# iammcy/BFLC-demo

Hardware: NVIDIA H100
Metric: federated_rounds_per_sec (higher is better)
Workload: dtype mxfp8

## Files before the change

### bflc_demo_b200/csrc/bindings/bindings_extra.cpp

```cpp
#include <ATen/cuda/CUDAContext.h>
#include <c10/cuda/CUDAGuard.h>
#include <torch/extension.h>

#include <cmath>
#include <cstring>
#include <memory>
#include <cuda.h>

#include <optional>

#include "bflc_kernels.h"
#include "consensus_math.hpp"
#include "symm_heap.hpp"

namespace py = pybind11;
using OptT = std::optional<at::Tensor>;

namespace {

void check(cudaError_t e, const char* what) {
  TORCH_CHECK(e == cudaSuccess, "bflc::", what, " failed: ", cudaGetErrorString(e));
}
cudaStream_t cur_stream() { return at::cuda::getCurrentCUDAStream().stream(); }

template <typename T>
T* P(int64_t addr) { return reinterpret_cast<T*>(static_cast<uintptr_t>(addr)); }

void check_flat(const at::Tensor& t, const char* what, at::ScalarType dtype, int64_t n, int align) {
  TORCH_CHECK(t.is_cuda() && t.is_contiguous() && t.scalar_type() == dtype, what, " must be a contiguous CUDA ",
              c10::toString(dtype), " tensor");
  TORCH_CHECK(t.numel() == n, what, " has ", t.numel(), " elements, expected ", n);
  TORCH_CHECK(reinterpret_cast<uintptr_t>(t.data_ptr()) % align == 0, what, " must be ", align, "-byte aligned");
}

const float* prox_anchor(const OptT& anchor, double mu, const at::Tensor& master, const char* what) {
  const float m32 = static_cast<float>(mu);
  TORCH_CHECK(std::isfinite(m32) && m32 >= 0.f, what, ": prox_mu must be finite and >= 0, got ", mu);
  if (m32 == 0.f) return nullptr;
  TORCH_CHECK(anchor.has_value(), what, ": prox_mu > 0 needs the anchor (the round's global model)");
  check_flat(*anchor, "anchor", at::kFloat, master.numel(), 16);
  TORCH_CHECK(anchor->device() == master.device(), what, ": anchor must be on master's device");
  return anchor->data_ptr<float>();
}

bflc::FedArgs make_fed(const py::dict& d) {
  bflc::FedArgs f;
  std::memset(&f, 0, sizeof(f));
  f.rank = d["rank"].cast<int>();
  f.n_ranks = d["n_ranks"].cast<int>();
  auto bases = d["peer_bases"].cast<std::vector<int64_t>>();
  TORCH_CHECK((int)bases.size() == f.n_ranks && f.n_ranks <= bflc::kMaxRanks, "bad peer table");
  for (int r = 0; r < f.n_ranks; ++r) f.peers.base[r] = P<char>(bases[r]);
  f.peers.mc_base = P<char>(d["mc_base"].cast<int64_t>());
  auto& l = f.lay;
  l.flags_off = d["flags_off"].cast<int64_t>();
  l.state_off = d["state_off"].cast<int64_t>();
  l.plan_off = d["plan_off"].cast<int64_t>();
  l.scores_off = d["scores_off"].cast<int64_t>();
  l.meta_off = d["meta_off"].cast<int64_t>();
  l.work_master_off = d["work_master_off"].cast<int64_t>();
  l.work_shadow_off = d["work_shadow_off"].cast<int64_t>();
  auto um = d["upload_master_off"].cast<std::vector<int64_t>>();
  auto us = d["upload_shadow_off"].cast<std::vector<int64_t>>();
  l.upload_master_off[0] = um.at(0); l.upload_master_off[1] = um.at(1);
  l.upload_shadow_off[0] = us.at(0); l.upload_shadow_off[1] = us.at(1);
  l.global_off = d["global_off"].cast<int64_t>();
  l.global_shadow_off = d["global_shadow_off"].cast<int64_t>();
  l.ring_off = d["ring_off"].cast<int64_t>();
  l.n_params = d["n_params"].cast<int64_t>();
  l.admit_off = d["admit_off"].cast<int64_t>();
  l.ring_slots = d["ring_slots"].cast<int>();
  return f;
}

struct PyHeap {
  std::unique_ptr<bflc::SymmHeap> h;
};

}

void bind_extra(py::module_& m) {
  py::class_<PyHeap>(m, "SymmHeap")
      .def(py::init([](int64_t bytes, int rank, int world, int device, const std::string& mode) {
        bflc::SymmHeap::Mode md = mode == "vmm"   ? bflc::SymmHeap::Mode::VMM
                                  : mode == "ipc" ? bflc::SymmHeap::Mode::IPC
                                                  : bflc::SymmHeap::Mode::LOCAL;
        auto p = std::make_unique<PyHeap>();
        p->h = std::make_unique<bflc::SymmHeap>((size_t)bytes, rank, world, device, md);
        return p;
      }))
      .def("export_handle", [](PyHeap& s) { return py::bytes(s.h->export_handle()); })
      .def("import_handles",
           [](PyHeap& s, const std::vector<py::bytes>& blobs) {
             std::vector<std::string> v;
             for (auto& b : blobs) v.emplace_back(static_cast<std::string>(b));
             s.h->import_handles(v);
           })
      .def("fd_listen", [](PyHeap& s, const std::string& tag) { return s.h->fd_listen(tag); })
      .def("import_via_sockets",
           [](PyHeap& s, const std::vector<std::string>& names) { s.h->import_via_sockets(names); })
      .def("mc_import_via_sockets",
           [](PyHeap& s, const std::vector<std::string>& names) { return s.h->mc_import_via_sockets(names); })
      .def("mc_create_and_export", [](PyHeap& s) { return py::bytes(s.h->mc_create_and_export()); })
      .def("mc_import_and_add",
           [](PyHeap& s, const py::bytes& b) { return s.h->mc_import_and_add(std::string(b)); })
      .def("mc_bind_and_map", [](PyHeap& s) { return s.h->mc_bind_and_map(); })
      .def("local_ptr", [](PyHeap& s) { return reinterpret_cast<int64_t>(s.h->local_ptr()); })
      .def("peer_ptr", [](PyHeap& s, int r) { return reinterpret_cast<int64_t>(s.h->peer_ptr(r)); })
      .def("mc_ptr", [](PyHeap& s) { return reinterpret_cast<int64_t>(s.h->mc_ptr()); })
      .def("bytes", [](PyHeap& s) { return (int64_t)s.h->bytes(); })
      .def("last_error", [](PyHeap& s) { return s.h->last_error(); })
      .def_static("multicast_supported", [](int dev) { return bflc::SymmHeap::multicast_supported(dev); });

  m.def("tensor_from_ptr", [](int64_t ptr, std::vector<int64_t> shape, py::object dtype, int device) {
    auto st = torch::python::detail::py_object_to_dtype(dtype);
    auto opts = at::TensorOptions().dtype(st).device(at::kCUDA, device);
    return at::for_blob(P<void>(ptr), shape)
        .deleter([](void*) {})
        .options(opts)
        .target_device(at::Device(at::kCUDA, static_cast<c10::DeviceIndex>(device)))
        .make_tensor();
  });

  m.def("struct_sizes", [] {
    py::dict d;
    d["RoundState"] = sizeof(bflc::RoundState);
    d["RoundPlan"] = sizeof(bflc::RoundPlan);
    d["BlockRecord"] = sizeof(bflc::BlockRecord);
    d["UploadMeta"] = sizeof(bflc::UploadMeta);
    d["AdmitPage"] = sizeof(bflc::AdmitPage);
    d["DpPage"] = sizeof(bflc::DpPage);
    d["dp_norm_off"] = offsetof(bflc::DpPage, norm);
    d["dp_scale_off"] = offsetof(bflc::DpPage, scale);
    d["dp_sigma_off"] = offsetof(bflc::DpPage, sigma);
    d["dp_epoch_off"] = offsetof(bflc::DpPage, epoch);
    d["FLAG_NORM"] = (int)bflc::FLAG_NORM;
    d["GemmDynamic"] = sizeof(bflc::GemmDynamic);
    d["FLAG_COUNT"] = (int)bflc::FLAG_COUNT;
    d["kMaxRanks"] = bflc::kMaxRanks;
    d["kMirrorSeqWord"] = bflc::kMirrorSeqWord;
    d["plan_dyn_off"] = offsetof(bflc::RoundPlan, dyn);
    d["plan_correct_off"] = offsetof(bflc::RoundPlan, correct);
    d["plan_loss_sum_off"] = offsetof(bflc::RoundPlan, loss_sum);
    d["plan_train_correct_off"] = offsetof(bflc::RoundPlan, train_correct);
    d["plan_opt_step_off"] = offsetof(bflc::RoundPlan, opt_step);
    d["plan_is_trainer_off"] = offsetof(bflc::RoundPlan, is_trainer);
    d["plan_is_comm_off"] = offsetof(bflc::RoundPlan, is_comm);
    d["plan_step_barrier_off"] = offsetof(bflc::RoundPlan, step_barrier);
    d["plan_stamps_off"] = offsetof(bflc::RoundPlan, t_stamp);
    d["plan_round_seq_off"] = offsetof(bflc::RoundPlan, round_seq);
    d["plan_opt_total_off"] = offsetof(bflc::RoundPlan, opt_total);
    d["plan_cand_blob_off"] = offsetof(bflc::RoundPlan, cand_blob);
    d["plan_n_cand_off"] = offsetof(bflc::RoundPlan, n_cand);
    d["plan_cand_rank_off"] = offsetof(bflc::RoundPlan, cand_rank);
    d["plan_parity_off"] = offsetof(bflc::RoundPlan, parity);
    d["plan_digest_acc_off"] = offsetof(bflc::RoundPlan, digest_acc);
    d["plan_upload_blocks_off"] = offsetof(bflc::RoundPlan, upload_blocks_done);
    d["plan_consensus_blocks_off"] = offsetof(bflc::RoundPlan, consensus_blocks_done);
    d["dyn_map_index_off"] = offsetof(bflc::GemmDynamic, map_index);
    d["dyn_bias_off"] = offsetof(bflc::GemmDynamic, bias);
    d["dyn_wait_flag_off"] = offsetof(bflc::GemmDynamic, wait_flag);
    d["dyn_wait_value_off"] = offsetof(bflc::GemmDynamic, wait_value);
    d["admit_slot_off"] = offsetof(bflc::AdmitPage, slot);
    d["rec_role_before_off"] = offsetof(bflc::BlockRecord, role_before);
    d["rec_score_rows_off"] = offsetof(bflc::BlockRecord, score_rows);
    d["rec_scored_mask_off"] = offsetof(bflc::BlockRecord, scored_mask);
    d["rec_median_off"] = offsetof(bflc::BlockRecord, median);
    d["rec_n_samples_off"] = offsetof(bflc::BlockRecord, n_samples);
    d["rec_avg_cost_off"] = offsetof(bflc::BlockRecord, avg_cost);
    d["rec_weight_off"] = offsetof(bflc::BlockRecord, weight);
    d["rec_admitted_mask_off"] = offsetof(bflc::BlockRecord, admitted_mask);
    d["rec_weight_by_score_off"] = offsetof(bflc::BlockRecord, weight_by_score);
    d["rec_model_digest_off"] = offsetof(bflc::BlockRecord, model_digest);
    d["rec_seq_off"] = offsetof(bflc::BlockRecord, seq);
    d["rec_agg_off"] = offsetof(bflc::BlockRecord, agg);
    d["state_epoch_off"] = offsetof(bflc::RoundState, epoch);
    d["state_role_off"] = offsetof(bflc::RoundState, role);
    d["state_global_loss_off"] = offsetof(bflc::RoundState, global_loss);
    d["state_digest_off"] = offsetof(bflc::RoundState, model_digest);
    d["CUtensorMap"] = sizeof(CUtensorMap);
    return d;
  });

  m.def("state_init_bytes", [](int n_ranks, int n_comm, int n_aggregate, std::vector<int> roles, int n_needed) {
    bflc::RoundState st;
    std::memset(&st, 0, sizeof(st));
    st.epoch = 0; st.n_ranks = n_ranks; st.n_comm = n_comm; st.n_aggregate = n_aggregate;
    st.n_needed = (uint32_t)n_needed;
    for (int r = 0; r < n_ranks && r < bflc::kMaxRanks; ++r) st.role[r] = (uint32_t)roles.at(r);
    return py::bytes(reinterpret_cast<const char*>(&st), sizeof(st));
  }, py::arg("n_ranks"), py::arg("n_comm"), py::arg("n_aggregate"), py::arg("roles"), py::arg("n_needed") = 0);

  m.def("fed_plan_round", [](const py::dict& fd, std::vector<std::pair<int64_t, bool>> layers,
                             int steps_per_round, bool staged, int64_t blob_stage_ptr, int64_t blob_bytes,
                             std::vector<int64_t> upq_off, int64_t stage_master_ptr) {
    bflc::FedArgs f = make_fed(fd);
    TORCH_CHECK(stage_master_ptr == 0 || staged, "stage_master_ptr: the fp32 staging slots of staged validation");
    bflc::PlanLayer pl[bflc::kMaxPlanLayers];
    TORCH_CHECK((int)layers.size() <= bflc::kMaxPlanLayers, "too many plan layers");
    for (size_t i = 0; i < layers.size(); ++i) {
      pl[i].bias_off = layers[i].first;
      pl[i].use_bias = layers[i].second ? 1 : 0;
    }
    bflc::PlanBlobs pb;
    const bool blobs = blob_bytes > 0;
    if (blobs) {
      TORCH_CHECK(upq_off.size() == 2, "upq_off: heap offsets of the two parity upload blobs");
      pb.stage = P<uint8_t>(blob_stage_ptr); pb.bytes = blob_bytes;
      pb.upq_off[0] = upq_off[0]; pb.upq_off[1] = upq_off[1];
    }
    check(bflc::fed_plan_round(f, pl, (int)layers.size(), steps_per_round, staged ? 1 : 0, cur_stream(),
                               blobs ? &pb : nullptr, P<const float>(stage_master_ptr)),
          "fed_plan_round");
  }, py::arg("fed"), py::arg("layers"), py::arg("steps_per_round"), py::arg("staged"),
     py::arg("blob_stage_ptr") = 0, py::arg("blob_bytes") = 0, py::arg("upq_off") = std::vector<int64_t>{},
     py::arg("stage_master_ptr") = 0);
  m.def("fed_pull_blobs", [](const py::dict& fd, int64_t off0, int64_t off1, at::Tensor stage, at::Tensor stage_dq,
                             int in_dim, int hidden, int n_classes, std::vector<int64_t> w_offs) {
    TORCH_CHECK(stage.dim() == 2 && stage_dq.dim() == 2 && stage.size(0) == stage_dq.size(0) &&
                    stage_dq.scalar_type() == at::kBFloat16 && stage.is_contiguous() && stage_dq.is_contiguous(),
                "stage: u8 [slots, blob_bytes]; stage_dq: bf16 [slots, n_params]");
    TORCH_CHECK(w_offs.size() == 2 && w_offs[0] + (int64_t)hidden * in_dim <= stage_dq.size(1) &&
                    w_offs[1] + (int64_t)n_classes * hidden <= stage_dq.size(1) && w_offs[0] % 8 == 0 &&
                    w_offs[1] % 8 == 0,
                "w_offs: 8-aligned element offsets of W1 and W2 inside a stage_dq row");
    const bflc::Mx8Unpack un = bflc::mx8_unpack_args(in_dim, hidden, n_classes, w_offs[0], w_offs[1]);
    check(bflc::fed_pull_blobs(make_fed(fd), off0, off1, un, stage.data_ptr(), stage.size(1), stage_dq.data_ptr(),
                               stage_dq.size(1), cur_stream()),
          "fed_pull_blobs");
  });
  m.def("fed_upload", [](const py::dict& fd, int n_samples, int n_loss_terms, int byz_mode,
                         double byz_scale, int straggle_us) {
    check(bflc::fed_upload(make_fed(fd), n_samples, n_loss_terms, byz_mode, (float)byz_scale, cur_stream(),
                           straggle_us),
          "fed_upload");
  }, py::arg("fed"), py::arg("n_samples"), py::arg("n_loss_terms"), py::arg("byz_mode"), py::arg("byz_scale"),
     py::arg("straggle_us") = 0);
  m.def("fed_consensus_aggregate", [](const py::dict& fd, int n_val, bool weight_by_score,
                                      bool two_shot, bool use_mc, int64_t host_mirror,
                                      int64_t bump_seq, int rule, int trim, int server_opt,
                                      const std::vector<float>& server_hp, int64_t server_m_off,
                                      int64_t server_v_off, int dp_mode, double dp_clip, double dp_noise,
                                      uint64_t dp_seed, int64_t dp_off) {
    TORCH_CHECK(bflc::agg_rule_valid(rule, trim), "fed_consensus_aggregate: rule must be 0 (FedAvg), 1 (median) "
                "or 2 (trimmed mean, 1 <= trim <= ", bflc::kMaxTrim, "), got rule ", rule, " trim ", trim);
    TORCH_CHECK(rule == bflc::AGG_FEDAVG || !weight_by_score,
                "fed_consensus_aggregate: weight_by_score needs the FedAvg rule");
    bflc::ServerOptArgs so{};
    so.opt = server_opt;
    if (server_opt != bflc::SOPT_NONE) {
      TORCH_CHECK(server_hp.size() == 6, "fed_consensus_aggregate: server_hp = (lr, b1, b2, c1, c2, tau)");
      so.lr = server_hp[0]; so.b1 = server_hp[1]; so.b2 = server_hp[2];
      so.c1 = server_hp[3]; so.c2 = server_hp[4]; so.tau = server_hp[5];
      so.m_off = server_m_off; so.v_off = server_v_off;
    }
    const char* err = bflc::server_opt_check(so.opt, so.lr, so.b1, so.b2, so.tau);
    TORCH_CHECK(*err == '\0', "fed_consensus_aggregate: ", err);
    TORCH_CHECK(server_opt == bflc::SOPT_NONE ||
                    (server_m_off > 0 && server_m_off % 16 == 0 &&
                     (bflc::server_state_vectors(server_opt) < 2 || (server_v_off > 0 && server_v_off % 16 == 0))),
                "fed_consensus_aggregate: server optimizer state offsets must be positive multiples of 16 "
                "(server_v_off for adam / yogi)");
    bflc::DpArgs dp{};
    dp.mode = dp_mode; dp.clip = (float)dp_clip; dp.noise = (float)dp_noise; dp.seed = dp_seed; dp.off = dp_off;
    const char* dperr = bflc::dp_check(dp.mode, dp.clip, dp.noise, rule);
    TORCH_CHECK(*dperr == '\0', "fed_consensus_aggregate: ", dperr);
    TORCH_CHECK(dp_mode == bflc::DP_OFF || (dp_off > 0 && dp_off % 16 == 0),
                "fed_consensus_aggregate: dp_off must be a positive multiple of 16 (the HeapLayout dp region)");
    check(bflc::fed_consensus_aggregate(make_fed(fd), n_val, weight_by_score ? 1 : 0,
                                        two_shot ? 1 : 0, use_mc ? 1 : 0, cur_stream(),
                                        P<uint32_t>(host_mirror), P<uint32_t>(bump_seq), rule, trim, &so, &dp),
          "fed_consensus_aggregate");
  }, py::arg("fed"), py::arg("n_val"), py::arg("weight_by_score"), py::arg("two_shot"),
     py::arg("use_mc"), py::arg("host_mirror") = 0, py::arg("bump_seq") = 0, py::arg("rule") = 0,
     py::arg("trim") = 0, py::arg("server_opt") = 0, py::arg("server_hp") = std::vector<float>{},
     py::arg("server_m_off") = 0, py::arg("server_v_off") = 0, py::arg("dp_mode") = 0, py::arg("dp_clip") = 0.0,
     py::arg("dp_noise") = 0.0, py::arg("dp_seed") = 0, py::arg("dp_off") = 0);
  m.def("fed_update_norms", [](const py::dict& fd, int64_t dp_off) {
    TORCH_CHECK(dp_off > 0 && dp_off % 16 == 0, "fed_update_norms: dp_off must be a positive multiple of 16");
    check(bflc::fed_update_norms(make_fed(fd), dp_off, cur_stream()), "fed_update_norms");
  }, py::arg("fed"), py::arg("dp_off"));
  m.def("fed_pull_candidates", [](const py::dict& fd, at::Tensor stage_shadow, const OptT& stage_master,
                                  const OptT& ranges) {
    const long long* rp = ranges.has_value() ? reinterpret_cast<const long long*>(ranges->data_ptr<int64_t>())
                                             : nullptr;
    check(bflc::fed_pull_candidates(make_fed(fd), stage_shadow.data_ptr(),
                                    stage_master.has_value() ? stage_master->data_ptr<float>() : nullptr,
                                    cur_stream(), rp, ranges.has_value() ? (int)ranges->size(0) : 0),
          "fed_pull_candidates");
  }, py::arg("fed"), py::arg("stage_shadow"), py::arg("stage_master"), py::arg("ranges") = py::none());
  m.def("fed_wait_trained", [](const py::dict& fd) {
    check(bflc::fed_wait_trained(make_fed(fd), cur_stream()), "fed_wait_trained");
  });
  m.def("set_predicate", [](int64_t ptr) { bflc::set_predicate(P<const int>(ptr)); });
  m.def("current_predicate_is_null", [] { return bflc::current_predicate() == nullptr; });
  m.def("set_pdl", [](bool on) { bflc::set_pdl(on); });
  m.def("pdl_fallbacks", [] { return bflc::pdl_fallbacks(); });
  m.def("set_debug_times", [](int64_t ptr) { bflc::set_debug_times(P<long long>(ptr)); });
  m.def("p2p_read_probe", [](int64_t src, int64_t dst, int64_t n_vec) {
    check(bflc::p2p_read_probe(P<const float4>(src), P<float4>(dst), n_vec, cur_stream()),
          "p2p_read_probe");
  });
  m.def("mc_store_probe", [](int64_t mc_dst, int64_t src, int64_t n_vec) {
    check(bflc::mc_store_probe(P<float4>(mc_dst), P<const float4>(src), n_vec, cur_stream()),
          "mc_store_probe");
  });

  m.def("mx8_mlp_layout", [](int in_dim, int hidden) {
    const bflc::Mx8MlpLayout l = bflc::mx8_mlp_layout(in_dim, hidden);
    py::dict d;
    d["w1q"] = l.w1q; d["w1sf"] = l.w1sf; d["w2q"] = l.w2q; d["w2sf"] = l.w2sf;
    d["b1"] = l.b1; d["b2"] = l.b2; d["total"] = l.total; d["kb1"] = l.kb1; d["kb2"] = l.kb2;
    return d;
  });
  m.def("mlp_round", [](at::Tensor x, at::Tensor labels, at::Tensor master, at::Tensor shadow,
                        at::Tensor grad, std::vector<int64_t> offs, at::Tensor h, at::Tensor dlogits,
                        at::Tensor dh, at::Tensor loss_sum, at::Tensor correct, int64_t barrier_ptr,
                        int batch, int steps, int in_dim, int hidden, int n_classes, double lr,
                        bool adam, const OptT& mm, const OptT& vv, int64_t step_base_ptr,
                        const OptT& dbg, int plan, int epiopt, int64_t x_ready_ptr,
                        int64_t round_seq_ptr, const OptT& x_dq, const OptT& work_q, const OptT& work_dq,
                        const OptT& h_dq, const std::optional<py::dict>& fed,
                        std::vector<int64_t> upq_off, int n_samples, int n_loss_terms, int byz_mode,
                        double byz_scale, int straggle_us, const OptT& anchor, double prox_mu,
                        int64_t epoch_rows) {
    TORCH_CHECK(offs.size() == 4, "offs = element offsets of w1, b1, w2, b2 in the flat buffer");
    if (epoch_rows == 0) epoch_rows = (int64_t)steps * batch;
    TORCH_CHECK(batch > 0 && steps > 0 && epoch_rows >= batch && epoch_rows % batch == 0 &&
                    epoch_rows / batch <= steps && epoch_rows <= INT32_MAX,
                "mlp_round: epoch_rows must be a multiple of batch, between batch and steps * batch (got ",
                epoch_rows, " rows, batch ", batch, ", steps ", steps, ")");
    auto rows_of = [&](const at::Tensor& t, const char* name, int64_t width, at::ScalarType dt) {
      TORCH_CHECK(t.is_cuda() && t.scalar_type() == dt && t.is_contiguous(), "mlp_round: ", name,
                  " must be a contiguous CUDA tensor of ", c10::toString(dt));
      TORCH_CHECK(t.numel() >= epoch_rows * width, "mlp_round: ", name, " holds ", t.numel() / width,
                  " rows, one local epoch reads ", epoch_rows);
    };
    rows_of(x, "x", in_dim, at::kBFloat16);
    rows_of(labels, "labels", 1, at::kInt);
    if (x_dq.has_value()) rows_of(*x_dq, "x_dq", in_dim, at::kBFloat16);
    bflc::MlpRoundArgs r;
    r.epoch_rows = (int)epoch_rows;
    r.prox_anchor = prox_anchor(anchor, prox_mu, master, "mlp_round");
    r.prox_mu = static_cast<float>(prox_mu);
    r.batch = batch; r.steps = steps; r.in_dim = in_dim; r.hidden = hidden; r.n_classes = n_classes;
    r.ncp = (int)dlogits.stride(0);
    r.n_params = master.numel();
    r.x = x.data_ptr(); r.labels = labels.data_ptr<int32_t>();
    float* mp = master.data_ptr<float>(); float* gp = grad.data_ptr<float>();
    auto* sp = reinterpret_cast<uint16_t*>(shadow.data_ptr());
    r.master = mp; r.shadow = sp; r.grad = gp;
    r.w1_shadow = sp + offs[0]; r.w2_shadow = sp + offs[2];
    r.b1 = mp + offs[1]; r.b2 = mp + offs[3];
    r.gw1 = gp + offs[0]; r.gb1 = gp + offs[1]; r.gw2 = gp + offs[2]; r.gb2 = gp + offs[3];
    r.h = h.data_ptr(); r.dlogits = dlogits.data_ptr(); r.dh = dh.data_ptr();
    r.loss_sum = loss_sum.data_ptr<float>();
    r.correct = reinterpret_cast<unsigned int*>(correct.data_ptr());
    r.barrier = P<unsigned int>(barrier_ptr);
    r.adam = adam;
    r.adam_m = mm.has_value() ? mm->data_ptr<float>() : nullptr;
    r.adam_v = vv.has_value() ? vv->data_ptr<float>() : nullptr;
    r.lr = (float)lr;
    r.step_base = P<const int>(step_base_ptr);
    r.plan = plan; r.epiopt = epiopt;
    r.x_ready = P<const unsigned int>(x_ready_ptr); r.round_seq = P<const unsigned int>(round_seq_ptr);
    if (dbg.has_value()) {
      TORCH_CHECK(dbg->numel() >= (int64_t)steps * 32 && dbg->element_size() == 8, "dbg: int64 [steps, 32]");
      r.dbg = reinterpret_cast<unsigned long long*>(dbg->data_ptr());
    }
    if (x_dq.has_value()) {
      TORCH_CHECK(work_q.has_value() && work_dq.has_value() && h_dq.has_value(),
                  "fp8 mode needs x_dq, work_q, work_dq, h_dq");
      TORCH_CHECK(x_dq->scalar_type() == at::kBFloat16 && work_dq->scalar_type() == at::kBFloat16 &&
                      h_dq->scalar_type() == at::kBFloat16 &&
                      work_dq->numel() >= (int64_t)hidden * in_dim + 64LL * hidden,
                  "x_dq / h_dq: bf16; work_dq: bf16 [hidden * in_dim + 64 * hidden]");
      r.fp8 = true;
      r.x_dq = x_dq->data_ptr();
      r.work_q = work_q->data_ptr<uint8_t>();
      r.work_dq = reinterpret_cast<uint16_t*>(work_dq->data_ptr());
      r.h_dq = h_dq->data_ptr();
    }
    bflc::FedArgs f;
    if (fed.has_value()) {
      f = make_fed(*fed);
      r.fed = &f;
      if (upq_off.size() == 2) { r.upq_off[0] = upq_off[0]; r.upq_off[1] = upq_off[1]; }
      r.n_samples = n_samples; r.n_loss_terms = n_loss_terms; r.byz_mode = byz_mode; r.byz_scale = (float)byz_scale;
      r.straggle_us = straggle_us;
    }
    check(bflc::mlp_round_sm100(r, cur_stream()), "mlp_round_sm100");
  }, py::arg("x"), py::arg("labels"), py::arg("master"), py::arg("shadow"), py::arg("grad"), py::arg("offs"),
     py::arg("h"), py::arg("dlogits"), py::arg("dh"), py::arg("loss_sum"), py::arg("correct"),
     py::arg("barrier_ptr"), py::arg("batch"), py::arg("steps"), py::arg("in_dim"), py::arg("hidden"),
     py::arg("n_classes"), py::arg("lr"), py::arg("adam"), py::arg("m"), py::arg("v"),
     py::arg("step_base_ptr"), py::arg("dbg"), py::arg("plan"), py::arg("epiopt"), py::arg("x_ready_ptr") = 0,
     py::arg("round_seq_ptr") = 0, py::arg("x_dq") = py::none(), py::arg("work_q") = py::none(),
     py::arg("work_dq") = py::none(), py::arg("h_dq") = py::none(),
     py::arg("fed") = py::none(), py::arg("upq_off") = std::vector<int64_t>{}, py::arg("n_samples") = 0,
     py::arg("n_loss_terms") = 0, py::arg("byz_mode") = 0, py::arg("byz_scale") = 0.0,
     py::arg("straggle_us") = 0, py::arg("anchor") = py::none(), py::arg("prox_mu") = 0.0,
     py::arg("epoch_rows") = 0);
  m.def("mlp_val", [](at::Tensor x, at::Tensor labels, at::Tensor correct, at::Tensor maps,
                      int64_t dyn1_ptr, int64_t dyn2_ptr, int n_val, int in_dim, int hidden,
                      int n_classes, int max_cand, int64_t cand_blob_ptr) {
    TORCH_CHECK(x.scalar_type() == at::kBFloat16, "x: bf16 (fp8 mode: the dequantised MXFP8 x)");
    bflc::MlpValArgs r;
    r.n_val = n_val; r.in_dim = in_dim; r.hidden = hidden; r.n_classes = n_classes;
    r.max_cand = max_cand;
    r.x = x.data_ptr(); r.ldx = x.stride(0);
    r.maps = reinterpret_cast<const CUtensorMap*>(maps.data_ptr());
    r.dyn1 = P<const bflc::GemmDynamic>(dyn1_ptr);
    r.dyn2 = P<const bflc::GemmDynamic>(dyn2_ptr);
    r.labels = labels.data_ptr<int32_t>();
    r.correct = reinterpret_cast<unsigned int*>(correct.data_ptr());
    if (cand_blob_ptr != 0) {
      r.fp8 = true;
      r.cand_blob = P<const uint8_t* const>(cand_blob_ptr);
    }
    check(bflc::mlp_val_sm100(r, cur_stream()), "mlp_val_sm100");
  }, py::arg("x"), py::arg("labels"), py::arg("correct"), py::arg("maps"), py::arg("dyn1_ptr"),
     py::arg("dyn2_ptr"), py::arg("n_val"), py::arg("in_dim"), py::arg("hidden"), py::arg("n_classes"),
     py::arg("max_cand"), py::arg("cand_blob_ptr") = 0);
  m.def("quantize_mlp_blob", [](at::Tensor master, std::vector<int64_t> offs, int in_dim, int hidden,
                                int n_classes, at::Tensor blob, const OptT& dq) {
    TORCH_CHECK(offs.size() == 4, "offs = element offsets of w1, b1, w2, b2");
    TORCH_CHECK(!dq.has_value() || (dq->scalar_type() == at::kBFloat16 &&
                                    dq->numel() >= (int64_t)hidden * in_dim + 64LL * hidden),
                "dq: bf16 [hidden * in_dim + 64 * hidden]");
    check(bflc::quantize_mlp_blob(master.data_ptr<float>(), offs[0], offs[1], offs[2], offs[3], in_dim, hidden,
                                  n_classes, blob.data_ptr<uint8_t>(), cur_stream(),
                                  dq.has_value() ? dq->data_ptr() : nullptr),
          "quantize_mlp_blob");
  }, py::arg("master"), py::arg("offs"), py::arg("in_dim"), py::arg("hidden"), py::arg("n_classes"),
     py::arg("blob"), py::arg("dq") = py::none());
  m.def("mx8_dequant", [](at::Tensor q, at::Tensor sf, at::Tensor dst) {
    TORCH_CHECK(q.dim() == 2 && q.is_contiguous() && q.element_size() == 1, "q: contiguous e4m3 / u8 [R, K]");
    TORCH_CHECK(dst.sizes() == q.sizes() && dst.is_contiguous() && dst.scalar_type() == at::kBFloat16,
                "dst: contiguous bf16 [R, K]");
    check(bflc::mx8_dequant_bf16(q.data_ptr(), sf.data_ptr<uint8_t>(), (int)q.size(0), (int)q.size(1),
                                 dst.data_ptr(), cur_stream()),
          "mx8_dequant_bf16");
  });
  m.def("optim_step",
        [](bool adam, at::Tensor master, at::Tensor grad, const OptT& shadow, const OptT& mm,
           const OptT& vv, double lr, double wd, double b1, double b2, double eps, int step,
           int64_t step_dev_ptr, int64_t active_ptr, bool zero_grad) {
          const int64_t n = master.numel();
          check_flat(master, "master", at::kFloat, n, 16);
          check_flat(grad, "grad", at::kFloat, n, 16);
          if (shadow.has_value()) check_flat(*shadow, "shadow", at::kBFloat16, n, 8);
          if (adam) {
            TORCH_CHECK(mm.has_value() && vv.has_value(), "adam needs m and v");
            check_flat(*mm, "m", at::kFloat, n, 16);
            check_flat(*vv, "v", at::kFloat, n, 16);
            TORCH_CHECK(step >= 1, "adam step must be >= 1 (bias correction 1 - beta^t), got ", step);
          }
          bflc::OptimArgs a;
          a.master = master.data_ptr<float>();
          a.grad = grad.data_ptr<float>();
          a.shadow_bf16 = shadow.has_value() ? shadow->data_ptr() : nullptr;
          a.n = master.numel();
          a.lr = (float)lr; a.weight_decay = (float)wd;
          a.m = mm.has_value() ? mm->data_ptr<float>() : nullptr;
          a.v = vv.has_value() ? vv->data_ptr<float>() : nullptr;
          a.beta1 = (float)b1; a.beta2 = (float)b2; a.eps = (float)eps;
          a.step = step;
          a.step_dev = P<const int>(step_dev_ptr);
          a.active = active_ptr ? P<const int>(active_ptr) : bflc::current_predicate();
          a.zero_grad = zero_grad ? 1 : 0;
          check(adam ? bflc::adam_step(a, cur_stream()) : bflc::sgd_step(a, cur_stream()),
                "optim_step");
        });
  m.def("grad_norm_workspace_bytes", [] { return bflc::kGradNormWorkspaceBytes; });
  m.def("grad_norm",
        [](at::Tensor grad, at::Tensor workspace, at::Tensor norms, int64_t index, double max_norm,
           const OptT& skipped, int64_t active_ptr) {
          auto f32 = [](const at::Tensor& t, const char* what) {
            TORCH_CHECK(t.is_cuda() && t.is_contiguous() && t.scalar_type() == at::kFloat, what,
                        " must be a contiguous CUDA float32 tensor");
          };
          check_flat(grad, "grad", at::kFloat, grad.numel(), 16);
          f32(norms, "norms");
          TORCH_CHECK(grad.numel() > 0, "grad is empty");
          TORCH_CHECK(workspace.is_cuda() && workspace.is_contiguous() && workspace.scalar_type() == at::kByte &&
                          workspace.numel() >= bflc::kGradNormWorkspaceBytes &&
                          reinterpret_cast<uintptr_t>(workspace.data_ptr()) % 8 == 0,
                      "workspace must be an 8-byte aligned contiguous CUDA uint8 tensor of grad_norm_workspace_bytes()");
          TORCH_CHECK(0 <= index && index < norms.numel(), "norm index ", index, " outside norms[", norms.numel(), "]");
          TORCH_CHECK(max_norm > 0, "max_norm must be > 0");
          if (skipped.has_value())
            TORCH_CHECK(skipped->is_cuda() && skipped->scalar_type() == at::kInt && skipped->numel() >= 1,
                        "skipped must be a CUDA int32 tensor");
          check(bflc::grad_norm_f32(grad.data_ptr<float>(), grad.numel(), workspace.data_ptr(),
                                    norms.data_ptr<float>() + index, (float)max_norm,
                                    skipped.has_value() ? skipped->data_ptr<int>() : nullptr,
                                    active_ptr ? P<const int>(active_ptr) : bflc::current_predicate(), cur_stream()),
                "grad_norm");
        },
        py::arg("grad"), py::arg("workspace"), py::arg("norms"), py::arg("index"), py::arg("max_norm"),
        py::arg("skipped") = py::none(), py::arg("active_ptr") = 0);
  m.def("optim_recipe_step",
        [](bool adam, at::Tensor master, at::Tensor grad, const OptT& shadow, const OptT& mm, const OptT& vv,
           double lr, double b1, double b2, double eps, int step, int64_t step_dev_ptr, double decay,
           const OptT& no_decay, int schedule, int warmup, int total, const OptT& clip_workspace,
           int64_t active_ptr, bool zero_grad, const OptT& anchor, double prox_mu) {
          const int64_t n = master.numel();
          check_flat(master, "master", at::kFloat, n, 16);
          check_flat(grad, "grad", at::kFloat, n, 16);
          if (shadow.has_value()) check_flat(*shadow, "shadow", at::kBFloat16, n, 8);
          if (adam) {
            TORCH_CHECK(mm.has_value() && vv.has_value(), "adam needs m and v");
            check_flat(*mm, "m", at::kFloat, n, 16);
            check_flat(*vv, "v", at::kFloat, n, 16);
          }
          const float* anc = prox_anchor(anchor, prox_mu, master, "optim_recipe_step");
          TORCH_CHECK(step >= 1, "step must be >= 1, got ", step);
          TORCH_CHECK(schedule >= bflc::kLrConstant && schedule <= bflc::kLrCosine, "schedule id ", schedule,
                      " outside [0, 2] (constant, linear, cosine)");
          TORCH_CHECK(warmup >= 0 && total >= 0, "warmup and total steps must be >= 0");
          TORCH_CHECK(schedule == bflc::kLrConstant || total > warmup,
                      "a decaying schedule needs total steps > warmup steps");
          TORCH_CHECK(decay >= 0, "weight decay must be >= 0");
          if (no_decay.has_value()) {
            TORCH_CHECK(no_decay->is_cuda() && no_decay->is_contiguous() && no_decay->scalar_type() == at::kInt,
                        "no_decay must be a contiguous CUDA int32 tensor");
            TORCH_CHECK(no_decay->numel() == (n + 255) / 256, "no_decay has ", no_decay->numel(),
                        " words, n = ", n, " needs ", (n + 255) / 256, " (one bit per 8 floats)");
          }
          TORCH_CHECK(decay == 0 || no_decay.has_value(), "weight decay needs the no_decay mask");
          if (clip_workspace.has_value())
            TORCH_CHECK(clip_workspace->is_cuda() && clip_workspace->scalar_type() == at::kByte &&
                            clip_workspace->numel() >= bflc::kGradNormWorkspaceBytes &&
                            reinterpret_cast<uintptr_t>(clip_workspace->data_ptr()) % 8 == 0,
                        "clip_workspace must be grad_norm's CUDA uint8 workspace");
          bflc::RecipeArgs a;
          a.master = master.data_ptr<float>();
          a.grad = grad.data_ptr<float>();
          a.shadow_bf16 = shadow.has_value() ? shadow->data_ptr() : nullptr;
          a.n = n;
          a.lr = (float)lr;
          a.m = adam ? mm->data_ptr<float>() : nullptr;
          a.v = adam ? vv->data_ptr<float>() : nullptr;
          a.beta1 = (float)b1; a.beta2 = (float)b2; a.eps = (float)eps;
          a.step = step;
          a.step_dev = P<const int>(step_dev_ptr);
          a.active = active_ptr ? P<const int>(active_ptr) : bflc::current_predicate();
          a.zero_grad = zero_grad ? 1 : 0;
          a.decay = (float)decay;
          a.no_decay = no_decay.has_value() ? reinterpret_cast<const uint32_t*>(no_decay->data_ptr<int>()) : nullptr;
          a.schedule = schedule; a.warmup = warmup; a.total = total;
          a.clip = clip_workspace.has_value() ? static_cast<const bflc::GradNormState*>(clip_workspace->data_ptr())
                                              : nullptr;
          a.anchor = anc;
          a.mu = static_cast<float>(prox_mu);
          check(adam ? bflc::adam_recipe_step(a, cur_stream()) : bflc::sgd_recipe_step(a, cur_stream()),
                "optim_recipe_step");
        },
        py::arg("adam"), py::arg("master"), py::arg("grad"), py::arg("shadow"), py::arg("m"), py::arg("v"),
        py::arg("lr"), py::arg("beta1"), py::arg("beta2"), py::arg("eps"), py::arg("step"), py::arg("step_dev_ptr"),
        py::arg("decay"), py::arg("no_decay"), py::arg("schedule"), py::arg("warmup"), py::arg("total"),
        py::arg("clip_workspace"), py::arg("active_ptr") = 0, py::arg("zero_grad") = true,
        py::arg("anchor") = py::none(), py::arg("prox_mu") = 0.0);

  m.def("cast_f32_to_bf16", [](at::Tensor src, at::Tensor dst) {
    check_flat(src, "src", at::kFloat, src.numel(), 16);
    check_flat(dst, "dst", at::kBFloat16, src.numel(), 16);
    check(bflc::cast_f32_to_bf16(src.data_ptr<float>(), dst.data_ptr(), src.numel(), cur_stream()),
          "cast_f32_to_bf16");
  });
  m.def("cast_bf16_to_f32", [](at::Tensor src, at::Tensor dst) {
    check(bflc::cast_bf16_to_f32(src.data_ptr(), dst.data_ptr<float>(), src.numel(), cur_stream()),
          "cast_bf16_to_f32");
  });
  m.def("prep_inputs", [](at::Tensor src, const OptT& dst_bf16, const OptT& dst_q, const OptT& dst_sf,
                          double scale, const OptT& dst_dq) {
    TORCH_CHECK(src.dim() == 2 && src.is_contiguous(), "src: contiguous u8 [R, K]");
    TORCH_CHECK(!dst_dq.has_value() || (dst_dq->scalar_type() == at::kBFloat16 && dst_dq->numel() >= src.numel()),
                "dst_dq: bf16 [R, K]");
    check(bflc::prep_inputs_u8(src.data_ptr<uint8_t>(), dst_bf16.has_value() ? dst_bf16->data_ptr() : nullptr,
// ... 105 lines not shown
```

### bflc_demo_b200/csrc/include/bflc_kernels.h

```cpp
#pragma once
#include <cstdint>
#include <cuda.h>
#include <cuda_runtime.h>

namespace bflc {

enum class DType : int { F32 = 0, BF16 = 1, FP8_E4M3 = 2, U8 = 3 };
enum class Act : int { NONE = 0, RELU = 1, GELU = 2 };
enum class EpiKind : int { GENERIC = 0, XENT = 1, ARGMAX_ACC = 2 };

struct GemmOperand {
  const void* ptr = nullptr;
  int64_t ld = 0;
  int64_t batch_stride = 0;
  bool mn_major = false;
};

struct GemmEpilogue {
  EpiKind kind = EpiKind::GENERIC;
  void* d = nullptr;
  DType d_dtype = DType::BF16;
  int64_t ldd = 0;
  int64_t d_batch_stride = 0;
  float alpha = 1.f;
// ... 130 lines not shown
cudaError_t mlp_val_sm100(const MlpValArgs& r, cudaStream_t stream);

cudaError_t prep_inputs_u8(const uint8_t* src, void* dst_bf16, void* dst_q, uint8_t* dst_sf, int R,
                           int K, float scale, cudaStream_t s, void* dst_dq = nullptr);
cudaError_t prep_inputs_u8_chunks(const uint8_t* src, void* dst_bf16, void* dst_q, uint8_t* dst_sf,
                                  int rows_per_chunk, int K, int n_chunks, float scale,
                                  const int* in_flags, const int* in_seq, unsigned int* cnt,
                                  unsigned int* ready, unsigned int* err, cudaStream_t s,
                                  void* dst_dq = nullptr);
cudaError_t mx8_dequant_bf16(const void* q, const uint8_t* sf, int R, int K, void* dst, cudaStream_t s);
cudaError_t quantize_mlp_blob(const float* master, long long off_w1, long long off_b1,
                              long long off_w2, long long off_b2, int in_dim, int hidden,
                              int n_classes, uint8_t* blob, cudaStream_t s, void* dq = nullptr);

int gemm_pick_bn(int N, EpiKind kind, int M, int z);
unsigned long long launch_count();
void note_launch();

cudaError_t cast_f32_to_bf16(const float* src, void* dst, int64_t n, cudaStream_t s);
cudaError_t cast_bf16_to_f32(const void* src, float* dst, int64_t n, cudaStream_t s);
cudaError_t cast_u8_to_bf16(const uint8_t* src, void* dst, int64_t n, float scale, cudaStream_t s);
cudaError_t quantize_fp8(const void* src_bf16, uint8_t* dst, int64_t n, float inv_scale,
                         cudaStream_t s);
cudaError_t amax_bf16(const void* src, int64_t n, float* amax_out, cudaStream_t s);
cudaError_t fill_f32(float* dst, int64_t n, float v, cudaStream_t s);

struct OptimArgs {
  float* master = nullptr;
  const float* grad = nullptr;
  void* shadow_bf16 = nullptr;
  int64_t n = 0;
  float lr = 1e-3f, weight_decay = 0.f;
  float* m = nullptr;
  float* v = nullptr;
  float beta1 = 0.9f, beta2 = 0.999f, eps = 1e-8f;
  const int* step_dev = nullptr;
  int step = 1;
  const int* active = nullptr;
  int zero_grad = 1;
};
cudaError_t sgd_step(const OptimArgs& a, cudaStream_t s);
cudaError_t adam_step(const OptimArgs& a, cudaStream_t s);

enum LrSchedule : int { kLrConstant = 0, kLrLinear = 1, kLrCosine = 2 };
struct GradNormState {
  float coef;
  int nonfinite;
  unsigned int ticket;
  int pad;
};
constexpr int kGradNormMaxCtas = 132 * 8;
constexpr int64_t kGradNormWorkspaceBytes = sizeof(GradNormState) + 8 * kGradNormMaxCtas;
struct RecipeArgs : OptimArgs {
  float decay = 0.f;
  const uint32_t* no_decay = nullptr;
  int schedule = kLrConstant, warmup = 0, total = 0;
  const GradNormState* clip = nullptr;
  const float* anchor = nullptr;
  float mu = 0.f;
};
cudaError_t sgd_recipe_step(const RecipeArgs& a, cudaStream_t s);
cudaError_t adam_recipe_step(const RecipeArgs& a, cudaStream_t s);
cudaError_t grad_norm_f32(const float* grad, int64_t n, void* workspace, float* norm_out, float max_norm,
                          int* skipped, const int* active, cudaStream_t s);

cudaError_t im2col_bf16(const void* x, void* col, int N, int C, int H, int W, int KH, int KW,
                        int stride, int pad, int OH, int OW, int64_t ld_col, cudaStream_t s);
cudaError_t upsample_zero_bf16(const void* dy, void* up, int N, int H, int W, int OH, int OW, int C,
                               int stride, cudaStream_t s);
cudaError_t col2im_bf16(const void* col, void* dx, int N, int C, int H, int W, int KH, int KW,
                        int stride, int pad, int OH, int OW, int64_t ld_col, cudaStream_t s);
cudaError_t maxpool2d_fwd(const void* x, void* y, int32_t* idx, int N, int C, int H, int W, int k,
                          int stride, int pad, int OH, int OW, cudaStream_t s);
cudaError_t maxpool2d_bwd(const void* dy, const int32_t* idx, float* dx_f32, int64_t n_out,
                          int64_t per_out, int64_t per_in, cudaStream_t s);
cudaError_t avgpool_global_fwd(const void* x, void* y, int N, int HW, int C, cudaStream_t s);
cudaError_t avgpool_global_bwd(const void* dy, void* dx, int N, int HW, int C, cudaStream_t s);
cudaError_t batchnorm_fwd(const void* x, void* y, const float* gamma, const float* beta,
                          float* mean, float* rstd, float* run_mean, float* run_var,
                          int64_t rows, int C, float eps, float momentum, int training, int relu,
                          const void* residual, cudaStream_t s);
cudaError_t batchnorm_bwd(const void* dy, const void* x, const void* y, const float* gamma,
                          const float* mean, const float* rstd, void* dx, float* dgamma,
                          float* dbeta, void* dresidual, int64_t rows, int C, int relu,
                          cudaStream_t s);
cudaError_t layernorm_fwd(const void* x, const void* residual, void* y, const float* gamma,
                          const float* beta, float* mean, float* rstd, int64_t rows, int C,
                          float eps, cudaStream_t s);
cudaError_t layernorm_bwd(const void* dy, const void* xin, const float* gamma, const float* mean,
                          const float* rstd, void* dx, float* dgamma, float* dbeta, int64_t rows,
                          int C, cudaStream_t s);
cudaError_t softmax_rows_fwd(const void* x, void* y, int64_t rows, int cols, float scale,
                             cudaStream_t s);
cudaError_t softmax_rows_bwd(const void* dy, const void* y, void* dx, int64_t rows, int cols,
                             float scale, cudaStream_t s);
cudaError_t embedding_fwd(const int32_t* ids, const void* table_bf16, const void* pos_bf16,
                          void* out, int64_t rows, int seq, int C, cudaStream_t s,
                          const int32_t* pos_ids = nullptr);
cudaError_t embedding_bwd(const int32_t* ids, const void* dy, float* dtable, float* dpos,
                          int64_t rows, int seq, int C, cudaStream_t s, const int32_t* pos_ids = nullptr);
cudaError_t add_bf16(const void* a, const void* b, void* out, int64_t n, cudaStream_t s);
cudaError_t act_bwd_colsum(const void* dy, const void* aux, void* dz, float* colsum, int64_t rows,
                           int C, int mode, cudaStream_t s);
struct DropoutArgs {
  float p = 0.f;
  uint64_t seed = 0;
  const int32_t* step = nullptr;
  int step_add = 0;
  uint32_t site = 0;
};
cudaError_t attention_fwd_sm100(const void* q, const void* k, const void* v, void* o, float* lse, int B,
                                int S, int H, int D, long long ld, float scale, cudaStream_t stream,
                                const int32_t* lengths, const DropoutArgs* drop = nullptr, bool causal = false);
cudaError_t attention_bwd_sm100(const void* q, const void* k, const void* v, const void* o,
                                const void* dout, const float* lse, void* dq, void* dk, void* dv, int B,
                                int S, int H, int D, long long ld, float scale, cudaStream_t stream,
                                float* delta, const int32_t* lengths, const DropoutArgs* drop = nullptr,
                                bool causal = false);
cudaError_t attention_packed_fwd_sm100(const void* q, const void* k, const void* v, void* o, float* lse,
                                       const int32_t* cu_seqlens, int B, int T, int max_seqlen, int H, int D,
                                       long long ld, float scale, cudaStream_t stream,
                                       const DropoutArgs* drop = nullptr);
cudaError_t attention_packed_bwd_sm100(const void* q, const void* k, const void* v, const void* o,
                                       const void* dout, const float* lse, void* dq, void* dk, void* dv,
                                       const int32_t* cu_seqlens, int B, int T, int max_seqlen, int H, int D,
                                       long long ld, float scale, cudaStream_t stream, float* delta,
                                       const DropoutArgs* drop = nullptr);
cudaError_t dropout_keep_mask(uint8_t* mask, int B, int H, int S, const DropoutArgs& drop, cudaStream_t s);
cudaError_t dropout_add_bf16(const void* x, const void* z, void* y, int64_t rows, int C, int S,
                             const int32_t* seq_ids, const int32_t* pos_ids, const DropoutArgs& drop,
                             cudaStream_t s);
cudaError_t transpose_0213_bf16(const void* x, void* y, int d0, int d1, int d2, int d3,
                                cudaStream_t s);
cudaError_t xent_rows(const float* logits, int64_t M, int V, int64_t ld, const int32_t* targets, float* loss,
                      int32_t* hits, void* dlogits, int64_t ldd, float grad_scale, cudaStream_t s);

constexpr int kMaxRanks = 8;
constexpr int kMaxPlanLayers = 4;

struct GemmDynamic {
  int active_batches;
  int map_index[kMaxRanks];
  const float* bias[kMaxRanks];
  const uint32_t* wait_flag[kMaxRanks];
  uint32_t wait_value;
};

struct RoundState {
  uint32_t epoch;
  uint32_t n_ranks, n_comm, n_aggregate;
  uint32_t role[kMaxRanks];
  float last_median[kMaxRanks];
  uint32_t selected_mask;
  float global_loss;
  unsigned long long model_digest;
  uint32_t blocks_appended;
  uint32_t n_needed;
};

struct UploadMeta {
  uint32_t n_samples;
  float avg_cost;
};

struct RoundPlan {
  int is_trainer;
  int is_comm;
  int n_cand;
  int cand_rank[kMaxRanks];
  uint32_t parity;
  GemmDynamic dyn[kMaxPlanLayers];
  const uint8_t* cand_blob[kMaxRanks];
  unsigned int correct[kMaxRanks];
  float loss_sum;
  unsigned int train_correct;
  int opt_step;
  int opt_total;
  unsigned int upload_blocks_done;
  unsigned int consensus_blocks_done;
  unsigned long long digest_acc;
  unsigned int step_barrier;
  unsigned int round_seq;
  unsigned long long t_stamp[8];
};

enum StampSlot : int {
  STAMP_PLAN = 0,
  STAMP_UPLOAD_BEGIN = 1,
  STAMP_UPLOAD_END = 2,
  STAMP_PULL_BEGIN = 3,
  STAMP_PULL_END = 4,
  STAMP_CONS_BEGIN = 5,
  STAMP_CONS_SCORED = 6,
  STAMP_CONS_END = 7,
};

struct PeerTable {
  char* base[kMaxRanks];
  char* mc_base;
};

struct HeapLayout {
  long long flags_off;
  long long state_off;
  long long plan_off;
  long long scores_off;
  long long meta_off;
  long long work_master_off;
  long long work_shadow_off;
  long long upload_master_off[2];
  long long upload_shadow_off[2];
  long long global_off;
  long long global_shadow_off;
  long long ring_off;
  long long n_params;
  long long admit_off;
  int ring_slots;
  int pad;
};

struct AdmitPage {
  uint32_t ticket;
  uint32_t slot[kMaxRanks];
  uint32_t pad[7];
};

struct BlockRecord {
  uint32_t epoch;
  uint32_t n_ranks, n_comm, n_aggregate;
  uint32_t role_before[kMaxRanks];
  uint32_t role_after[kMaxRanks];
  float score_rows[kMaxRanks][kMaxRanks];
  uint32_t scored_mask[kMaxRanks];
  float median[kMaxRanks];
  uint32_t n_samples[kMaxRanks];
  float avg_cost[kMaxRanks];
  float weight[kMaxRanks];
  uint32_t admitted_mask;
  uint32_t selected_mask;
  float global_loss;
  uint32_t weight_by_score;
  unsigned long long model_digest;
  uint32_t seq;
  uint32_t agg;
};

enum FlagSlot : int {
  FLAG_TRAINED = 0,
  FLAG_SCORED = 8,
  FLAG_DONE = 16,
  FLAG_SLICE = 24,
  FLAG_NORM = 32,
  FLAG_COUNT = 64
};

constexpr int kDpMaxBlocks = 132 * 4;
struct DpPage {
  double partial[2][kMaxRanks][kMaxRanks];
  float norm[kMaxRanks];
  float scale[kMaxRanks];
  float sigma;
  uint32_t epoch;
  unsigned int ticket;
  uint32_t pad;
  double block[kDpMaxBlocks][kMaxRanks];
};

struct FedArgs {
  PeerTable peers;
  HeapLayout lay;
  int rank;
  int n_ranks;
};

struct PlanLayer {
  long long bias_off;
  int use_bias;
};

struct PlanBlobs {
  uint8_t* stage = nullptr; long long bytes = 0; long long upq_off[2] = {0, 0};
};
cudaError_t fed_plan_round(const FedArgs& f, const PlanLayer* layers, int n_layers,
                           int steps_per_round, int staged, cudaStream_t s,
                           const PlanBlobs* blobs = nullptr, const float* stage_master = nullptr);
cudaError_t fed_upload(const FedArgs& f, int n_samples, int n_loss_terms, int byz_mode,
                       float byz_scale, cudaStream_t s, int straggle_us = 0);
constexpr int kMirrorSeqWord = 64;
struct ServerOptArgs {
  int opt;
  float lr, b1, b2, c1, c2, tau;
  long long m_off, v_off;
};
struct DpArgs {
  int mode;
  float clip, noise;
  unsigned long long seed;
  long long off;
};
cudaError_t fed_consensus_aggregate(const FedArgs& f, int n_val, int weight_by_score,
                                    int two_shot, int use_multicast, cudaStream_t s,
                                    uint32_t* host_mirror = nullptr, uint32_t* bump_seq = nullptr,
                                    int rule = 0, int trim = 0, const ServerOptArgs* so = nullptr,
                                    const DpArgs* dp = nullptr);
cudaError_t fed_update_norms(const FedArgs& f, long long dp_off, cudaStream_t s);

cudaError_t fed_pull_candidates(const FedArgs& f, void* stage_shadow, float* stage_master,
                                cudaStream_t s, const long long* ranges = nullptr, int n_ranges = 0);
cudaError_t fed_pull_blobs(const FedArgs& f, long long off0, long long off1, const Mx8Unpack& un,
                           void* stage_blob, long long blob_bytes, void* stage_dq, long long stage_stride,
                           cudaStream_t s);
cudaError_t fed_wait_trained(const FedArgs& f, cudaStream_t s);

void set_predicate(const int* pred);
void set_pdl(bool on);
bool pdl_enabled();
unsigned long long pdl_fallbacks();
void set_debug_times(long long* dev_buf8);
const int* current_predicate();

cudaError_t p2p_read_probe(const float4* peer_src, float4* local_dst, int64_t n_vec,
                           cudaStream_t s);
cudaError_t mc_store_probe(float4* mc_dst, const float4* local_src, int64_t n_vec,
                           cudaStream_t s);

}
```

### bflc_demo_b200/csrc/kernels/elementwise_optim.cu

```cuda
#include <cuda_bf16.h>
#include <cuda_fp8.h>

#include "bflc_kernels.h"
#include "epi_common.cuh"
#include "launch.cuh"
#include "sm100_ptx.cuh"

namespace bflc {

namespace {

constexpr int kBlock = 256;
inline int grid_for(int64_t n_vec) {
  int64_t g = (n_vec + kBlock - 1) / kBlock;
  const int64_t cap = 132 * 8;
  if (g > cap) g = cap;
  if (g < 1) g = 1;
  return static_cast<int>(g);
}

using epi::pack_bf16x2;

__global__ void k_cast_f32_bf16(const float* __restrict__ src, __nv_bfloat16* __restrict__ dst,
                                int64_t n) {
// ... 132 lines not shown
}

__device__ __forceinline__ float prox_grad(float g, float w, float w0, float mu) {
  return __fmaf_rn(mu, __fsub_rn(w, w0), g);
}

template <bool kAdam, bool kRecipe = false>
__global__ void k_optim(OptimParams<kRecipe> a) {
  ptx::pdl_launch_dependents();
  ptx::pdl_wait();
  if (a.active != nullptr && *a.active == 0) return;
  const int64_t tid = blockIdx.x * static_cast<int64_t>(blockDim.x) + threadIdx.x;
  const int64_t stride = static_cast<int64_t>(gridDim.x) * blockDim.x;
  float bc1 = 1.f, bc2 = 1.f;
  if (kAdam) {
    const int t = (a.step_dev ? *a.step_dev : 0) + a.step;
    bc1 = 1.f - powf(a.beta1, static_cast<float>(t));
    bc2 = 1.f - powf(a.beta2, static_cast<float>(t));
  }
  float lr = a.lr, coef = 1.f, dec = 0.f;
  if constexpr (kRecipe) {
    if (a.clip != nullptr) {
      coef = a.clip->coef;
      if (a.clip->nonfinite) {
        if (a.zero_grad) {
          float* g = const_cast<float*>(a.grad);
          for (int64_t i = tid; i < a.n / 4; i += stride)
            reinterpret_cast<float4*>(g)[i] = make_float4(0.f, 0.f, 0.f, 0.f);
          for (int64_t i = a.n / 4 * 4 + tid; i < a.n; i += stride) g[i] = 0.f;
        }
        return;
      }
    }
    const int t = (a.step_dev ? *a.step_dev : 0) + a.step;
    lr = a.lr * lr_factor(a.schedule, a.warmup, a.total, t - 1);
    dec = lr * a.decay;
  }
  const int64_t nv = a.n / 4;
  __nv_bfloat16* sh = reinterpret_cast<__nv_bfloat16*>(a.shadow_bf16);
  for (int64_t i = tid; i < nv; i += stride) {
    float4 w = reinterpret_cast<float4*>(a.master)[i];
    const float4 g4 = reinterpret_cast<const float4*>(a.grad)[i];
    float wv[4] = {w.x, w.y, w.z, w.w};
    const float gv[4] = {g4.x, g4.y, g4.z, g4.w};
    float keep = 1.f;
    float gq[4] = {gv[0], gv[1], gv[2], gv[3]};
    if constexpr (kRecipe) {
      keep = 1.f - block_decay(a.no_decay, i >> 1, dec);
#pragma unroll
      for (int k = 0; k < 4; ++k) gq[k] = __fmul_rn(coef, gv[k]);
      if (a.anchor != nullptr) {
        const float4 w0 = __ldg(reinterpret_cast<const float4*>(a.anchor) + i);
        gq[0] = prox_grad(gq[0], wv[0], w0.x, a.mu); gq[1] = prox_grad(gq[1], wv[1], w0.y, a.mu);
        gq[2] = prox_grad(gq[2], wv[2], w0.z, a.mu); gq[3] = prox_grad(gq[3], wv[3], w0.w, a.mu);
      }
    }
    if (kAdam) {
      float4 m4 = reinterpret_cast<float4*>(a.m)[i];
      float4 v4 = reinterpret_cast<float4*>(a.v)[i];
      float mv[4] = {m4.x, m4.y, m4.z, m4.w};
      float vv[4] = {v4.x, v4.y, v4.z, v4.w};
#pragma unroll
      for (int k = 0; k < 4; ++k) {
        if constexpr (kRecipe) {
          recipe_update<true>(wv[k], mv[k], vv[k], gq[k], keep, a, lr, bc1, bc2);
        } else {
          const float g = gv[k] + a.weight_decay * wv[k];
          mv[k] = a.beta1 * mv[k] + (1.f - a.beta1) * g;
          vv[k] = a.beta2 * vv[k] + (1.f - a.beta2) * g * g;
          wv[k] -= a.lr * (mv[k] / bc1) / (sqrtf(vv[k] / bc2) + a.eps);
        }
      }
      reinterpret_cast<float4*>(a.m)[i] = make_float4(mv[0], mv[1], mv[2], mv[3]);
      reinterpret_cast<float4*>(a.v)[i] = make_float4(vv[0], vv[1], vv[2], vv[3]);
    } else {
#pragma unroll
      for (int k = 0; k < 4; ++k) {
        if constexpr (kRecipe) {
          float m_unused = 0.f, v_unused = 0.f;
          recipe_update<false>(wv[k], m_unused, v_unused, gq[k], keep, a, lr, bc1, bc2);
        } else {
          wv[k] -= a.lr * (gv[k] + a.weight_decay * wv[k]);
        }
      }
    }
    reinterpret_cast<float4*>(a.master)[i] = make_float4(wv[0], wv[1], wv[2], wv[3]);
    if (sh) {
      uint2 o;
      o.x = pack_bf16x2(wv[0], wv[1]);
      o.y = pack_bf16x2(wv[2], wv[3]);
      reinterpret_cast<uint2*>(sh)[i] = o;
    }
    if (a.zero_grad)
      reinterpret_cast<float4*>(const_cast<float*>(a.grad))[i] = make_float4(0.f, 0.f, 0.f, 0.f);
  }
  for (int64_t i = nv * 4 + tid; i < a.n; i += stride) {
    float w = a.master[i];
    if constexpr (kRecipe) {
      float m = kAdam ? a.m[i] : 0.f, v = kAdam ? a.v[i] : 0.f;
      float g = __fmul_rn(coef, a.grad[i]);
      if (a.anchor != nullptr) g = prox_grad(g, w, __ldg(a.anchor + i), a.mu);
      recipe_update<kAdam>(w, m, v, g, 1.f - block_decay(a.no_decay, i >> 3, dec), a, lr, bc1, bc2);
      if (kAdam) { a.m[i] = m; a.v[i] = v; }
    } else {
      float g = a.grad[i] + a.weight_decay * w;
      if (kAdam) {
        const float m = a.beta1 * a.m[i] + (1.f - a.beta1) * g;
        const float v = a.beta2 * a.v[i] + (1.f - a.beta2) * g * g;
        a.m[i] = m; a.v[i] = v;
        w -= a.lr * (m / bc1) / (sqrtf(v / bc2) + a.eps);
      } else {
        w -= a.lr * g;
      }
    }
    a.master[i] = w;
    if (sh) sh[i] = __float2bfloat16(w);
    if (a.zero_grad) const_cast<float*>(a.grad)[i] = 0.f;
  }
}

struct NormArgs {
  const float* grad; int64_t n; GradNormState* st; double* partials; float* norm_out; float max_norm;
  int* skipped; const int* active;
};

__device__ __forceinline__ double block_sum(double x, double* red) {
#pragma unroll
  for (int off = 16; off >= 1; off >>= 1) x += __shfl_xor_sync(0xffffffffu, x, off);
  if ((threadIdx.x & 31) == 0) red[threadIdx.x >> 5] = x;
  __syncthreads();
  double s = 0.0;
#pragma unroll
  for (int w = 0; w < kBlock / 32; ++w) s += red[w];
  return s;
}

__global__ void __launch_bounds__(kBlock) k_grad_norm(NormArgs a) {
  ptx::pdl_launch_dependents();
  ptx::pdl_wait();
  if (a.active != nullptr && *a.active == 0) return;
  __shared__ double red[kBlock / 32];
  __shared__ bool last;
  const int64_t tid = blockIdx.x * static_cast<int64_t>(blockDim.x) + threadIdx.x;
  const int64_t stride = static_cast<int64_t>(gridDim.x) * blockDim.x;
  const int64_t nv = a.n / 4;
  double acc = 0.0;
  for (int64_t i = tid; i < nv; i += stride) {
    const float4 g = reinterpret_cast<const float4*>(a.grad)[i];
    acc = fma(static_cast<double>(g.x), static_cast<double>(g.x), acc);
    acc = fma(static_cast<double>(g.y), static_cast<double>(g.y), acc);
    acc = fma(static_cast<double>(g.z), static_cast<double>(g.z), acc);
    acc = fma(static_cast<double>(g.w), static_cast<double>(g.w), acc);
  }
  for (int64_t i = nv * 4 + tid; i < a.n; i += stride) acc = fma(static_cast<double>(a.grad[i]), static_cast<double>(a.grad[i]), acc);
  const double cta = block_sum(acc, red);
  if (threadIdx.x == 0) {
    a.partials[blockIdx.x] = cta;
    __threadfence();
    last = atomicAdd(&a.st->ticket, 1u) == gridDim.x - 1;
  }
  __syncthreads();
  if (!last) return;
  __threadfence();
  double p = 0.0;
  for (int j = threadIdx.x; j < static_cast<int>(gridDim.x); j += kBlock) p += __ldcg(a.partials + j);
  __syncthreads();
  const double total = block_sum(p, red);
  if (threadIdx.x == 0) {
    const float norm = static_cast<float>(sqrt(total));
    const bool bad = !isfinite(norm);
    *a.norm_out = norm;
    a.st->coef = bad ? 1.f : fminf(1.f, __fdiv_rn(a.max_norm, norm + 1e-6f));
    a.st->nonfinite = bad ? 1 : 0;
    if (bad && a.skipped != nullptr) *a.skipped += 1;
    a.st->ticket = 0u;
  }
}

__device__ __forceinline__ void prep_group(const uint8_t* __restrict__ src, __nv_bfloat16* dbf, uint8_t* dq,
                                           uint8_t* dsf, __nv_bfloat16* ddq, int row, int g, int K, int n_kb,
                                           float scale) {
  const int k0 = g * 32;
  const int n = K - k0 < 32 ? K - k0 : 32;
  const long long off = static_cast<long long>(row) * K + k0;
  uint32_t wd[8] = {0, 0, 0, 0, 0, 0, 0, 0};
  {
    const uint4 a = __ldcg(reinterpret_cast<const uint4*>(src + off));
    wd[0] = a.x; wd[1] = a.y; wd[2] = a.z; wd[3] = a.w;
    if (n > 16) {
      const uint4 b = __ldcg(reinterpret_cast<const uint4*>(src + off + 16));
      wd[4] = b.x; wd[5] = b.y; wd[6] = b.z; wd[7] = b.w;
    }
  }
  float v[32];
#pragma unroll
  for (int i = 0; i < 32; ++i) v[i] = static_cast<float>((wd[i >> 2] >> (8 * (i & 3))) & 0xffu) * scale;
  if (dbf != nullptr) {
    uint4* o = reinterpret_cast<uint4*>(dbf + off);
#pragma unroll
    for (int i = 0; i < 4; ++i) {
      if (i * 8 >= n) break;
      o[i] = make_uint4(pack_bf16x2(v[8 * i], v[8 * i + 1]), pack_bf16x2(v[8 * i + 2], v[8 * i + 3]),
                        pack_bf16x2(v[8 * i + 4], v[8 * i + 5]), pack_bf16x2(v[8 * i + 6], v[8 * i + 7]));
    }
  }
  if (dq != nullptr || ddq != nullptr) {
    uint32_t w[8];
    const int e = epi::mx8_quant32(v, w);
    if (dq != nullptr) {
      uint4* o = reinterpret_cast<uint4*>(dq + off);
      o[0] = make_uint4(w[0], w[1], w[2], w[3]);
      if (n > 16) o[1] = make_uint4(w[4], w[5], w[6], w[7]);
      dsf[epi::mx8_sf_index(row, g, n_kb)] = static_cast<uint8_t>(e);
    }
    if (ddq != nullptr) epi::mx8_dq32_store(w, e, ddq + off, n);
  }
}

struct PrepArgs {
  const uint8_t* src; __nv_bfloat16* dbf; uint8_t* dq; uint8_t* dsf; __nv_bfloat16* ddq;
  int R, K; float scale;
  int rows_per_chunk, n_chunks;
  const int* in_flags;
  const int* in_seq;
  unsigned int* cnt;
  unsigned int* ready;
  unsigned int* err;
};

__global__ void __launch_bounds__(256) k_prep_inputs(PrepArgs a, const int* pred) {
  ptx::pdl_launch_dependents();
  ptx::pdl_wait();
  if (pred != nullptr && *pred == 0) return;
  const int G = (a.K + 31) / 32, n_kb = (a.K + 127) / 128;
  const long long total = static_cast<long long>(a.R) * G;
  const long long stride = static_cast<long long>(gridDim.x) * blockDim.x;
  for (long long i = blockIdx.x * static_cast<long long>(blockDim.x) + threadIdx.x; i < total; i += stride)
    prep_group(a.src, a.dbf, a.dq, a.dsf, a.ddq, static_cast<int>(i / G), static_cast<int>(i % G), a.K, n_kb,
               a.scale);
}

__global__ void __launch_bounds__(256) k_mx8_dequant(const uint8_t* __restrict__ q, const uint8_t* __restrict__ sf,
                                                     int R, int K, __nv_bfloat16* __restrict__ dst) {
  ptx::pdl_launch_dependents();
  ptx::pdl_wait();
  const int G = (K + 31) / 32, n_kb = (K + 127) / 128;
  const long long total = static_cast<long long>(R) * G;
  const long long stride = static_cast<long long>(gridDim.x) * blockDim.x;
  for (long long i = blockIdx.x * static_cast<long long>(blockDim.x) + threadIdx.x; i < total; i += stride) {
    const int row = static_cast<int>(i / G), g = static_cast<int>(i % G);
    const int n = K - g * 32 < 32 ? K - g * 32 : 32;
    const long long off = static_cast<long long>(row) * K + g * 32;
    uint32_t w[8] = {0, 0, 0, 0, 0, 0, 0, 0};
    const uint4 a = *reinterpret_cast<const uint4*>(q + off);
    w[0] = a.x; w[1] = a.y; w[2] = a.z; w[3] = a.w;
    if (n > 16) {
      const uint4 b = *reinterpret_cast<const uint4*>(q + off + 16);
      w[4] = b.x; w[5] = b.y; w[6] = b.z; w[7] = b.w;
    }
    epi::mx8_dq32_store(w, sf[epi::mx8_sf_index(row, g, n_kb)], dst + off, n);
  }
}

__global__ void __launch_bounds__(256) k_prep_chunks(PrepArgs a) {
  ptx::pdl_launch_dependents();
  ptx::pdl_wait();
  const int want = *reinterpret_cast<const volatile int*>(a.in_seq) + 1;
  const int G = (a.K + 31) / 32, n_kb = (a.K + 127) / 128;
  const long long per = static_cast<long long>(a.rows_per_chunk) * G;
  const long long tid = blockIdx.x * static_cast<long long>(blockDim.x) + threadIdx.x;
  const long long stride = static_cast<long long>(gridDim.x) * blockDim.x;
  for (int s = 0; s < a.n_chunks; ++s) {
    if (threadIdx.x == 0) {
      unsigned long long spins = 0;
      unsigned int ns = 20;
      while (static_cast<int>(ptx::ld_acquire_sys(reinterpret_cast<const uint32_t*>(a.in_flags + s))) - want < 0) {
        if (++spins > (1ull << 14)) { __nanosleep(ns); if (ns < 2000) ns *= 2; }
        if (spins > (1ull << 14) + 5000000ull) {
          if (a.err != nullptr) atomicExch(a.err, 1u);
          break;
        }
      }
    }
    __syncthreads();
    const int row0 = s * a.rows_per_chunk;
    for (long long i = tid; i < per; i += stride)
      prep_group(a.src, a.dbf, a.dq, a.dsf, a.ddq, row0 + static_cast<int>(i / G), static_cast<int>(i % G), a.K,
                 n_kb, a.scale);
    __syncthreads();
    if (threadIdx.x == 0) {
      __threadfence();
      const unsigned int old = atomicAdd(a.cnt + s, 1u);
      if ((old + 1u) % gridDim.x == 0u)
        asm volatile("st.release.gpu.global.u32 [%0], %1;" ::"l"(a.ready + s), "r"(static_cast<unsigned int>(want))
                     : "memory");
    }
  }
}

struct BlobArgs {
  const float* master; long long off_w1, off_b1, off_w2, off_b2;
  int in_dim, hidden, n_classes; uint8_t* blob; Mx8MlpLayout l; __nv_bfloat16* dq;
};
__device__ __forceinline__ void blob_group(const float* w, int ld, int rows, int K, int row, int g, int n_kb,
                                           uint8_t* q, uint8_t* sf, int q_rows, __nv_bfloat16* dq) {
  uint8_t* sfp = sf + epi::mx8_sf_index(row, g, n_kb);
  const int k0 = g * 32;
  if (k0 >= K || row >= q_rows) { *sfp = 127; return; }
  const int n = K - k0 < 32 ? K - k0 : 32;
  float v[32];
#pragma unroll
  for (int i = 0; i < 32; ++i) v[i] = (row < rows && i < n) ? w[static_cast<long long>(row) * ld + k0 + i] : 0.f;
  uint32_t o[8];
  const int e = epi::mx8_quant32(v, o);
  *sfp = static_cast<uint8_t>(e);
  uint8_t* qp = q + static_cast<long long>(row) * ld + k0;
  for (int i = 0; i < n / 4; ++i) reinterpret_cast<uint32_t*>(qp)[i] = o[i];
  if (dq != nullptr) {
    __nv_bfloat16* d = dq + static_cast<long long>(row) * ld + k0;
    for (int i = 0; i < n / 4; ++i) *reinterpret_cast<uint2*>(d + 4 * i) = epi::mx8_dq4(o[i], e);
  }
}
__global__ void __launch_bounds__(256) k_quantize_mlp_blob(BlobArgs a) {
  ptx::pdl_launch_dependents();
  ptx::pdl_wait();
  const int g1 = a.l.kb1 * 4, g2 = a.l.kb2 * 4;
  const int r1 = (a.hidden + 127) / 128 * 128;
  const long long n1 = static_cast<long long>(r1) * g1, n2 = 128LL * g2, n3 = a.hidden + 64;
  const long long stride = static_cast<long long>(gridDim.x) * blockDim.x;
  for (long long i = blockIdx.x * static_cast<long long>(blockDim.x) + threadIdx.x; i < n1 + n2 + n3; i += stride) {
    if (i < n1) {
      blob_group(a.master + a.off_w1, a.in_dim, a.hidden, a.in_dim, static_cast<int>(i / g1), static_cast<int>(i % g1),
                 a.l.kb1, a.blob + a.l.w1q, a.blob + a.l.w1sf, a.hidden, a.dq);
    } else if (i < n1 + n2) {
      const long long u = i - n1;
      blob_group(a.master + a.off_w2, a.hidden, a.n_classes, a.hidden, static_cast<int>(u / g2), static_cast<int>(u % g2),
                 a.l.kb2, a.blob + a.l.w2q, a.blob + a.l.w2sf, 64,
                 a.dq != nullptr ? a.dq + static_cast<long long>(a.hidden) * a.in_dim : nullptr);
    } else {
      const int u = static_cast<int>(i - n1 - n2);
      float* b = reinterpret_cast<float*>(a.blob + (u < a.hidden ? a.l.b1 + 4 * u : a.l.b2 + 4 * (u - a.hidden)));
      *b = u < a.hidden ? a.master[a.off_b1 + u]
                        : (u - a.hidden < a.n_classes ? a.master[a.off_b2 + u - a.hidden] : 0.f);
    }
  }
}

}

#define BFLC_LAUNCH_1D(kernel, nvec, ...)                       \
  do {                                                          \
    (void)cudaGetLastError();  \
    kernel<<<grid_for(nvec), kBlock, 0, s>>>(__VA_ARGS__);      \
    note_launch();                                              \
    return cudaGetLastError();                                  \
  } while (0)

#define BFLC_LAUNCH_1D_PDL(kernel, nvec, ...)                                          \
  do {                                                                                \
    note_launch();                                                                    \
    return launch_pdl(kernel, dim3(grid_for(nvec)), dim3(kBlock), 0, s, __VA_ARGS__); \
  } while (0)

cudaError_t cast_f32_to_bf16(const float* src, void* dst, int64_t n, cudaStream_t s) {
  BFLC_LAUNCH_1D(k_cast_f32_bf16, n / 8 + 1, src, reinterpret_cast<__nv_bfloat16*>(dst), n);
}
cudaError_t cast_bf16_to_f32(const void* src, float* dst, int64_t n, cudaStream_t s) {
  BFLC_LAUNCH_1D(k_cast_bf16_f32, n, reinterpret_cast<const __nv_bfloat16*>(src), dst, n);
}
cudaError_t prep_inputs_u8(const uint8_t* src, void* dst_bf16, void* dst_q, uint8_t* dst_sf, int R,
                           int K, float scale, cudaStream_t s, void* dst_dq) {
  if (K % 16 != 0 || R <= 0 || (dst_q != nullptr && dst_sf == nullptr)) return cudaErrorInvalidValue;
  PrepArgs a{};
  a.src = src; a.dbf = reinterpret_cast<__nv_bfloat16*>(dst_bf16); a.dq = static_cast<uint8_t*>(dst_q);
  a.dsf = dst_sf; a.ddq = static_cast<__nv_bfloat16*>(dst_dq); a.R = R; a.K = K; a.scale = scale;
  const long long total = static_cast<long long>(R) * ((K + 31) / 32);
  note_launch();
  return launch_pdl(k_prep_inputs, dim3(grid_for(total)), dim3(kBlock), 0, s, a, current_predicate());
}
cudaError_t prep_inputs_u8_chunks(const uint8_t* src, void* dst_bf16, void* dst_q, uint8_t* dst_sf,
                                  int rows_per_chunk, int K, int n_chunks, float scale,
                                  const int* in_flags, const int* in_seq, unsigned int* cnt,
                                  unsigned int* ready, unsigned int* err, cudaStream_t s, void* dst_dq) {
  if (K % 16 != 0 || n_chunks <= 0 || rows_per_chunk <= 0 || (dst_q != nullptr && dst_sf == nullptr))
    return cudaErrorInvalidValue;
  PrepArgs a{};
  a.src = src; a.dbf = reinterpret_cast<__nv_bfloat16*>(dst_bf16); a.dq = static_cast<uint8_t*>(dst_q);
  a.dsf = dst_sf; a.ddq = static_cast<__nv_bfloat16*>(dst_dq); a.R = rows_per_chunk * n_chunks; a.K = K; a.scale = scale;
  a.rows_per_chunk = rows_per_chunk; a.n_chunks = n_chunks;
  a.in_flags = in_flags; a.in_seq = in_seq; a.cnt = cnt; a.ready = ready; a.err = err;
  note_launch();
  return launch_pdl(k_prep_chunks, dim3(16), dim3(256), 0, s, a);
}
cudaError_t quantize_mlp_blob(const float* master, long long off_w1, long long off_b1,
                              long long off_w2, long long off_b2, int in_dim, int hidden,
                              int n_classes, uint8_t* blob, cudaStream_t s, void* dq) {
  if (in_dim % 4 != 0 || hidden % 4 != 0 || n_classes > 64) return cudaErrorInvalidValue;
  BlobArgs a{master, off_w1, off_b1, off_w2, off_b2, in_dim, hidden, n_classes, blob,
             mx8_mlp_layout(in_dim, hidden), static_cast<__nv_bfloat16*>(dq)};
  const long long total = static_cast<long long>((hidden + 127) / 128 * 128) * a.l.kb1 * 4 + 128LL * a.l.kb2 * 4 +
                          hidden + 64;
  note_launch();
  return launch_pdl(k_quantize_mlp_blob, dim3(grid_for(total)), dim3(kBlock), 0, s, a);
}
cudaError_t mx8_dequant_bf16(const void* q, const uint8_t* sf, int R, int K, void* dst, cudaStream_t s) {
  if (K % 16 != 0 || R <= 0) return cudaErrorInvalidValue;
  note_launch();
  return launch_pdl(k_mx8_dequant, dim3(grid_for(static_cast<long long>(R) * ((K + 31) / 32))), dim3(kBlock), 0, s,
                    static_cast<const uint8_t*>(q), sf, R, K, static_cast<__nv_bfloat16*>(dst));
}
cudaError_t cast_u8_to_bf16(const uint8_t* src, void* dst, int64_t n, float scale,
                            cudaStream_t s) {
  BFLC_LAUNCH_1D_PDL(k_cast_u8_bf16, n / 16 + 1, src, reinterpret_cast<__nv_bfloat16*>(dst), n,
                     scale, current_predicate());
}
cudaError_t quantize_fp8(const void* src_bf16, uint8_t* dst, int64_t n, float inv_scale,
                         cudaStream_t s) {
  BFLC_LAUNCH_1D(k_quant_fp8, n / 8 + 1, reinterpret_cast<const __nv_bfloat16*>(src_bf16), dst, n,
                 inv_scale);
}
cudaError_t amax_bf16(const void* src, int64_t n, float* amax_out, cudaStream_t s) {
  BFLC_LAUNCH_1D(k_amax_bf16, n, reinterpret_cast<const __nv_bfloat16*>(src), n, amax_out);
}
cudaError_t fill_f32(float* dst, int64_t n, float v, cudaStream_t s) {
  BFLC_LAUNCH_1D(k_fill, n, dst, n, v);
}
cudaError_t add_bf16(const void* a, const void* b, void* out, int64_t n, cudaStream_t s) {
  BFLC_LAUNCH_1D(k_add_bf16, n / 8 + 1, reinterpret_cast<const __nv_bfloat16*>(a),
                 reinterpret_cast<const __nv_bfloat16*>(b), reinterpret_cast<__nv_bfloat16*>(out),
                 n);
}
cudaError_t sgd_step(const OptimArgs& a, cudaStream_t s) {
  BFLC_LAUNCH_1D_PDL(k_optim<false>, a.n / 4 + 1, a);
}
cudaError_t adam_step(const OptimArgs& a, cudaStream_t s) {
  if (!a.m || !a.v) return cudaErrorInvalidValue;
  BFLC_LAUNCH_1D_PDL(k_optim<true>, a.n / 4 + 1, a);
}

static bool recipe_ok(const RecipeArgs& a) {
  if (a.schedule < kLrConstant || a.schedule > kLrCosine || a.warmup < 0 || a.total < 0 || !(a.decay >= 0.f))
    return false;
  if (a.schedule != kLrConstant && a.total <= a.warmup) return false;
  return a.decay == 0.f || a.no_decay != nullptr;
}
cudaError_t sgd_recipe_step(const RecipeArgs& a, cudaStream_t s) {
  if (!recipe_ok(a)) return cudaErrorInvalidValue;
  BFLC_LAUNCH_1D_PDL((k_optim<false, true>), a.n / 4 + 1, a);
}
cudaError_t adam_recipe_step(const RecipeArgs& a, cudaStream_t s) {
  if (!a.m || !a.v || !recipe_ok(a)) return cudaErrorInvalidValue;
  BFLC_LAUNCH_1D_PDL((k_optim<true, true>), a.n / 4 + 1, a);
}
cudaError_t grad_norm_f32(const float* grad, int64_t n, void* workspace, float* norm_out, float max_norm,
                          int* skipped, const int* active, cudaStream_t s) {
  if (workspace == nullptr || norm_out == nullptr || n <= 0) return cudaErrorInvalidValue;
  NormArgs a{grad, n, static_cast<GradNormState*>(workspace),
             reinterpret_cast<double*>(static_cast<char*>(workspace) + sizeof(GradNormState)), norm_out,
             max_norm, skipped, active};
  static_assert(sizeof(GradNormState) % 8 == 0, "partials must be 8-byte aligned");
  BFLC_LAUNCH_1D_PDL(k_grad_norm, n / 4 + 1, a);
}

}
```

### bflc_demo_b200/csrc/kernels/fed_kernels.cu

```cuda
#include <cuda_bf16.h>

#include "bflc_kernels.h"
#include "consensus_math.hpp"
#include "epi_common.cuh"
#include "fed_admit.cuh"
#include "launch.cuh"
#include "sm100_ptx.cuh"

namespace bflc {

namespace {

constexpr int kFedThreads = 256;

template <typename T>
__device__ __forceinline__ T* at(char* base, long long off) {
  return reinterpret_cast<T*>(base + off);
}

__device__ __forceinline__ uint32_t pack_bf16x2(float a, float b) {
  __nv_bfloat162 t = __floats2bfloat162_rn(a, b);
  return *reinterpret_cast<uint32_t*>(&t);
}

struct PlanLayers {
  PlanLayer l[kMaxPlanLayers];
  int n;
  int steps_per_round;
  int staged;
  int use_blob;
  uint8_t* stage_blob; long long blob_bytes; long long upq_off[2];
  const float* stage_master;
};

__device__ __forceinline__ unsigned long long globaltimer_ns() {
  unsigned long long t;
  asm volatile("mov.u64 %0, %%globaltimer;" : "=l"(t));
  return t;
}
__device__ __forceinline__ void stamp(RoundPlan* plan, int slot) {
  atomicMax(&plan->t_stamp[slot], globaltimer_ns());
}

__global__ void k_plan(FedArgs f, PlanLayers layers) {
  ptx::pdl_launch_dependents();
  ptx::pdl_wait();
  if (threadIdx.x != 0 || blockIdx.x != 0) return;
  char* me = f.peers.base[f.rank];
  const RoundState* st = at<RoundState>(me, f.lay.state_off);
  RoundPlan* plan = at<RoundPlan>(me, f.lay.plan_off);
  for (int i = 0; i < 8; ++i) plan->t_stamp[i] = 0;
  plan->t_stamp[STAMP_PLAN] = globaltimer_ns();
  uint32_t* flags = at<uint32_t>(me, f.lay.flags_off);
  const uint32_t epoch = st->epoch;
  const uint32_t par = epoch & 1u;
  if (epoch >= 2) {
    for (int r = 0; r < f.n_ranks; ++r) ptx::wait_flag_ge(flags + FLAG_DONE + r, epoch - 1);
  }
  plan->is_trainer = (st->role[f.rank] & ROLE_TRAINER) ? 1 : 0;
  plan->is_comm = (st->role[f.rank] & ROLE_COMM) ? 1 : 0;
  plan->parity = par;
  int n_cand = 0;
  for (int r = 0; r < f.n_ranks; ++r)
    if (st->role[r] & ROLE_TRAINER) plan->cand_rank[n_cand++] = r;
  if (admit::first_k(st)) {
    n_cand = static_cast<int>(st->n_needed);
    for (int z = 0; z < kMaxRanks; ++z) plan->cand_rank[z] = -1;
  }
  plan->n_cand = n_cand;
  for (int l = 0; l < layers.n; ++l) {
    GemmDynamic& d = plan->dyn[l];
    d.active_batches = plan->is_comm ? n_cand : 0;
    d.wait_value = epoch + 1;
    for (int z = 0; z < kMaxRanks; ++z) {
      const int t = (z < n_cand && plan->cand_rank[z] >= 0) ? plan->cand_rank[z] : 0;
      d.map_index[z] = layers.staged ? (l * kMaxRanks + z)
                                     : ((l * 2 + static_cast<int>(par)) * kMaxRanks + t);
      const float* params = layers.staged && layers.stage_master != nullptr
                                ? layers.stage_master + static_cast<long long>(z) * f.lay.n_params
                                : at<float>(f.peers.base[t], f.lay.upload_master_off[par]);
      d.bias[z] = layers.l[l].use_bias ? params + layers.l[l].bias_off : nullptr;
      d.wait_flag[z] = layers.staged ? nullptr : flags + FLAG_TRAINED + t;
    }
  }
  for (int z = 0; z < kMaxRanks; ++z) {
    plan->correct[z] = 0;
    const int t = (z < n_cand && plan->cand_rank[z] >= 0) ? plan->cand_rank[z] : f.rank;
    plan->cand_blob[z] = !layers.use_blob ? nullptr
                         : layers.staged  ? layers.stage_blob + z * layers.blob_bytes
                                          : reinterpret_cast<const uint8_t*>(f.peers.base[t]) + layers.upq_off[par];
  }
  plan->loss_sum = 0.f;
  plan->train_correct = 0;
  plan->upload_blocks_done = 0;
  plan->consensus_blocks_done = 0;
  plan->digest_acc = 0ull;
  plan->step_barrier = 0u;
  plan->round_seq = plan->round_seq + 1u;
  plan->opt_step = plan->opt_total;
  if (plan->is_trainer) plan->opt_total += layers.steps_per_round;
}

__global__ void __launch_bounds__(kFedThreads)
k_upload(FedArgs f, int n_samples, int n_loss_terms, int byz_mode, float byz_scale, int straggle_us) {
  ptx::pdl_launch_dependents();
  ptx::pdl_wait();
  char* me = f.peers.base[f.rank];
  const RoundState* st = at<RoundState>(me, f.lay.state_off);
  RoundPlan* plan = at<RoundPlan>(me, f.lay.plan_off);
  if (!(st->role[f.rank] & ROLE_TRAINER)) return;
  if (blockIdx.x == 0 && threadIdx.x == 0) stamp(plan, STAMP_UPLOAD_BEGIN);
  const uint32_t epoch = st->epoch;
  const uint32_t par = epoch & 1u;
  const float4* wm = at<const float4>(me, f.lay.work_master_off);
  const float4* gm = at<const float4>(me, f.lay.global_off);
  float4* um = at<float4>(me, f.lay.upload_master_off[par]);
  uint2* us = at<uint2>(me, f.lay.upload_shadow_off[par]);
  const long long nv = f.lay.n_params / 4;
  const long long tid = blockIdx.x * static_cast<long long>(blockDim.x) + threadIdx.x;
  const long long stride = static_cast<long long>(gridDim.x) * blockDim.x;
  for (long long i = tid; i < nv; i += stride) {
    float4 w = wm[i];
    if (byz_mode == 1) {
      const float4 g = gm[i];
      w.x = g.x - byz_scale * (w.x - g.x);
      w.y = g.y - byz_scale * (w.y - g.y);
      w.z = g.z - byz_scale * (w.z - g.z);
      w.w = g.w - byz_scale * (w.w - g.w);
    }
    um[i] = w;
    us[i] = make_uint2(pack_bf16x2(w.x, w.y), pack_bf16x2(w.z, w.w));
  }
  __syncthreads();
  __shared__ bool last;
  if (threadIdx.x == 0) {
    __threadfence_system();
    const unsigned done = atomicAdd(&plan->upload_blocks_done, 1u);
    last = (done == gridDim.x - 1);
  }
  __syncthreads();
  if (!last) return;
  __threadfence_system();
  __shared__ int ticket;
  if (threadIdx.x == 0) {
    admit::straggle(straggle_us);
    ticket = admit::first_k(st) ? admit::take_ticket(&admit::page(f.peers.base[0], f.lay, par)->ticket, epoch) : 0;
    if (ticket >= static_cast<int>(st->n_needed) && admit::first_k(st)) ticket = -1;
  }
  __syncthreads();
  if (ticket >= 0 && threadIdx.x < f.n_ranks) {
    const int r = threadIdx.x;
    UploadMeta* meta = at<UploadMeta>(f.peers.base[r], f.lay.meta_off) + par * kMaxRanks + f.rank;
    UploadMeta m;
    m.n_samples = static_cast<uint32_t>(n_samples);
    m.avg_cost = plan->loss_sum / static_cast<float>(n_loss_terms > 0 ? n_loss_terms : 1);
    *meta = m;
    __threadfence_system();
    if (admit::first_k(st))
      ptx::st_release_sys(&admit::page(f.peers.base[r], f.lay, par)->slot[ticket],
                          ((epoch + 1u) << 8) | static_cast<uint32_t>(f.rank));
    ptx::st_release_sys(at<uint32_t>(f.peers.base[r], f.lay.flags_off) + FLAG_TRAINED + f.rank,
                        epoch + 1);
  }
  __syncthreads();
  if (threadIdx.x == 0) stamp(plan, STAMP_UPLOAD_END);
}

struct ConsShared {
  ConsensusIn<kMaxRanks> in;
  ConsensusOut<kMaxRanks> out;
  int sel_rank[kMaxRanks];
  float sel_w[kMaxRanks];
  int n_sel;
};

__device__ __forceinline__ unsigned long long digest_term(float v, long long idx) {
  return static_cast<unsigned long long>(__float_as_uint(v)) *
         (static_cast<unsigned long long>(2 * idx + 1) * 0x9E3779B97F4A7C15ull);
}

struct DpShared {
  float s[kMaxRanks];
  float norm[kMaxRanks];
  float scale[kMaxRanks];
  float sigma;
  uint32_t clipped;
};

template <bool kRobust, int kServerOpt, int kDp>
__device__ __forceinline__ void consensus_body(FedArgs f, int n_val, int weight_by_score, int two_shot, int use_mc,
                                               uint32_t* host_mirror, uint32_t* bump_seq, uint32_t agg,
                                               ServerOptArgs so, DpArgs dp, DpShared* dsh) {
  __shared__ ConsShared sh;
  __shared__ bool last;
  ptx::pdl_launch_dependents();
  ptx::pdl_wait();
  char* me = f.peers.base[f.rank];
  RoundState* st = at<RoundState>(me, f.lay.state_off);
  RoundPlan* plan = at<RoundPlan>(me, f.lay.plan_off);
  uint32_t* flags = at<uint32_t>(me, f.lay.flags_off);
  const uint32_t epoch = st->epoch;
  const uint32_t par = epoch & 1u;
  const int n = f.n_ranks;
  const bool i_am_comm = (st->role[f.rank] & ROLE_COMM) != 0;
  if (blockIdx.x == 0 && threadIdx.x == 0) stamp(plan, STAMP_CONS_BEGIN);

  const bool fk = admit::first_k(st);
  __shared__ int cand_of[kMaxRanks];
  __shared__ uint32_t adm_mask;
  if (threadIdx.x == 0) {
    uint32_t m = 0;
    for (int z = 0; z < plan->n_cand; ++z) {
      cand_of[z] = fk ? admit::wait_slot(admit::page(me, f.lay, par), z, epoch) : plan->cand_rank[z];
      m |= 1u << cand_of[z];
    }
    adm_mask = m;
  }
  __syncthreads();

  if (blockIdx.x == 0 && i_am_comm) {
    if (threadIdx.x < n) {
      const int r = threadIdx.x;
      float* row = at<float>(f.peers.base[r], f.lay.scores_off) +
                   (par * kMaxRanks + f.rank) * kMaxRanks;
      for (int z = 0; z < plan->n_cand; ++z)
        row[cand_of[z]] =
            static_cast<float>(plan->correct[z]) / static_cast<float>(n_val > 0 ? n_val : 1);
      ptx::st_release_sys(at<uint32_t>(f.peers.base[r], f.lay.flags_off) + FLAG_SCORED + f.rank,
                          epoch + 1);
    }
  }

  if (threadIdx.x < n) {
    const int r = threadIdx.x;
    if (st->role[r] & ROLE_COMM) ptx::wait_flag_ge(flags + FLAG_SCORED + r, epoch + 1);
    if ((st->role[r] & ROLE_TRAINER) && ((adm_mask >> r) & 1u)) ptx::wait_flag_ge(flags + FLAG_TRAINED + r, epoch + 1);
  }
  __syncthreads();
  if (blockIdx.x == 0 && threadIdx.x == 0) stamp(plan, STAMP_CONS_SCORED);

  {
    ConsensusIn<kMaxRanks>& in = sh.in;
    const float* rows = at<float>(me, f.lay.scores_off) + par * kMaxRanks * kMaxRanks;
    const UploadMeta* meta = at<UploadMeta>(me, f.lay.meta_off) + par * kMaxRanks;
    const int i = threadIdx.x;
    if (i < kMaxRanks * kMaxRanks) {
      const int r = i / kMaxRanks, t = i % kMaxRanks;
      const bool ok = r < n && t < n && (st->role[r] & ROLE_COMM) && (st->role[t] & ROLE_TRAINER) &&
                      ((adm_mask >> t) & 1u);
      in.scored[r][t] = ok ? 1 : 0;
      in.score[r][t] =
          ok ? __uint_as_float(ptx::ld_relaxed_sys(reinterpret_cast<const uint32_t*>(rows + r * kMaxRanks + t))) : 0.f;
    } else if (i < kMaxRanks * kMaxRanks + kMaxRanks) {
      const int r = i - kMaxRanks * kMaxRanks;
      in.role[r] = r < n ? st->role[r] : 0u;
      in.admitted[r] = (r < n && (st->role[r] & ROLE_TRAINER) && ((adm_mask >> r) & 1u)) ? 1 : 0;
      in.n_samples[r] = r < n ? ptx::ld_relaxed_sys(&meta[r].n_samples) : 0u;
      in.avg_cost[r] =
          r < n ? __uint_as_float(ptx::ld_relaxed_sys(reinterpret_cast<const uint32_t*>(&meta[r].avg_cost))) : 0.f;
    }
  }
  __syncthreads();
  if (threadIdx.x == 0) {
    ConsensusIn<kMaxRanks>& in = sh.in;
    in.n_ranks = n;
    in.n_comm = static_cast<int>(st->n_comm);
    in.n_aggregate = static_cast<int>(st->n_aggregate);
    in.weight_by_score = weight_by_score;
    run_consensus<kMaxRanks>(in, sh.out);
    int k = 0;
    for (int r = 0; r < n; ++r)
      if (sh.out.selected[r]) {
        sh.sel_rank[k] = r;
        sh.sel_w[k] = sh.out.weight[r];
        ++k;
      }
    sh.n_sel = k;
  }
  __syncthreads();
  if constexpr (kDp != DP_OFF) {
    if (threadIdx.x < n) ptx::wait_flag_ge(flags + FLAG_NORM + threadIdx.x, epoch + 1);
    __syncthreads();
    if (threadIdx.x == 0) {
      const volatile double* part = at<const double>(me, dp.off + offsetof(DpPage, partial)) + par * kMaxRanks * kMaxRanks;
      for (int t = 0; t < kMaxRanks; ++t) {
        float nrm = __uint_as_float(0x7FC00000u), sc = nrm;
        if (sh.in.admitted[t]) {
          double sum = 0.0;
          for (int q = 0; q < n; ++q) sum += part[q * kMaxRanks + t];
          nrm = dp_norm(sum);
          sc = dp_scale(nrm, dp.clip);
        }
        dsh->norm[t] = nrm;
        dsh->scale[t] = sc;
      }
      uint32_t clipped = 0, wmax = 0;
      for (int k = 0; k < sh.n_sel; ++k) {
        const float sc = dsh->scale[sh.sel_rank[k]];
        dsh->s[k] = sc;
        if (dp_bits(sc) != 0x3F800000u) clipped |= 1u << k;
        const uint32_t wb = dp_bits(sh.sel_w[k]);
        wmax = wb > wmax ? wb : wmax;
      }
      dsh->clipped = clipped;
      dsh->sigma = kDp == DP_NOISE && sh.n_sel > 0 ? so_mul(so_mul(dp.noise, dp.clip), dp_float(wmax)) : 0.f;
    }
    __syncthreads();
  }

  const int n_sel = sh.n_sel;
  const int trim = agg_trim(static_cast<int>(agg & 0xFFu), static_cast<int>((agg >> 8) & 0xFFu), n_sel);
  const float4* src[kMaxRanks];
  float w[kMaxRanks];
#pragma unroll
  for (int k = 0; k < kMaxRanks; ++k) {
    const int r = k < n_sel ? sh.sel_rank[k] : f.rank;
    src[k] = at<const float4>(f.peers.base[r], f.lay.upload_master_off[par]);
    w[k] = k < n_sel ? sh.sel_w[k] : 0.f;
  }
  const long long nv = f.lay.n_params / 4;
  long long lo = 0, hi = nv;
  if (two_shot) {
    long long per = (nv + n - 1) / n;
    per += per & 1;
    lo = per * f.rank;
    hi = lo + per < nv ? lo + per : nv;
    if (lo > nv) lo = nv;
  }
  float4* g_f32 = at<float4>(me, f.lay.global_off);
  uint2* g_b16 = at<uint2>(me, f.lay.global_shadow_off);
  float4* w_f32 = at<float4>(me, f.lay.work_master_off);
  uint2* w_b16 = at<uint2>(me, f.lay.work_shadow_off);
  const bool mc = two_shot && use_mc && f.peers.mc_base != nullptr;
  float4* s_m = at<float4>(me, so.m_off);
  float4* s_v = at<float4>(me, so.v_off);
  unsigned long long dig = 0ull;
  const long long tid = blockIdx.x * static_cast<long long>(blockDim.x) + threadIdx.x;
  const long long stride = static_cast<long long>(gridDim.x) * blockDim.x;
  for (long long i = lo + tid; i < hi; i += stride) {
    float4 acc = make_float4(0.f, 0.f, 0.f, 0.f);
    if (n_sel == 0) {
      acc = g_f32[i];
    } else {
      float4 v[kMaxRanks];
#pragma unroll
      for (int k = 0; k < kMaxRanks; ++k)
        if (k < n_sel) v[k] = ptx::ld_peer_f4(src[k] + i);
      if constexpr (kDp != DP_OFF) {
        const float4 g = g_f32[i];
        const uint32_t clipped = dsh->clipped;
#pragma unroll
        for (int k = 0; k < kMaxRanks; ++k)
          if (k < n_sel && ((clipped >> k) & 1u)) {
            const float s = dsh->s[k];
            v[k].x = dp_clip_value(g.x, v[k].x, s);
            v[k].y = dp_clip_value(g.y, v[k].y, s);
            v[k].z = dp_clip_value(g.z, v[k].z, s);
            v[k].w = dp_clip_value(g.w, v[k].w, s);
          }
      }
      if constexpr (kRobust) {
        float c[kMaxRanks];
#pragma unroll
        for (int k = 0; k < kMaxRanks; ++k) c[k] = v[k].x;
        acc.x = robust_combine<kMaxRanks>(c, n_sel, trim);
#pragma unroll
        for (int k = 0; k < kMaxRanks; ++k) c[k] = v[k].y;
        acc.y = robust_combine<kMaxRanks>(c, n_sel, trim);
#pragma unroll
        for (int k = 0; k < kMaxRanks; ++k) c[k] = v[k].z;
        acc.z = robust_combine<kMaxRanks>(c, n_sel, trim);
#pragma unroll
        for (int k = 0; k < kMaxRanks; ++k) c[k] = v[k].w;
        acc.w = robust_combine<kMaxRanks>(c, n_sel, trim);
      } else {
#pragma unroll
        for (int k = 0; k < kMaxRanks; ++k)
          if (k < n_sel) {
            acc.x = fmaf(w[k], v[k].x, acc.x);
            acc.y = fmaf(w[k], v[k].y, acc.y);
            acc.z = fmaf(w[k], v[k].z, acc.z);
            acc.w = fmaf(w[k], v[k].w, acc.w);
          }
      }
      if constexpr (kDp == DP_NOISE) {
        float z[4];
        dp_gauss4(dp.seed, epoch, static_cast<uint64_t>(i), z);
        const float sigma = dsh->sigma;
        acc.x = so_add(acc.x, so_mul(sigma, z[0]));
        acc.y = so_add(acc.y, so_mul(sigma, z[1]));
        acc.z = so_add(acc.z, so_mul(sigma, z[2]));
        acc.w = so_add(acc.w, so_mul(sigma, z[3]));
      }
      if constexpr (kServerOpt != SOPT_NONE) {
        const ServerOptParams p{so.lr, so.b1, so.b2, so.c1, so.c2, so.tau};
        const float4 g = g_f32[i];
        float4 m = s_m[i];
        float4 v = make_float4(0.f, 0.f, 0.f, 0.f);
        if constexpr (kServerOpt != SOPT_MOMENTUM) v = s_v[i];
        acc.x = server_step(kServerOpt, g.x, acc.x, m.x, v.x, p);
        acc.y = server_step(kServerOpt, g.y, acc.y, m.y, v.y, p);
        acc.z = server_step(kServerOpt, g.z, acc.z, m.z, v.z, p);
        acc.w = server_step(kServerOpt, g.w, acc.w, m.w, v.w, p);
        s_m[i] = m;
        if constexpr (kServerOpt != SOPT_MOMENTUM) s_v[i] = v;
      }
    }
    dig += digest_term(acc.x, 4 * i) + digest_term(acc.y, 4 * i + 1) +
           digest_term(acc.z, 4 * i + 2) + digest_term(acc.w, 4 * i + 3);
    const uint2 b = make_uint2(pack_bf16x2(acc.x, acc.y), pack_bf16x2(acc.z, acc.w));
    if (!two_shot) {
      g_f32[i] = acc; g_b16[i] = b; w_f32[i] = acc; w_b16[i] = b;
    } else if (mc) {
      ptx::multimem_st_f4(at<float4>(f.peers.mc_base, f.lay.global_off) + i, acc);
      ptx::multimem_st_f4(at<float4>(f.peers.mc_base, f.lay.work_master_off) + i, acc);
      const unsigned am = __activemask();
      const uint32_t ox = __shfl_down_sync(am, b.x, 1), oy = __shfl_down_sync(am, b.y, 1);
      if ((i & 1) == 0) {
        const float4 pk = make_float4(__uint_as_float(b.x), __uint_as_float(b.y), __uint_as_float(ox),
                                      __uint_as_float(oy));
        ptx::multimem_st_f4(at<float4>(f.peers.mc_base, f.lay.global_shadow_off) + (i >> 1), pk);
        ptx::multimem_st_f4(at<float4>(f.peers.mc_base, f.lay.work_shadow_off) + (i >> 1), pk);
      }
    } else {
      for (int r = 0; r < n; ++r) {
        char* pb = f.peers.base[r];
        at<float4>(pb, f.lay.global_off)[i] = acc;
        at<uint2>(pb, f.lay.global_shadow_off)[i] = b;
        at<float4>(pb, f.lay.work_master_off)[i] = acc;
        at<uint2>(pb, f.lay.work_shadow_off)[i] = b;
      }
    }
  }
#pragma unroll
  for (int off = 16; off >= 1; off >>= 1) dig += __shfl_xor_sync(0xffffffffu, dig, off);
  if ((threadIdx.x & 31) == 0 && dig) atomicAdd(&plan->digest_acc, dig);

  __syncthreads();
  if (threadIdx.x == 0) {
    __threadfence_system();
    const unsigned done = atomicAdd(&plan->consensus_blocks_done, 1u);
    last = (done == gridDim.x - 1);
  }
  __syncthreads();
  if (!last) return;
  __threadfence_system();

  if (two_shot) {
    if (threadIdx.x < n) {
      const int r = threadIdx.x;
      unsigned long long* slot =
          reinterpret_cast<unsigned long long*>(at<float>(f.peers.base[r], f.lay.scores_off) +
                                                2 * kMaxRanks * kMaxRanks) +
          par * kMaxRanks + f.rank;
      *slot = *reinterpret_cast<volatile unsigned long long*>(&plan->digest_acc);
      __threadfence_system();
      ptx::st_release_sys(at<uint32_t>(f.peers.base[r], f.lay.flags_off) + FLAG_SLICE + f.rank,
                          epoch + 1);
    }
    __syncthreads();
    if (threadIdx.x < n) ptx::wait_flag_ge(flags + FLAG_SLICE + threadIdx.x, epoch + 1);
    __syncthreads();
  }

  if (threadIdx.x == 0) {
    unsigned long long digest = 0ull;
    if (two_shot) {
      const unsigned long long* slots =
          reinterpret_cast<const unsigned long long*>(at<float>(me, f.lay.scores_off) +
                                                      2 * kMaxRanks * kMaxRanks) +
          par * kMaxRanks;
      for (int r = 0; r < n; ++r)
        digest += *reinterpret_cast<const volatile unsigned long long*>(slots + r);
    } else {
      digest = *reinterpret_cast<volatile unsigned long long*>(&plan->digest_acc);
    }
    const ConsensusIn<kMaxRanks>& in = sh.in;
    const ConsensusOut<kMaxRanks>& out = sh.out;
    BlockRecord* rec =
        at<BlockRecord>(me, f.lay.ring_off) + (epoch % static_cast<uint32_t>(f.lay.ring_slots));
    rec->epoch = epoch;
    rec->n_ranks = static_cast<uint32_t>(n);
    rec->n_comm = st->n_comm;
    rec->n_aggregate = st->n_aggregate;
    uint32_t adm = 0, sel = 0;
    for (int r = 0; r < kMaxRanks; ++r) {
      rec->role_before[r] = in.role[r];
      rec->role_after[r] = r < n ? out.role_after[r] : 0u;
      uint32_t m = 0;
      for (int t = 0; t < kMaxRanks; ++t) {
        rec->score_rows[r][t] = in.score[r][t];
        if (in.scored[r][t]) m |= 1u << t;
      }
      rec->scored_mask[r] = m;
      rec->median[r] = r < n ? out.median[r] : 0.f;
      rec->n_samples[r] = in.n_samples[r];
      rec->avg_cost[r] = in.avg_cost[r];
      rec->weight[r] = r < n ? out.weight[r] : 0.f;
      if (in.admitted[r]) adm |= 1u << r;
      if (r < n && out.selected[r]) sel |= 1u << r;
    }
    rec->admitted_mask = adm;
    rec->selected_mask = sel;
    rec->global_loss = out.global_loss;
    rec->weight_by_score = static_cast<uint32_t>(weight_by_score);
    rec->model_digest = digest;
    rec->agg = agg;
    __threadfence();
    rec->seq = epoch + 1;
    for (int r = 0; r < n; ++r) {
      st->role[r] = out.role_after[r];
      st->last_median[r] = out.median[r];
    }
    st->selected_mask = sel;
    st->global_loss = out.global_loss;
    st->model_digest = digest;
    st->blocks_appended = st->blocks_appended + 1;
    st->epoch = epoch + 1;
    if constexpr (kDp != DP_OFF) {
      DpPage* page = at<DpPage>(me, dp.off);
      for (int t = 0; t < kMaxRanks; ++t) {
        page->norm[t] = dsh->norm[t];
        page->scale[t] = dsh->scale[t];
      }
      page->sigma = dsh->sigma;
      page->epoch = epoch + 1;
    }
    __threadfence_system();
  }
  __syncthreads();
  if (bump_seq != nullptr && threadIdx.x == 0) *bump_seq = *bump_seq + 1u;
  if (host_mirror != nullptr) {
    constexpr int kWords = static_cast<int>(sizeof(RoundState) / 4);
    const volatile uint32_t* src = reinterpret_cast<const volatile uint32_t*>(st);
    for (int i = threadIdx.x; i < kWords; i += blockDim.x)
      asm volatile("st.relaxed.sys.global.u32 [%0], %1;" ::"l"(host_mirror + i), "r"(src[i]) : "memory");
    __threadfence_system();
    __syncthreads();
    if (threadIdx.x == 0) ptx::st_release_sys(host_mirror + kMirrorSeqWord, epoch + 1);
  }
  if (threadIdx.x < n)
    ptx::st_release_sys(
        at<uint32_t>(f.peers.base[threadIdx.x], f.lay.flags_off) + FLAG_DONE + f.rank, epoch + 1);
  if (threadIdx.x == 0) stamp(plan, STAMP_CONS_END);
}

template <bool kRobust, int kServerOpt>
__global__ void __launch_bounds__(kFedThreads)
k_consensus(FedArgs f, int n_val, int weight_by_score, int two_shot, int use_mc,
            uint32_t* host_mirror, uint32_t* bump_seq, uint32_t agg, ServerOptArgs so) {
  consensus_body<kRobust, kServerOpt, DP_OFF>(f, n_val, weight_by_score, two_shot, use_mc, host_mirror, bump_seq,
                                               agg, so, DpArgs{}, nullptr);
}

template <bool kRobust, int kServerOpt, int kDp>
__global__ void __launch_bounds__(kFedThreads)
k_consensus_dp(FedArgs f, int n_val, int weight_by_score, int two_shot, int use_mc,
               uint32_t* host_mirror, uint32_t* bump_seq, uint32_t agg, ServerOptArgs so, DpArgs dp) {
  __shared__ DpShared dsh;
  consensus_body<kRobust, kServerOpt, kDp>(f, n_val, weight_by_score, two_shot, use_mc, host_mirror, bump_seq,
                                           agg, so, dp, &dsh);
}

__global__ void __launch_bounds__(kFedThreads) k_update_norms(FedArgs f, long long dp_off) {
  ptx::pdl_launch_dependents();
  ptx::pdl_wait();
  char* me = f.peers.base[f.rank];
  const RoundState* st = at<RoundState>(me, f.lay.state_off);
  const RoundPlan* plan = at<RoundPlan>(me, f.lay.plan_off);
  const uint32_t* flags = at<uint32_t>(me, f.lay.flags_off);
  DpPage* page = at<DpPage>(me, dp_off);
  const uint32_t epoch = st->epoch;
  const uint32_t par = epoch & 1u;
  const int n = f.n_ranks;
  __shared__ int cand_of[kMaxRanks];
  __shared__ int n_cand;
  __shared__ bool last;
  __shared__ double warp_part[kFedThreads / 32][kMaxRanks];
  if (threadIdx.x == 0) {
    const bool fk = admit::first_k(st);
    const int nc = plan->n_cand;
    for (int z = 0; z < nc; ++z) {
      const int t = fk ? admit::wait_slot(admit::page(me, f.lay, par), z, epoch) : plan->cand_rank[z];
      ptx::wait_flag_ge(flags + FLAG_TRAINED + t, epoch + 1);
      cand_of[z] = t;
    }
    n_cand = nc;
  }
  __syncthreads();
  const int nc = n_cand;
  const float4* src[kMaxRanks];
#pragma unroll
  for (int z = 0; z < kMaxRanks; ++z)
    src[z] = at<const float4>(f.peers.base[z < nc ? cand_of[z] : f.rank], f.lay.upload_master_off[par]);
  const float4* g = at<const float4>(me, f.lay.global_off);
  const long long nv = f.lay.n_params / 4;
  const long long per = (nv + n - 1) / n;
  const long long lo = per * f.rank < nv ? per * f.rank : nv;
  const long long hi = lo + per < nv ? lo + per : nv;
  double acc[kMaxRanks];
#pragma unroll
  for (int z = 0; z < kMaxRanks; ++z) acc[z] = 0.0;
  const long long stride = static_cast<long long>(gridDim.x) * blockDim.x;
  for (long long i = lo + blockIdx.x * static_cast<long long>(blockDim.x) + threadIdx.x; i < hi; i += stride) {
    const float4 gv = g[i];
    float4 u[kMaxRanks];
#pragma unroll
    for (int z = 0; z < kMaxRanks; ++z)
      if (z < nc) u[z] = ptx::ld_peer_f4(src[z] + i);
#pragma unroll
    for (int z = 0; z < kMaxRanks; ++z)
      if (z < nc) {
        const double dx = so_sub(u[z].x, gv.x), dy = so_sub(u[z].y, gv.y);
        const double dz = so_sub(u[z].z, gv.z), dw = so_sub(u[z].w, gv.w);
        acc[z] += dx * dx;
        acc[z] += dy * dy;
        acc[z] += dz * dz;
        acc[z] += dw * dw;
      }
  }
  const int lane = threadIdx.x & 31, warp = threadIdx.x >> 5;
#pragma unroll
  for (int z = 0; z < kMaxRanks; ++z) {
#pragma unroll
    for (int o = 16; o >= 1; o >>= 1) acc[z] += __shfl_xor_sync(0xffffffffu, acc[z], o);
    if (lane == 0) warp_part[warp][z] = acc[z];
  }
  __syncthreads();
  if (threadIdx.x < kMaxRanks) {
    double s = 0.0;
    for (int w = 0; w < kFedThreads / 32; ++w) s += warp_part[w][threadIdx.x];
    page->block[blockIdx.x][threadIdx.x] = s;
    __threadfence();
  }
  __syncthreads();
  if (threadIdx.x == 0) {
    const unsigned done = atomicAdd(&page->ticket, 1u);
    last = (done == gridDim.x - 1);
  }
  __syncthreads();
  if (!last) return;
  __threadfence();
  if (threadIdx.x < nc) {
    const int z = threadIdx.x;
    const volatile double* blk = &page->block[0][0];
    double s = 0.0;
    for (unsigned b = 0; b < gridDim.x; ++b) s += blk[b * kMaxRanks + z];
    for (int r = 0; r < n; ++r)
      at<DpPage>(f.peers.base[r], dp_off)->partial[par][f.rank][cand_of[z]] = s;
  }
  __syncthreads();
  if (threadIdx.x == 0) page->ticket = 0u;
  if (threadIdx.x < n) {
    __threadfence_system();
    ptx::st_release_sys(at<uint32_t>(f.peers.base[threadIdx.x], f.lay.flags_off) + FLAG_NORM + f.rank, epoch + 1);
  }
}

__global__ void k_p2p_read(const float4* __restrict__ src, float4* __restrict__ dst, long long n) {
  const long long tid = blockIdx.x * static_cast<long long>(blockDim.x) + threadIdx.x;
  const long long stride = static_cast<long long>(gridDim.x) * blockDim.x;
  for (long long i = tid; i + 3 * stride < n; i += 4 * stride) {
    const float4 a = ptx::ld_peer_f4(src + i);
    const float4 b = ptx::ld_peer_f4(src + i + stride);
    const float4 c = ptx::ld_peer_f4(src + i + 2 * stride);
    const float4 d = ptx::ld_peer_f4(src + i + 3 * stride);
    dst[i] = a; dst[i + stride] = b; dst[i + 2 * stride] = c; dst[i + 3 * stride] = d;
  }
}
__global__ void k_mc_store(float4* mc_dst, const float4* __restrict__ src, long long n) {
  const long long tid = blockIdx.x * static_cast<long long>(blockDim.x) + threadIdx.x;
  const long long stride = static_cast<long long>(gridDim.x) * blockDim.x;
  for (long long i = tid; i < n; i += stride) ptx::multimem_st_f4(mc_dst + i, src[i]);
}

__global__ void k_wait_trained(FedArgs f) {
  char* me = f.peers.base[f.rank];
  const RoundState* st = at<RoundState>(me, f.lay.state_off);
  const uint32_t* flags = at<uint32_t>(me, f.lay.flags_off);
  const int r = threadIdx.x;
  if (r < f.n_ranks && (st->role[r] & ROLE_TRAINER))
    ptx::wait_flag_ge(flags + FLAG_TRAINED + r, st->epoch + 1);
}

__global__ void __launch_bounds__(256)
k_pull(FedArgs f, uint4* stage_shadow, float4* stage_master, const long long* ranges, int n_ranges) {
  ptx::pdl_launch_dependents();
  ptx::pdl_wait();
  char* me = f.peers.base[f.rank];
  const RoundState* st = at<RoundState>(me, f.lay.state_off);
  RoundPlan* plan = at<RoundPlan>(me, f.lay.plan_off);
  if (!(st->role[f.rank] & ROLE_COMM)) return;
  const int z = blockIdx.y;
  if (z >= plan->n_cand) return;
  if (blockIdx.x == 0 && z == 0 && threadIdx.x == 0) stamp(plan, STAMP_PULL_BEGIN);
  const uint32_t epoch = st->epoch;
  const uint32_t par = epoch & 1u;
  __shared__ int t_sh;
  if (threadIdx.x == 0) {
    const int tt = admit::first_k(st) ? admit::wait_slot(admit::page(me, f.lay, par), z, epoch) : plan->cand_rank[z];
    ptx::wait_flag_ge(at<uint32_t>(me, f.lay.flags_off) + FLAG_TRAINED + tt, epoch + 1);
    t_sh = tt;
  }
  __syncthreads();
  const int t = t_sh;
  const long long tid = blockIdx.x * static_cast<long long>(blockDim.x) + threadIdx.x;
  const long long stride = static_cast<long long>(gridDim.x) * blockDim.x;
  {
    const long long nv = f.lay.n_params / 8;
    const uint4* src = at<const uint4>(f.peers.base[t], f.lay.upload_shadow_off[par]);
    uint4* dst = stage_shadow + static_cast<long long>(z) * nv;
    const float4* s4 = reinterpret_cast<const float4*>(src);
    float4* d4 = reinterpret_cast<float4*>(dst);
    long long i = tid;
    for (; i + 3 * stride < nv; i += 4 * stride) {
      const float4 a = ptx::ld_peer_f4(s4 + i), b = ptx::ld_peer_f4(s4 + i + stride);
      const float4 c = ptx::ld_peer_f4(s4 + i + 2 * stride), d = ptx::ld_peer_f4(s4 + i + 3 * stride);
      d4[i] = a; d4[i + stride] = b; d4[i + 2 * stride] = c; d4[i + 3 * stride] = d;
    }
    for (; i < nv; i += stride) d4[i] = ptx::ld_peer_f4(s4 + i);
  }
  if (stage_master != nullptr) {
    const long long nv = f.lay.n_params / 4;
    const float4* src = at<const float4>(f.peers.base[t], f.lay.upload_master_off[par]);
    float4* dst = stage_master + static_cast<long long>(z) * nv;
    if (ranges == nullptr) {
      for (long long i = tid; i < nv; i += stride) dst[i] = ptx::ld_peer_f4(src + i);
    } else {
      for (int r = blockIdx.x; r < n_ranges; r += gridDim.x) {
        const long long o = ranges[2 * r], n4 = ranges[2 * r + 1];
        for (long long i = threadIdx.x; i < n4; i += blockDim.x) dst[o + i] = ptx::ld_peer_f4(src + o + i);
      }
    }
  }
  __syncthreads();
  if (threadIdx.x == 0) stamp(plan, STAMP_PULL_END);
}

__global__ void __launch_bounds__(256)
k_pull_blob(FedArgs f, long long off0, long long off1, Mx8Unpack un, uint8_t* stage_blob, long long blob_bytes,
            __nv_bfloat16* stage_dq, long long stage_stride) {
  ptx::pdl_launch_dependents();
  ptx::pdl_wait();
  char* me = f.peers.base[f.rank];
  const RoundState* st = at<RoundState>(me, f.lay.state_off);
  RoundPlan* plan = at<RoundPlan>(me, f.lay.plan_off);
  if (!(st->role[f.rank] & ROLE_COMM)) return;
  const int z = blockIdx.y;
  if (z >= plan->n_cand) return;
  if (blockIdx.x == 0 && z == 0 && threadIdx.x == 0) stamp(plan, STAMP_PULL_BEGIN);
  const uint32_t epoch = st->epoch;
  __shared__ int t_sh;
  if (threadIdx.x == 0) {
    const int tt = admit::first_k(st) ? admit::wait_slot(admit::page(me, f.lay, epoch & 1u), z, epoch)
                                      : plan->cand_rank[z];
    ptx::wait_flag_ge(at<uint32_t>(me, f.lay.flags_off) + FLAG_TRAINED + tt, epoch + 1);
    t_sh = tt;
  }
  __syncthreads();
  const int t = t_sh;
  const uint8_t* src = at<const uint8_t>(f.peers.base[t], (epoch & 1u) ? off1 : off0);
  uint8_t* dblob = stage_blob + static_cast<long long>(z) * blob_bytes;
  __nv_bfloat16* ddq = stage_dq + static_cast<long long>(z) * stage_stride;
  const long long n = epi::mx8_unpack_units(un);
  const long long stride = static_cast<long long>(gridDim.x) * blockDim.x;
  for (long long i = blockIdx.x * static_cast<long long>(blockDim.x) + threadIdx.x; i < n; i += stride)
    epi::mx8_unpack_unit(un, src, ddq, dblob, i);
  __syncthreads();
  if (threadIdx.x == 0) stamp(plan, STAMP_PULL_END);
}

int fed_grid(long long n_params) {
  long long blocks = (n_params / 4 + kFedThreads * 2 - 1) / (kFedThreads * 2);
  if (blocks > 132 * 4) blocks = 132 * 4;
  if (blocks < 1) blocks = 1;
  return static_cast<int>(blocks);
}

}

cudaError_t fed_plan_round(const FedArgs& f, const PlanLayer* layers, int n_layers,
                           int steps_per_round, int staged, cudaStream_t s, const PlanBlobs* blobs,
                           const float* stage_master) {
  if (n_layers > kMaxPlanLayers) return cudaErrorInvalidValue;
  PlanLayers pl{};
  pl.n = n_layers;
  pl.steps_per_round = steps_per_round;
  pl.staged = staged;
  pl.stage_master = stage_master;
  if (blobs != nullptr) {
    pl.use_blob = 1;
    pl.stage_blob = blobs->stage; pl.blob_bytes = blobs->bytes;
    pl.upq_off[0] = blobs->upq_off[0]; pl.upq_off[1] = blobs->upq_off[1];
  }
  for (int i = 0; i < n_layers; ++i) pl.l[i] = layers[i];
  note_launch();
  return launch_pdl(k_plan, dim3(1), dim3(32), 0, s, f, pl);
}

cudaError_t fed_upload(const FedArgs& f, int n_samples, int n_loss_terms, int byz_mode,
                       float byz_scale, cudaStream_t s, int straggle_us) {
  note_launch();
  return launch_pdl(k_upload, dim3(fed_grid(f.lay.n_params)), dim3(kFedThreads), 0, s, f, n_samples,
                    n_loss_terms, byz_mode, byz_scale, straggle_us);
}

template <bool kRobust>
static cudaError_t launch_consensus(int opt, dim3 grid, dim3 block, cudaStream_t s, const FedArgs& f, int n_val,
                                    int weight_by_score, int two_shot, int use_multicast, uint32_t* host_mirror,
                                    uint32_t* bump_seq, uint32_t agg, const ServerOptArgs& so) {
  switch (opt) {
    case SOPT_MOMENTUM:
      return launch_pdl(k_consensus<kRobust, SOPT_MOMENTUM>, grid, block, 0, s, f, n_val, weight_by_score, two_shot,
                        use_multicast, host_mirror, bump_seq, agg, so);
    case SOPT_ADAM:
      return launch_pdl(k_consensus<kRobust, SOPT_ADAM>, grid, block, 0, s, f, n_val, weight_by_score, two_shot,
                        use_multicast, host_mirror, bump_seq, agg, so);
    case SOPT_YOGI:
      return launch_pdl(k_consensus<kRobust, SOPT_YOGI>, grid, block, 0, s, f, n_val, weight_by_score, two_shot,
                        use_multicast, host_mirror, bump_seq, agg, so);
    default:
      return launch_pdl(k_consensus<kRobust, SOPT_NONE>, grid, block, 0, s, f, n_val, weight_by_score, two_shot,
                        use_multicast, host_mirror, bump_seq, agg, so);
  }
}

template <bool kRobust, int kDp>
static cudaError_t launch_consensus_dp(int opt, dim3 grid, dim3 block, cudaStream_t s, const FedArgs& f, int n_val,
                                       int weight_by_score, int two_shot, int use_multicast, uint32_t* host_mirror,
                                       uint32_t* bump_seq, uint32_t agg, const ServerOptArgs& so, const DpArgs& dp) {
  switch (opt) {
    case SOPT_MOMENTUM:
      return launch_pdl(k_consensus_dp<kRobust, SOPT_MOMENTUM, kDp>, grid, block, 0, s, f, n_val, weight_by_score,
                        two_shot, use_multicast, host_mirror, bump_seq, agg, so, dp);
    case SOPT_ADAM:
      return launch_pdl(k_consensus_dp<kRobust, SOPT_ADAM, kDp>, grid, block, 0, s, f, n_val, weight_by_score,
                        two_shot, use_multicast, host_mirror, bump_seq, agg, so, dp);
    case SOPT_YOGI:
      return launch_pdl(k_consensus_dp<kRobust, SOPT_YOGI, kDp>, grid, block, 0, s, f, n_val, weight_by_score,
                        two_shot, use_multicast, host_mirror, bump_seq, agg, so, dp);
    default:
      return launch_pdl(k_consensus_dp<kRobust, SOPT_NONE, kDp>, grid, block, 0, s, f, n_val, weight_by_score,
                        two_shot, use_multicast, host_mirror, bump_seq, agg, so, dp);
  }
}

static bool dp_off_ok(long long off) { return off > 0 && off % 16 == 0; }

cudaError_t fed_update_norms(const FedArgs& f, long long dp_off, cudaStream_t s) {
  if (!dp_off_ok(dp_off) || f.n_ranks < 1) return cudaErrorInvalidValue;
  note_launch();
  return launch_pdl(k_update_norms, dim3(fed_grid(f.lay.n_params / f.n_ranks)), dim3(kFedThreads), 0, s, f, dp_off);
}

cudaError_t fed_consensus_aggregate(const FedArgs& f, int n_val, int weight_by_score,
                                    int two_shot, int use_multicast, cudaStream_t s,
                                    uint32_t* host_mirror, uint32_t* bump_seq, int rule, int trim,
                                    const ServerOptArgs* so, const DpArgs* dp) {
  if (!agg_rule_valid(rule, trim) || (rule != AGG_FEDAVG && weight_by_score)) return cudaErrorInvalidValue;
  ServerOptArgs sa{};
  if (so != nullptr) sa = *so;
  if (*server_opt_check(sa.opt, sa.lr, sa.b1, sa.b2, sa.tau) != '\0') return cudaErrorInvalidValue;
  if (sa.opt != SOPT_NONE) {
    const bool need_v = server_state_vectors(sa.opt) == 2;
    if (sa.m_off <= 0 || sa.m_off % 16 != 0 || (need_v && (sa.v_off <= 0 || sa.v_off % 16 != 0)))
      return cudaErrorInvalidValue;
  }
  DpArgs da{};
  if (dp != nullptr) da = *dp;
  if (*dp_check(da.mode, da.clip, da.noise, rule) != '\0' || (da.mode != DP_OFF && !dp_off_ok(da.off)))
    return cudaErrorInvalidValue;
  const long long work = two_shot ? f.lay.n_params / (f.n_ranks > 0 ? f.n_ranks : 1)
                                  : f.lay.n_params;
  note_launch();
  const dim3 grid(fed_grid(work)), block(kFedThreads);
  const uint32_t agg = agg_word(rule, trim, sa.opt, da.mode);
  if (da.mode == DP_CLIP && rule == AGG_FEDAVG)
    return launch_consensus_dp<false, DP_CLIP>(sa.opt, grid, block, s, f, n_val, weight_by_score, two_shot,
                                               use_multicast, host_mirror, bump_seq, agg, sa, da);
  if (da.mode == DP_CLIP)
    return launch_consensus_dp<true, DP_CLIP>(sa.opt, grid, block, s, f, n_val, weight_by_score, two_shot,
                                              use_multicast, host_mirror, bump_seq, agg, sa, da);
  if (da.mode == DP_NOISE)
    return launch_consensus_dp<false, DP_NOISE>(sa.opt, grid, block, s, f, n_val, weight_by_score, two_shot,
                                                use_multicast, host_mirror, bump_seq, agg, sa, da);
  if (rule == AGG_FEDAVG)
    return launch_consensus<false>(sa.opt, grid, block, s, f, n_val, weight_by_score, two_shot, use_multicast,
                                   host_mirror, bump_seq, agg, sa);
  return launch_consensus<true>(sa.opt, grid, block, s, f, n_val, weight_by_score, two_shot, use_multicast,
                                host_mirror, bump_seq, agg, sa);
}

cudaError_t fed_pull_candidates(const FedArgs& f, void* stage_shadow, float* stage_master,
                                cudaStream_t s, const long long* ranges, int n_ranges) {
  long long blocks = (f.lay.n_params / 8 + 256 * 4 - 1) / (256 * 4);
  if (blocks > 74) blocks = 74;
  if (blocks < 1) blocks = 1;
  note_launch();
  return launch_pdl(k_pull, dim3(static_cast<unsigned>(blocks), kMaxRanks), dim3(256), 0, s, f,
                    reinterpret_cast<uint4*>(stage_shadow),
                    reinterpret_cast<float4*>(stage_master), ranges, n_ranges);
}

cudaError_t fed_pull_blobs(const FedArgs& f, long long off0, long long off1, const Mx8Unpack& un,
                           void* stage_blob, long long blob_bytes, void* stage_dq, long long stage_stride,
                           cudaStream_t s) {
  if (un.in_dim % 16 != 0 || un.hidden % 32 != 0 || un.b1 + 4LL * un.hidden + 256 > blob_bytes) return cudaErrorInvalidValue;
  long long blocks = (epi::mx8_unpack_units(un) + 256 * 2 - 1) / (256 * 2);
  if (blocks > 18) blocks = 18;
  if (blocks < 1) blocks = 1;
  note_launch();
  return launch_pdl(k_pull_blob, dim3(static_cast<unsigned>(blocks), kMaxRanks), dim3(256), 0, s, f, off0, off1, un,
                    static_cast<uint8_t*>(stage_blob), blob_bytes, static_cast<__nv_bfloat16*>(stage_dq),
                    stage_stride);
}

cudaError_t fed_wait_trained(const FedArgs& f, cudaStream_t s) {
  (void)cudaGetLastError();
  k_wait_trained<<<1, 32, 0, s>>>(f);
  note_launch();
  return cudaGetLastError();
}

cudaError_t p2p_read_probe(const float4* peer_src, float4* local_dst, int64_t n_vec,
                           cudaStream_t s) {
  k_p2p_read<<<132 * 4, 256, 0, s>>>(peer_src, local_dst, n_vec);
  note_launch();
  return cudaGetLastError();
}
cudaError_t mc_store_probe(float4* mc_dst, const float4* local_src, int64_t n_vec,
                           cudaStream_t s) {
  k_mc_store<<<132 * 4, 256, 0, s>>>(mc_dst, local_src, n_vec);
  note_launch();
  return cudaGetLastError();
}

}
```

### bflc_demo_b200/csrc/kernels/mlp_val_sm100.cu

```cuda
#include <cuda_bf16.h>

#include <cstring>

#include "bflc_kernels.h"
#include "epi_common.cuh"
#include "launch.cuh"
#include "sm100_ptx.cuh"
#include "wgmma.cuh"

namespace bflc {

namespace {

__device__ __forceinline__ uint32_t pack2(float a, float b) { return epi::pack_bf16x2(a, b); }

constexpr int kEpiWarps = 8;
constexpr int kProducerWarp = kEpiWarps;
constexpr int kThreads = kEpiWarps * 32 + 32;
constexpr int kChainH = 256;
constexpr int kBarBytes = 512;
constexpr int kBiasFloats = 320;
constexpr int kBM = 64;
constexpr int kStages = 6;
constexpr int kA = kBM * 128, kB = 128 * 128, kStage = kA + kB;
constexpr int kHalf = 2 * kBM * 128;
constexpr int kOffH = kStages * kStage;
constexpr int kOffW2K = kOffH + 2 * kHalf;
constexpr int kOffBar = kOffW2K + 32768;
constexpr int kValSmem = kOffBar + kBarBytes + kBiasFloats * 4 + 1024;
static_assert(kValSmem <= 227 * 1024, "shared memory budget");

struct ValArgs {
  int n_val, in_dim, n_classes;
  const CUtensorMap* maps;
  const GemmDynamic* dyn1; const GemmDynamic* dyn2;
  const int32_t* labels; unsigned int* correct;
  const int* pred;
  const uint8_t* const* cand_blob; Mx8MlpLayout ql;
};

template <int R>
__device__ __forceinline__ void run_sync(float (&d)[R]) {
  wg::commit();
  wg::wait<0>();
  wg::reg_fence(d);
}

__device__ __forceinline__ void load_biases(float* sb, const ValArgs& v, const uint8_t* blob, int z, bool with_b2) {
  const int et = threadIdx.x;
  const float* b1 = blob != nullptr ? reinterpret_cast<const float*>(blob + v.ql.b1) : v.dyn1->bias[z];
  sb[et] = b1 != nullptr ? b1[et] : 0.f;
  if (with_b2 && et < 64) {
    const float* b2 = blob != nullptr ? reinterpret_cast<const float*>(blob + v.ql.b2) : v.dyn2->bias[z];
    sb[kChainH + et] = (b2 != nullptr && et < v.n_classes) ? b2[et] : 0.f;
  }
}

__device__ __forceinline__ void score_rows(const float (&lg)[32], const float* sb, const ValArgs& v, int z,
                                           int m0, int r0) {
  const int lane = threadIdx.x & 31, C = v.n_classes;
  unsigned hits = 0;
#pragma unroll
  for (int e = 0; e < 2; ++e) {
    float vmax = -INFINITY;
    int amax = 0x7fffffff;
#pragma unroll
    for (int i = 0; i < 32; ++i) {
      if (((i >> 1) & 1) != e) continue;
      const int n = wg::frag_col(i, lane);
      const float x = lg[i] + sb[kChainH + n];
      if (n < C && (x > vmax || (x == vmax && n < amax))) { vmax = x; amax = n; }
    }
#pragma unroll
    for (int off = 1; off <= 2; off <<= 1) {
      const float ov = __shfl_xor_sync(0xffffffffu, vmax, off);
      const int oi = __shfl_xor_sync(0xffffffffu, amax, off);
      if (ov > vmax || (ov == vmax && oi < amax)) { vmax = ov; amax = oi; }
    }
    const int row = m0 + r0 + 8 * e;
    const bool hit = (lane & 3) == 0 && row < v.n_val && amax == v.labels[row];
    hits += __popc(__ballot_sync(0xffffffffu, hit));
  }
  if (lane == 0 && hits) atomicAdd(v.correct + z, hits);
}

__global__ void __launch_bounds__(kThreads, 1)
mlp_val_pair_kernel(const __grid_constant__ CUtensorMap tmX, const __grid_constant__ ValArgs v) {
  extern __shared__ uint8_t smem_raw[];
  uint8_t* smem = reinterpret_cast<uint8_t*>(
      (reinterpret_cast<uintptr_t>(smem_raw) + 1023) & ~static_cast<uintptr_t>(1023));
  uint64_t* full = reinterpret_cast<uint64_t*>(smem + kOffBar);
  uint64_t* empty = full + kStages;
  uint64_t* w2k = empty + kStages;
  uint64_t* hx = w2k + 1;
  float* sb = reinterpret_cast<float*>(smem + kOffBar + kBarBytes);

  ptx::pdl_launch_dependents();
  const int warp = threadIdx.x >> 5, lane = threadIdx.x & 31;
  const uint32_t rank = blockIdx.x & 1;
  const bool leader = rank == 0;
  const int z = blockIdx.y, m0 = (blockIdx.x >> 1) * kBM;
  if (threadIdx.x == 0) {
    ptx::tma_prefetch_desc(&tmX);
    for (int s = 0; s < kStages; ++s) {
      ptx::mbar_init(&full[s], 1);
      ptx::mbar_init(&empty[s], kEpiWarps * 32);
    }
    ptx::mbar_init(w2k, 1);
    ptx::mbar_init(hx, 1);
    if (leader) ptx::mbar_expect_tx(hx, kHalf);
    ptx::fence_mbar_init();
  }
  ptx::cluster_sync();
  ptx::pdl_wait();
  const bool inactive = (v.pred != nullptr && *v.pred == 0) || z >= v.dyn1->active_batches;
  if (inactive) return;
  const int kb_d = (v.in_dim + 63) / 64;
  const uint8_t* blob = v.cand_blob != nullptr ? v.cand_blob[z] : nullptr;

  if (warp == kProducerWarp) {
    if (v.dyn1->wait_flag[z] != nullptr) {
      if (lane == 0) ptx::wait_flag_ge(v.dyn1->wait_flag[z], v.dyn1->wait_value);
      __syncwarp();
    }
    const CUtensorMap* m1 = v.maps + v.dyn1->map_index[z];
    const CUtensorMap* m2 = v.maps + v.dyn2->map_index[z];
    if (leader && ptx::elect_one()) {
      ptx::mbar_expect_tx(w2k, 32768);
#pragma unroll
      for (int kb = 0; kb < 4; ++kb) ptx::tma_load_3d(smem + kOffW2K + kb * 8192, m2, w2k, kb * 64, 0, 0);
    }
    __syncwarp();
    for (int i = 0; i < kb_d; ++i) {
      const int s = i % kStages;
      const uint32_t ph = (i / kStages) & 1;
      ptx::mbar_wait(&empty[s], ph ^ 1);
      if (ptx::elect_one()) {
        uint8_t* sa = smem + s * kStage;
        ptx::mbar_expect_tx(&full[s], kStage);
        ptx::tma_load_3d(sa, &tmX, &full[s], i * 64, m0, 0);
        ptx::tma_load_3d(sa + kA, m1, &full[s], i * 64, 128 * rank, 0);
      }
      __syncwarp();
    }
  } else if (warp < kEpiWarps) {
    const int g = warp >> 2, r0 = 16 * (warp & 3) + (lane >> 2);
    load_biases(sb, v, blob, z, leader);
    const uint32_t base = ptx::smem_u32(smem);
    float acc[32];
    wg::zero(acc);
    for (int i = 0; i < kb_d; ++i) {
      const int s = i % kStages;
      const uint32_t ph = (i / kStages) & 1;
      ptx::mbar_wait(&full[s], ph);
      const uint32_t sa = base + static_cast<uint32_t>(s) * kStage, sbw = sa + kA + g * 8192u;
      wg::fence();
#pragma unroll
      for (uint32_t k = 0; k < 4; ++k)
        wg::mma_bf16<64, 0, 0>(acc, wg::desc(sa + k * 32u, 16), wg::desc(sbw + k * 32u, 16),
                               (i > 0 || k > 0) ? 1u : 0u);
      wg::commit();
      wg::wait<1>();
      if (i > 0) ptx::mbar_arrive(&empty[(i - 1) % kStages]);
    }
    wg::wait<0>();
    wg::reg_fence(acc);
    asm volatile("bar.sync 1, 256;" ::: "memory");
    {
      const int c0 = 128 * static_cast<int>(rank) + 64 * g;
      uint8_t* tile = smem + kOffH + (c0 >> 6) * 8192;
#pragma unroll
      for (int i = 0; i < 32; i += 2) {
        const int row = r0 + 8 * ((i >> 1) & 1), col = wg::frag_col(i, lane);
        *reinterpret_cast<uint32_t*>(tile + row * 128 + (((col >> 3) ^ (row & 7)) << 4) + (col & 7) * 2) =
            pack2(fmaxf(acc[i] + sb[c0 + col], 0.f), fmaxf(acc[i + 1] + sb[c0 + col + 1], 0.f));
      }
    }
    ptx::fence_proxy_async_smem();
    asm volatile("bar.sync 1, 256;" ::: "memory");
    if (!leader) {
      if (threadIdx.x == 0) {
        uint8_t* half = smem + kOffH + kHalf;
        ptx::bulk_s2cluster(ptx::mapa(ptx::smem_u32(half), 0), half, kHalf, ptx::mapa(ptx::smem_u32(hx), 0));
      }
    } else if (g == 0) {
      ptx::mbar_wait(hx, 0);
      ptx::mbar_wait(w2k, 0);
      float lg[32];
      wg::zero(lg);
      const uint32_t ha = base + kOffH, wb = base + kOffW2K;
      wg::fence();
#pragma unroll
      for (int kb = 0; kb < 4; ++kb)
#pragma unroll
        for (uint32_t k = 0; k < 4; ++k)
          wg::mma_bf16<64, 0, 0>(lg, wg::desc(ha + kb * 8192u + k * 32u, 16), wg::desc(wb + kb * 8192u + k * 32u, 16),
                                 (kb > 0 || k > 0) ? 1u : 0u);
      run_sync(lg);
      score_rows(lg, sb, v, z, m0, r0);
    }
  }
  __syncwarp();
  ptx::cluster_sync();
}

}

cudaError_t mlp_val_sm100(const MlpValArgs& r, cudaStream_t stream) {
  bind_context_once();
  if (r.hidden != kChainH || r.n_classes > 64 || r.in_dim % 8 || r.n_val <= 0 || r.max_cand <= 0)
    return cudaErrorInvalidValue;
  if (r.fp8 && r.cand_blob == nullptr) return cudaErrorInvalidValue;
  CUtensorMap tx;
  GemmOperand op{r.x, r.ldx, 0, false};
  cudaError_t e = gemm_make_operand_map(&tx, op, DType::BF16, r.n_val, r.in_dim, 1, kBM);
  if (e != cudaSuccess) return e;
  ValArgs v{};
  v.n_val = r.n_val; v.in_dim = r.in_dim; v.n_classes = r.n_classes;
  v.maps = r.maps; v.dyn1 = r.dyn1; v.dyn2 = r.dyn2;
  v.labels = r.labels; v.correct = r.correct;
  v.pred = r.pred ? r.pred : current_predicate();
  v.ql = mx8_mlp_layout(r.in_dim, r.hidden);
  if (r.fp8) v.cand_blob = r.cand_blob;
  static bool configured = false;
  if (!configured) {
    e = cudaFuncSetAttribute(mlp_val_pair_kernel, cudaFuncAttributeMaxDynamicSharedMemorySize, kValSmem);
    if (e != cudaSuccess) return e;
    configured = true;
  }
  note_launch();
  const dim3 grid(2 * ((r.n_val + kBM - 1) / kBM), r.max_cand);
  return launch_pdl_cluster(2u, mlp_val_pair_kernel, grid, dim3(kThreads), kValSmem, stream, tx, v);
}

}
```

### bflc_demo_b200/engine/base.py

```python
from __future__ import annotations

import struct
from typing import List, Optional, Tuple

import numpy as np
import torch
import torch.distributed as dist

from .._native import C, ledger as _ledger
from ..config import FLConfig
from ..data.synthetic import Shard
from ..parallel.layout import HeapLayout
from ..parallel.symm import SymmetricHeap

ROLE_TRAINER, ROLE_COMM = 1, 2


def step_rows(i: int, batch: int, epoch_rows: int) -> slice:
    j = (i % (epoch_rows // batch)) * batch
    return slice(j, j + batch)


def initial_roles(cfg: FLConfig) -> List[int]:
    n = cfg.clients
    if cfg.solo:
        return [ROLE_TRAINER | ROLE_COMM] * n
    ids = list(range(n))
    if cfg.seed:
        rng = np.random.default_rng(cfg.seed)
        rng.shuffle(ids)
    roles = [ROLE_TRAINER] * n
    for i in ids[: cfg.committee_size]:
        roles[i] = ROLE_COMM
    return roles


def resolve_dp_seed(cfg: FLConfig, rank: int, world: int, group) -> int:
    if cfg.dp_mode != 2:
        return 0
    if cfg.dp_seed is not None:
        return int(cfg.dp_seed)
    import secrets
    box = [secrets.randbits(64) if rank == 0 else None]
    if world > 1:
        dist.broadcast_object_list(box, src=0, group=group)
    return int(box[0])


def vector_ranges(spec) -> torch.Tensor:
    runs = []
    for e in spec.entries:
        if len(e.shape) != 1:
            continue
        lo, hi = e.offset // 4, (e.offset + e.shape[0] + 3) // 4
        if runs and runs[-1][1] >= lo:
            runs[-1][1] = max(runs[-1][1], hi)
        else:
            runs.append([lo, hi])
    return torch.tensor([[lo, hi - lo] for lo, hi in runs], dtype=torch.int64).reshape(-1, 2)


ROUND_STATE = struct.Struct("<4I8I8fIfQII")


def parse_round_state(buf, world: int) -> dict:
    f = ROUND_STATE.unpack_from(buf, 0)
    return dict(epoch=f[0], roles=list(f[4:4 + world]), median=list(f[12:12 + world]), selected_mask=f[20],
                global_loss=f[21], model_digest=f[22])


BLOCK_RECORD_FIELDS = (
    ("epoch", 1, "I"), ("n_ranks", 1, "I"), ("n_comm", 1, "I"), ("n_aggregate", 1, "I"),
    ("role_before", 8, "I"), ("role_after", 8, "I"), ("score_rows", 8 * 8, "f"), ("scored_mask", 8, "I"),
    ("median", 8, "f"), ("n_samples", 8, "I"), ("avg_cost", 8, "f"), ("weight", 8, "f"),
    ("admitted_mask", 1, "I"), ("selected_mask", 1, "I"), ("global_loss", 1, "f"), ("weight_by_score", 1, "I"),
    ("model_digest", 1, "Q"), ("seq", 1, "I"), ("agg", 1, "I"))
BLOCK_RECORD = struct.Struct("<" + "".join(f"{n}{code}" for _, n, code in BLOCK_RECORD_FIELDS))


def parse_block_record(buf, offset: int, world: int) -> Tuple[int, int, dict]:
    flat, f, i = BLOCK_RECORD.unpack_from(buf, offset), {}, 0
    for name, n, _ in BLOCK_RECORD_FIELDS:
        f[name] = flat[i] if n == 1 else list(flat[i:i + n])
        i += n
    w = world
    return f["epoch"], f["seq"], dict(
        epoch=f["epoch"], role_before=f["role_before"][:w], role_after=f["role_after"][:w],
        score_rows=[f["score_rows"][8 * c:8 * c + w] for c in range(w)],
        scored_mask=f["scored_mask"][:w], n_samples=f["n_samples"][:w], avg_cost=f["avg_cost"][:w],
        admitted_mask=f["admitted_mask"], selected_mask=f["selected_mask"], global_loss=f["global_loss"],
        model_digest=f["model_digest"], weight_by_score=f["weight_by_score"], agg=f["agg"])


def drain_ring(host_ledger, ring, drained: int, epoch: int, world: int) -> Tuple[int, List[str]]:
    rs = BLOCK_RECORD.size
    slots = len(ring) // rs
    errs = []
    while drained < epoch:
        got, seq, rnd = parse_block_record(ring, (drained % slots) * rs, world)
        if got != drained or seq != drained + 1:
            errs.append(f"ring slot for epoch {drained} holds epoch {got} seq {seq}")
            break
        msg = host_ledger.AppendDeviceRound(rnd)
        if msg:
            errs.append(f"epoch {drained}: {msg}")
            break
        drained += 1
    return drained, errs


class ProtocolEngine:

    def __init__(self, cfg: FLConfig, spec, shard: Shard, init_, *, rank: int, world: int, device: int,
                 group, extra_bytes: int = 0):
        self.cfg, self.rank, self.world, self.device, self.group = cfg, rank, world, device, group
        torch.cuda.set_device(device)
        self.dev = torch.device("cuda", device)
        self.mod = C()
        self.sz = sz = self.mod.struct_sizes()
        assert (sz["RoundState"], sz["BlockRecord"]) == (ROUND_STATE.size, BLOCK_RECORD.size), \
            "RoundState / BlockRecord layout changed: update engine/base.py"
        self.spec = spec
        P = self.n_params = spec.total
        B = cfg.batch_size
        self.S = (len(shard) // B) * B
        self.steps = (self.S // B) * cfg.local_epochs
        self.n_val = min(cfg.val_samples or len(shard), len(shard))
        self.n_val_targets = int(shard.y[: self.n_val].numel())

        self.layout = HeapLayout(P, cfg.ring_slots, extra_bytes=extra_bytes,
                                 server_state=cfg.server_state_vectors, dp=cfg.dp_mode > 0)
        self.heap = SymmetricHeap(self.layout.total_bytes, rank=rank, world=world, device=device,
                                  group=group, want_multicast=cfg.use_multicast)
        self.fed = self.layout.fed_dict(rank, world, self.heap.peer_ptrs, self.heap.mc_ptr)
        self.multicast = cfg.use_multicast and self.heap.has_multicast
        o, hv = self.layout.offsets, self.heap.view
        self.work_master = hv(o["work_master"], [P], torch.float32)
        self.work_shadow = hv(o["work_shadow"], [P], torch.bfloat16)
        self.global_master = hv(o["global"], [P], torch.float32)
        self.global_shadow = hv(o["global_shadow"], [P], torch.bfloat16)
        self.state_bytes = hv(o["state"], [sz["RoundState"]], torch.uint8)
        self.plan_bytes = hv(o["plan"], [sz["RoundPlan"]], torch.uint8)
        self.ring_bytes = hv(o["ring"], [cfg.ring_slots * sz["BlockRecord"]], torch.uint8)
        self.plan_ptr = self.heap.local_ptr + o["plan"]
        self.loss_sum = hv(o["plan"] + sz["plan_loss_sum_off"], [1], torch.float32)
        self.val_correct = hv(o["plan"] + sz["plan_correct_off"], [sz["kMaxRanks"]], torch.int32)
        self.grad = torch.zeros(P, device=self.dev, dtype=torch.float32)

        init = torch.empty(P, dtype=torch.float32)
        init_(init, seed=cfg.seed + 1234)
        for t in (self.work_master, self.global_master):
            t.copy_(init)
        for t in (self.work_shadow, self.global_shadow):
            t.copy_(init.to(torch.bfloat16))
        self.server_state = [hv(o[k], [P], torch.float32) for k in ("server_m", "server_v")[: cfg.server_state_vectors]]
        for t in self.server_state:
            t.zero_()
        self.server_kw = self.layout.server_opt_kwargs(cfg.server_opt_id, cfg.server_opt_constants)
        self.dp_seed = resolve_dp_seed(cfg, rank, world, group)
        clip, noise = cfg.dp_constants
        self.dp_kw = self.layout.dp_kwargs(cfg.dp_mode, clip, noise, self.dp_seed)
        self.dp_page = hv(o["dp"], [sz["DpPage"]], torch.uint8) if cfg.dp_mode > 0 else None
        if self.dp_page is not None:
            self.dp_page.zero_()

        roles = initial_roles(cfg)
        st = self.mod.state_init_bytes(world, cfg.committee_size, cfg.aggregate_count, roles,
                                       cfg.needed_updates)
        self.state_bytes.copy_(torch.frombuffer(bytearray(st), dtype=torch.uint8))
        self.host_ledger = _ledger().Ledger(self.ledger_config())
        self.host_ledger.Bootstrap(roles)
        self.drained = 0
        self._rounds = 0
        self._drain_every = max(cfg.ring_slots // 2, 1)

        self.byz = 1 if rank in cfg.byzantine_ranks else 0
        self.straggle_us = cfg.straggler_delay_us if rank in cfg.straggler_ranks else 0
        self.staged = bool(cfg.stage_candidates) and world > 1

    def _next_round(self):
        self._rounds += 1
        if self._rounds - self.drained >= self._drain_every:
            errs = self.drain_blocks()
            if errs:
                raise RuntimeError(f"host/device ledgers disagree: {errs[:2]}")

    def _consensus(self, mirror_ptr: int = 0, seq_ptr: int = 0):
        m, cfg = self.mod, self.cfg
        if self.dp_kw:
            m.fed_update_norms(self.fed, self.layout.offsets["dp"])
        m.fed_consensus_aggregate(self.fed, self.n_val_targets, cfg.weight_by_score, self.two_shot, self.multicast,
                                  mirror_ptr, seq_ptr, cfg.aggregation_rule, cfg.trim,
                                  **self.server_kw, **self.dp_kw)

    @property
    def consensus_captured(self) -> bool:
        return False

    def read_state(self, buf: Optional[torch.Tensor] = None) -> dict:
        return parse_round_state((self.state_bytes.cpu() if buf is None else buf).numpy(), self.world)

    def drain_blocks(self) -> List[str]:
        torch.cuda.synchronize()
        epoch = self.read_state()["epoch"]
        self.drained, errs = drain_ring(self.host_ledger, self.ring_bytes.cpu().numpy(), self.drained, epoch,
                                        self.world)
        return errs

    def read_stamps(self) -> dict:
        torch.cuda.synchronize()
        raw = bytes(self.plan_bytes.cpu().numpy())
        t = struct.unpack_from("<8Q", raw, self.sz["plan_stamps_off"])

        def d(a, b):
            return (t[b] - t[a]) / 1e3 if t[a] and t[b] and t[b] >= t[a] else 0.0
        out = dict(train_us=d(0, 1) if t[1] else 0.0, upload_us=d(1, 2), pull_us=d(3, 4),
                   validate_us=d(4, 5) if t[4] else (d(2, 5) if t[2] else 0.0),
                   consensus_wait_us=d(5, 6),
                   aggregate_publish_us=d(6, 7), round_us=d(0, 7))
        out["exposed_comm_us"] = max(out["round_us"] - out["train_us"] - out["validate_us"], 0.0)
        return out

    def ledger_config(self):
        lc = self.cfg.to_ledger_config(self.n_params)
        lc.dp_seed = self.dp_seed
        return lc

    def last_update_norms(self) -> Optional[np.ndarray]:
        if self.dp_page is None:
            return None
        torch.cuda.synchronize()
        off = self.sz["dp_norm_off"]
        return self.dp_page[off:off + 4 * self.world].cpu().numpy().view(np.float32).copy()

    def privacy_spent(self) -> tuple:
        from ..protocol.privacy import epsilon
        if self.cfg.dp_mode != 2:
            return float("inf"), self.cfg.dp_delta
        rounds = int(self.read_state()["epoch"])
        return epsilon(float(self.cfg.dp_constants[1]), rounds, self.cfg.dp_delta), self.cfg.dp_delta
```

### bflc_demo_b200/engine/fused.py

```python
from __future__ import annotations

import os
import time
import weakref
from typing import Dict, List, Optional

import torch
import torch.distributed as dist

from .._native import C
from ..config import FLConfig
from ..data.synthetic import Shard
from ..models.mlp import FlatMLP, mlp_spec
from ..ops import gemm as G
from .base import ROUND_STATE as _ROUND_STATE
from .base import ProtocolEngine, parse_round_state, vector_ranges


class FusedEngine(ProtocolEngine):
    def __init__(self, cfg: FLConfig, shard: Shard, *, rank: int = 0, world: int = 1,
                 device: int = 0, group=None, in_dim: Optional[int] = None):
        assert cfg.clients == world, "one client per rank"
        assert world <= 8
        if cfg.lora_rank:
            raise ValueError("FusedEngine trains the MLP in full: LoRA (lora_rank > 0) needs GenericFedEngine "
                             "with a bert or gpt LoRANet")
        if cfg.has_optim_recipe:
            raise ValueError("FusedEngine's persistent trainer has no weight decay, lr schedule or gradient "
                             "clipping: run the model through GenericFedEngine for the optimizer recipe")

        x0 = shard.x.reshape(len(shard), -1)
        self.in_dim = in_dim or x0.shape[1]
        spec = mlp_spec(self.in_dim, cfg.hidden, shard.n_classes)
        self.fp8 = cfg.dtype == "fp8"
        if self.fp8 and not (cfg.hidden == 256 and shard.n_classes <= 64 and cfg.fused_step
                             and cfg.batch_size % 128 == 0 and self.in_dim % 16 == 0
                             and len(shard) % 128 == 0):
            raise ValueError("dtype='fp8' (MXFP8) needs hidden == 256, <= 64 classes, batch % 128 == 0, "
                             "in_dim % 16 == 0, shard rows % 128 == 0 and the fused step")
        self.ql = C().mx8_mlp_layout(self.in_dim, cfg.hidden) if self.fp8 else None
        self.blob_bytes = (self.ql["total"] + 4095) // 4096 * 4096 if self.fp8 else 0
        super().__init__(cfg, spec, shard, spec.init_, rank=rank, world=world, device=device, group=group,
                         extra_bytes=2 * self.blob_bytes)
        sz, o, hv, P = self.sz, self.layout.offsets, self.heap.view, self.n_params
        plan_ptr = self.plan_ptr
        self.is_trainer_ptr = plan_ptr + sz["plan_is_trainer_off"]
        self.is_comm_ptr = plan_ptr + sz["plan_is_comm_off"]
        self.train_correct = hv(o["plan"] + sz["plan_train_correct_off"], [1], torch.int32)

        self.trainer = FlatMLP(self.spec, self.work_master, self.work_shadow, self.grad,
                               cfg.batch_size, optimizer=cfg.optimizer, lr=cfg.learning_rate,
                               loss_sum=self.loss_sum, correct=self.train_correct,
                               step_dev_ptr=plan_ptr + sz["plan_opt_step_off"], fp8=self.fp8,
                               prox_mu=cfg.prox_mu, anchor=self.global_master)
        for par in (0, 1):
            hv(o[f"upload_master{par}"], [P], torch.float32).copy_(self.global_master)
            hv(o[f"upload_shadow{par}"], [P], torch.bfloat16).copy_(self.global_shadow)
        self.upq_off = [o["extra"], o["extra"] + self.blob_bytes] if self.fp8 else []
        if self.fp8:
            for off in self.upq_off:
                self.trainer.quantize_weights(self.global_master, hv(off, [self.blob_bytes], torch.uint8))
            self.trainer.quantize_weights()

        self.x_u8 = torch.empty(len(shard), self.in_dim, device=self.dev, dtype=torch.uint8)
        self.x_bf = torch.empty(len(shard), self.in_dim, device=self.dev, dtype=torch.bfloat16)
        self.x_dq = (torch.empty(len(shard), self.in_dim, device=self.dev, dtype=torch.bfloat16)
                     if self.fp8 else None)
        self.y = torch.empty(len(shard), device=self.dev, dtype=torch.int32)
        self.host_x = x0.contiguous().pin_memory()
        self.host_y = shard.y.to(torch.int32).contiguous().pin_memory()
        self.x_u8.copy_(self.host_x)
        self.y.copy_(self.host_y)
        self.h_val = torch.empty(world, self.n_val, cfg.hidden, device=self.dev, dtype=torch.bfloat16)
        self.out_host = torch.empty(sz["RoundState"], dtype=torch.uint8).pin_memory()

        K = sz["kMaxRanks"]
        e1, e2 = self.spec.by_name["w1"], self.spec.by_name["w2"]
        self.val_bn = [self.mod.gemm_pick_bn(e1.shape[0], G.EPI_GENERIC, self.n_val, world),
                       self.mod.gemm_pick_bn(e2.shape[0], G.EPI_ARGMAX, self.n_val, world)]
        self.val_chain = cfg.hidden == 256 and e2.shape[0] <= 64
        if self.val_chain:
            self.val_bn = [128, 64]
        self.first_k = (not cfg.solo) and cfg.needed_updates < cfg.n_trainers
        if self.first_k and not self.staged:
            raise ValueError("needed_updates < trainers (first-K-wins admission) needs stage_candidates=True")
        self.cand_shadow = torch.zeros(world, P, device=self.dev, dtype=torch.bfloat16)
        self.cand_q = (torch.zeros(world, self.blob_bytes, device=self.dev, dtype=torch.uint8)
                       if self.fp8 else None)
        self.cand_master = self.cand_ranges = None
        if self.staged and not self.fp8:
            self.cand_master = torch.zeros(world, P, device=self.dev, dtype=torch.float32)
            self.cand_ranges = vector_ranges(self.spec).to(self.dev)
        blob = bytearray(2 * 2 * K * 128)

        def b_map(base, e, kind, layer):
            return self.mod.gemm_b_map(base + e.offset * 2, e.shape[0], e.shape[1], e.shape[1], False,
                                       False, kind, self.val_bn[layer])

        for layer, (e, kind) in enumerate(((e1, G.EPI_GENERIC), (e2, G.EPI_ARGMAX))):
            if self.staged:
                for zslot in range(world):
                    base = self.cand_shadow.data_ptr() + zslot * P * 2
                    idx = layer * K + zslot
                    blob[idx * 128:(idx + 1) * 128] = b_map(base, e, kind, layer)
                continue
            for par in range(2):
                for r in range(world):
                    base = self.heap.peer_ptrs[r] + o[f"upload_shadow{par}"]
                    idx = (layer * 2 + par) * K + r
                    blob[idx * 128:(idx + 1) * 128] = b_map(base, e, kind, layer)
        self.b_maps = torch.frombuffer(blob, dtype=torch.uint8).to(self.dev)
        self._w_offs = [e1.offset, e2.offset]
        self.plan_layers = [(self.spec.offset("b1"), True), (self.spec.offset("b2"), True)]
        self.dyn_ptr = [plan_ptr + sz["plan_dyn_off"] + i * sz["GemmDynamic"] for i in range(2)]
        self.two_shot = (cfg.two_shot if cfg.two_shot is not None
                         else world > 1 and (P * 4 > (64 << 20) or world >= 8))
        self.fused_step = bool(cfg.fused_step) and self.trainer.fused_ok(self.steps)
        self.fused_upload = self.fused_step and os.environ.get("BFLC_MLP_EPIOPT", "1") != "0"
        if self.fp8 and not (self.fused_step and self.fused_upload):
            raise ValueError("dtype='fp8' needs the persistent trainer with the optimizer epilogue")
        self.graph: Optional[torch.cuda.CUDAGraph] = None
        self.graph_pipe: Optional[torch.cuda.CUDAGraph] = None
        self._exec: Dict[int, int] = {}
        self.stream = torch.cuda.Stream(device=self.dev)
        self._side = torch.cuda.Stream(device=self.dev)
        self._side2 = torch.cuda.Stream(device=self.dev)
        self._ev_fork, self._ev_join = torch.cuda.Event(), torch.cuda.Event()
        self.epoch_steps = self.S // cfg.batch_size
        self.pipelined_input = (self.fused_step and self.S == len(shard) and self.epoch_steps <= 16
                                and (cfg.batch_size * self.in_dim) % 16 == 0
                                and os.environ.get("BFLC_INPUT_PIPELINE", "1") != "0"
                                and os.environ.get("BFLC_MLP_CHAIN", "3") != "1")
        self.mirror = torch.zeros(128, dtype=torch.int32).pin_memory()
        self._mirror_np = self.mirror.numpy()
        self._epoch_known: Optional[int] = None
        self.mirror_result = os.environ.get("BFLC_RESULT_MIRROR", "1") != "0"
        self.in_flags = torch.zeros(16, device=self.dev, dtype=torch.int32)
        self.in_seq = torch.zeros(1, device=self.dev, dtype=torch.int32)
        self.cast_cnt = torch.zeros(16, device=self.dev, dtype=torch.int32)
        self.x_ready = torch.zeros(16, device=self.dev, dtype=torch.int32)
        self.in_err = torch.zeros(1, device=self.dev, dtype=torch.int32)
        self._ev_wq = torch.cuda.Event()
        self.seq_host = torch.zeros(1, dtype=torch.int32).pin_memory()
        self._seq_np = self.seq_host.numpy()
        self._seq = 0
        self._copy_stream = torch.cuda.Stream(device=self.dev)
        self._pipe_dst, self._pipe_y = self.x_u8.data_ptr(), self.y.data_ptr()
        self._pipe_chunk = self.cfg.batch_size * self.in_dim
        self._pipe_flags = (self.in_flags.data_ptr(), self.seq_host.data_ptr(), self._copy_stream.cuda_stream)
        self._prefeed = os.environ.get("BFLC_E2E_PREFEED", "1") == "1"
        self._host_checked: Dict[int, weakref.ref] = {}
        self._tag_wv = os.environ.get("BFLC_E2E_TAGS", "writevalue") != "memcpy"
        self.launches_per_round = 0
        if world > 1:
            dist.barrier(group=group)
        torch.cuda.synchronize()

    def _enqueue_round(self, pipe: bool = False):
        m, cfg = self.mod, self.cfg
        pipe = pipe and self.pipelined_input
        n0 = m.launch_count()
        main = torch.cuda.current_stream()
        self._ev_fork.record(main)
        self._side.wait_event(self._ev_fork)
        B = cfg.batch_size
        if self.fp8:
            self._side2.wait_event(self._ev_fork)
            with torch.cuda.stream(self._side2):
                self.trainer.quantize_weights()
                self._ev_wq.record(self._side2)
        with torch.cuda.stream(self._side):
            if pipe:
                m.prep_inputs_chunks(self.x_u8, self.x_bf, None, None, B, self.epoch_steps,
                                     1.0 / 255.0, self.in_flags, self.in_seq, self.cast_cnt,
                                     self.x_ready, self.in_err, self.x_dq)
            else:
                m.prep_inputs(self.x_u8, self.x_bf, None, None, 1.0 / 255.0, self.x_dq)
            self._ev_join.record(self._side)
        if self.fp8:
            m.fed_plan_round(self.fed, self.plan_layers, self.steps, self.staged,
                             self.cand_q.data_ptr(), self.blob_bytes, self.upq_off)
        else:
            m.fed_plan_round(self.fed, self.plan_layers, self.steps, self.staged,
                             stage_master_ptr=self.cand_master.data_ptr() if self.cand_master is not None else 0)
        if not pipe:
            main.wait_event(self._ev_join)
        if self.fp8:
            main.wait_event(self._ev_wq)
        m.set_predicate(self.is_trainer_ptr)
        if self.fused_step:
            up = dict(fed=self.fed, upq_off=self.upq_off, n_samples=self.S,
                      n_loss_terms=self.steps * B, byz_mode=self.byz,
                      byz_scale=cfg.byzantine_scale, straggle_us=self.straggle_us) if self.fused_upload else {}
            self.trainer.train_epoch_fused(
                self.x_bf, self.y, self.steps, self.plan_ptr + self.sz["plan_step_barrier_off"],
                None, -1, -1,
                self.x_ready.data_ptr() if pipe else 0, self.in_seq.data_ptr() if pipe else 0,
                x_dq=self.x_dq, epoch_rows=self.S, **up)
        else:
            self.trainer.train_epoch(self.x_bf, self.y, self.steps, epoch_rows=self.S)
        m.set_predicate(0)
        if pipe:
            main.wait_event(self._ev_join)
        if not (self.fused_step and self.fused_upload):
            m.fed_upload(self.fed, self.S, self.steps * B, self.byz, cfg.byzantine_scale, self.straggle_us)
        if self.staged:
            if self.fp8:
                m.fed_pull_blobs(self.fed, self.upq_off[0], self.upq_off[1], self.cand_q, self.cand_shadow,
                                 self.in_dim, cfg.hidden, self.spec.by_name["w2"].shape[0], self._w_offs)
            else:
                m.fed_pull_candidates(self.fed, self.cand_shadow, self.cand_master, self.cand_ranges)
        H = cfg.hidden
        yv = self.y[: self.n_val]
        if self.val_chain:
            m.set_predicate(self.is_comm_ptr)
            m.mlp_val((self.x_dq if self.fp8 else self.x_bf)[: self.n_val], yv, self.val_correct, self.b_maps,
                      self.dyn_ptr[0], self.dyn_ptr[1], self.n_val, self.in_dim, H,
                      self.spec.by_name["w2"].shape[0], self.world,
                      self.plan_ptr + self.sz["plan_cand_blob_off"] if self.fp8 else 0)
            m.set_predicate(0)
        else:
            self._validate_two_gemms(self.x_bf[: self.n_val], yv, H)
        self._consensus(self.mirror.data_ptr() if (pipe and self.mirror_result) else 0,
                        self.in_seq.data_ptr() if pipe else 0)
        self.launches_per_round = int(m.launch_count() - n0)

    def _validate_two_gemms(self, xv, yv, H):
        m = self.mod
        m.gemm(xv, self.work_shadow, self.h_val, self.n_val, H, self.in_dim, self.world,
               self.in_dim, self.in_dim, 0, 0, False, False, False, G.EPI_GENERIC, 1, H,
               self.n_val * H, 1.0, None, G.ACT_RELU, None, None, 0, None, 1, False, None, 0, 1.0,
               None, None, self.b_maps, None, 0, 0, 0, 0, self.dyn_ptr[0], self.val_bn[0])
        m.gemm(self.h_val, self.work_shadow, None, self.n_val, self.spec.by_name["w2"].shape[0], H,
               self.world, H, H, self.n_val * H, 0, False, False, False, G.EPI_ARGMAX, 1, 0, 0, 1.0,
               None, 0, None, None, 0, None, 1, False, yv, 0, 1.0, None, self.val_correct,
               self.b_maps, None, 0, 0, 0, 0, self.dyn_ptr[1], self.val_bn[1])

    def capture(self):
        with torch.cuda.stream(self.stream):
            self._enqueue_round()
        self.stream.synchronize()
        self._rounds += 1
        if not self.cfg.cuda_graph:
            return
        g = torch.cuda.CUDAGraph()
        with torch.cuda.graph(g, stream=self.stream):
            self._enqueue_round()
        self.graph = g
        if self.pipelined_input:
            with torch.cuda.stream(self.stream):
                self.in_seq.fill_(-1)
                self.mod.prep_inputs_chunks(self.x_u8, self.x_bf, None, None,
                                            self.cfg.batch_size, self.epoch_steps, 1.0 / 255.0,
                                            self.in_flags, self.in_seq, self.cast_cnt, self.x_ready,
                                            self.in_err, self.x_dq)
                self.in_seq.zero_()
            self.stream.synchronize()
            gp = torch.cuda.CUDAGraph()
            with torch.cuda.graph(gp, stream=self.stream):
                self._enqueue_round(pipe=True)
            self.graph_pipe = gp
        self._stream_ptr = self.stream.cuda_stream
        if os.environ.get("BFLC_RAW_GRAPH_LAUNCH", "1") != "0":
            for gg in (self.graph, self.graph_pipe):
                try:
                    if gg is not None:
                        self._exec[id(gg)] = int(gg.raw_cuda_graph_exec())
                except Exception:
                    pass

    @property
    def consensus_captured(self) -> bool:
        return self.graph is not None

    def run_round(self, pipe: bool = False):
        self._next_round()
        if self._epoch_known is not None:
            self._epoch_known += 1
        g = self.graph_pipe if (pipe and self.graph_pipe is not None) else self.graph
        if g is not None:
            ex = self._exec.get(id(g))
            if ex:
                self.mod.graph_launch(ex, self._stream_ptr)
            else:
                with torch.cuda.stream(self.stream):
                    g.replay()
        else:
            with torch.cuda.stream(self.stream):
                self._enqueue_round(pipe=pipe)

    def run_round_e2e(self, host_x: Optional[torch.Tensor] = None,
                      host_y: Optional[torch.Tensor] = None) -> dict:
        hx = self.host_x if host_x is None else self._check_host(host_x, self.host_x, "host_x")
        hy = self.host_y if host_y is None else self._check_host(host_y, self.host_y, "host_y")
        if self.pipelined_input:
            self._seq += 1
            self._seq_np[0] = self._seq
            yb = hy.numel() * hy.element_size()
            if self._prefeed:
                self.mod.h2d_pipeline(hx.data_ptr(), self._pipe_dst, self._pipe_chunk, 0, 1,
                                      hy.data_ptr(), self._pipe_y, yb, *self._pipe_flags, self._tag_wv)
                self.run_round(pipe=True)
                self.mod.h2d_pipeline(hx.data_ptr(), self._pipe_dst, self._pipe_chunk, 1, self.epoch_steps,
                                      0, 0, 0, *self._pipe_flags, self._tag_wv)
            else:
                self.run_round(pipe=True)
                self.mod.h2d_pipeline(hx.data_ptr(), self._pipe_dst, self._pipe_chunk, 0, self.epoch_steps,
                                      hy.data_ptr(), self._pipe_y, yb, *self._pipe_flags, self._tag_wv)
        else:
            with torch.cuda.stream(self.stream):
                self.x_u8.copy_(hx, non_blocking=True)
                self.y.copy_(hy, non_blocking=True)
            self.run_round()
        if self.pipelined_input and self.mirror_result and self.graph_pipe is not None \
                and self._epoch_known is not None:
            self._wait_mirror(self._epoch_known)
            return parse_round_state(self._mirror_np, self.world)
        with torch.cuda.stream(self.stream):
            self.out_host.copy_(self.state_bytes, non_blocking=True)
        self.stream.synchronize()
        if self.pipelined_input:
            self._copy_stream.synchronize()
        st = self.read_state(self.out_host)
        self._epoch_known = st["epoch"]
        return st

    def _check_host(self, t: torch.Tensor, like: torch.Tensor, name: str) -> torch.Tensor:
        seen = self._host_checked.get(id(t))
        if seen is not None and seen() is t:
            return t
        if not (t.shape == like.shape and t.dtype == like.dtype and t.is_contiguous() and t.is_pinned()):
            raise ValueError(f"run_round_e2e: {name} must be a contiguous pinned {like.dtype} tensor of shape "
                             f"{tuple(like.shape)}, got {t.dtype} {tuple(t.shape)} "
                             f"(contiguous {t.is_contiguous()}, pinned {t.is_pinned()})")
        checked = self._host_checked
        checked[id(t)] = weakref.ref(t, lambda _, k=id(t): checked.pop(k, None))
        return t

    def _wait_mirror(self, want: int):
        m, n, t0 = self._mirror_np, 0, None
        seq = int(self.sz["kMirrorSeqWord"])
        while int(m[seq]) != want:
            n += 1
            if (n & 0x3FFF) == 0:
                now = time.monotonic()
                if t0 is None:
                    t0 = now
                elif now - t0 > 30.0:
                    raise RuntimeError(f"round result never reached the host mirror page (want epoch {want}, "
                                       f"have {int(m[seq])})")

    @property
    def h2d_bytes_per_round(self) -> int:
        tags = 4 * self.epoch_steps if self.pipelined_input else 0
        return self.host_x.numel() * self.host_x.element_size() + self.host_y.numel() * 4 + tags

    @property
    def d2h_bytes_per_round(self) -> int:
        if self.pipelined_input and self.mirror_result:
            return int(self.sz["RoundState"]) + 4
        return self.out_host.numel()

    def drain_blocks(self) -> List[str]:
        torch.cuda.synchronize()
        in_err = getattr(self, "in_err", None)
        if in_err is not None and int(in_err.item()):
            raise RuntimeError("input pipeline: a chunk's H2D tag never arrived (host stalled > 10 s "
                               "between launching the round and feeding it); the round ran on stale inputs")
        return ProtocolEngine.drain_blocks(self)

    def reset_host_caches(self):
        self._epoch_known = None

    @property
    def opt_moments(self) -> tuple:
        return self.trainer.m, self.trainer.v

    def global_model(self) -> Dict[str, torch.Tensor]:
        return {k: v.clone() for k, v in self.spec.views(self.global_master).items()}

    def evaluate(self, shard: Shard) -> float:
        torch.cuda.current_stream(self.dev).wait_stream(self.stream)
        x = shard.x.reshape(len(shard), -1).to(self.dev)
        xb = torch.empty(x.shape, device=self.dev, dtype=torch.bfloat16)
        self.mod.prep_inputs(x.contiguous(), xb, None, None, 1.0 / 255.0)
        cnt = self.trainer.accuracy_counts(xb, shard.y.to(self.dev, torch.int32),
                                           shadow=self.global_shadow, master=self.global_master)
        return float(cnt.item()) / len(shard)
```

Baseline: 4206.

## Run consensus prologue before PDL wait and parallelize blob quantization across lanes

The consensus kernel now waits on trained flags and gathers role, sample and cost metadata before its PDL grid-dependency wait when the validation chain is active, so that setup overlaps the tail of validation. Record writing moves from a single thread to per-thread stores, and the MLP validation kernel now triggers its dependents after its own wait rather than at entry. MX-FP8 blob quantization spreads each 32-element group across 8 lanes with a shuffle-based amax reduction instead of one thread per group. Optional globaltimer debug stamps are added behind a null pointer. The risk is that reads moved ahead of the PDL wait could observe state that the previous kernel has not yet finished writing.

```diff
diff --git a/bflc_demo_b200/csrc/bindings/bindings_extra.cpp b/bflc_demo_b200/csrc/bindings/bindings_extra.cpp
--- a/bflc_demo_b200/csrc/bindings/bindings_extra.cpp
+++ b/bflc_demo_b200/csrc/bindings/bindings_extra.cpp
@@ -241,7 +241,7 @@
                                       int64_t bump_seq, int rule, int trim, int server_opt,
                                       const std::vector<float>& server_hp, int64_t server_m_off,
                                       int64_t server_v_off, int dp_mode, double dp_clip, double dp_noise,
-                                      uint64_t dp_seed, int64_t dp_off) {
+                                      uint64_t dp_seed, int64_t dp_off, bool early_prologue, int64_t dbg) {
     TORCH_CHECK(bflc::agg_rule_valid(rule, trim), "fed_consensus_aggregate: rule must be 0 (FedAvg), 1 (median) "
                 "or 2 (trimmed mean, 1 <= trim <= ", bflc::kMaxTrim, "), got rule ", rule, " trim ", trim);
     TORCH_CHECK(rule == bflc::AGG_FEDAVG || !weight_by_score,
@@ -269,13 +269,15 @@
                 "fed_consensus_aggregate: dp_off must be a positive multiple of 16 (the HeapLayout dp region)");
     check(bflc::fed_consensus_aggregate(make_fed(fd), n_val, weight_by_score ? 1 : 0,
                                         two_shot ? 1 : 0, use_mc ? 1 : 0, cur_stream(),
-                                        P<uint32_t>(host_mirror), P<uint32_t>(bump_seq), rule, trim, &so, &dp),
+                                        P<uint32_t>(host_mirror), P<uint32_t>(bump_seq), rule, trim, &so, &dp,
+                                        early_prologue ? 1 : 0, P<unsigned long long>(dbg)),
           "fed_consensus_aggregate");
   }, py::arg("fed"), py::arg("n_val"), py::arg("weight_by_score"), py::arg("two_shot"),
      py::arg("use_mc"), py::arg("host_mirror") = 0, py::arg("bump_seq") = 0, py::arg("rule") = 0,
      py::arg("trim") = 0, py::arg("server_opt") = 0, py::arg("server_hp") = std::vector<float>{},
      py::arg("server_m_off") = 0, py::arg("server_v_off") = 0, py::arg("dp_mode") = 0, py::arg("dp_clip") = 0.0,
-     py::arg("dp_noise") = 0.0, py::arg("dp_seed") = 0, py::arg("dp_off") = 0);
+     py::arg("dp_noise") = 0.0, py::arg("dp_seed") = 0, py::arg("dp_off") = 0,
+     py::arg("early_prologue") = false, py::arg("dbg") = 0);
   m.def("fed_update_norms", [](const py::dict& fd, int64_t dp_off) {
     TORCH_CHECK(dp_off > 0 && dp_off % 16 == 0, "fed_update_norms: dp_off must be a positive multiple of 16");
     check(bflc::fed_update_norms(make_fed(fd), dp_off, cur_stream()), "fed_update_norms");
diff --git a/bflc_demo_b200/csrc/include/bflc_kernels.h b/bflc_demo_b200/csrc/include/bflc_kernels.h
--- a/bflc_demo_b200/csrc/include/bflc_kernels.h
+++ b/bflc_demo_b200/csrc/include/bflc_kernels.h
@@ -456,7 +456,13 @@
                                     int two_shot, int use_multicast, cudaStream_t s,
                                     uint32_t* host_mirror = nullptr, uint32_t* bump_seq = nullptr,
                                     int rule = 0, int trim = 0, const ServerOptArgs* so = nullptr,
-                                    const DpArgs* dp = nullptr);
+                                    const DpArgs* dp = nullptr, int early_prologue = 0,
+                                    unsigned long long* dbg = nullptr);
+constexpr int kConsDbgSlots = 16;
+enum ConsDbgSlot {
+  CDBG_ENTRY = 0, CDBG_PROLOGUE = 1, CDBG_PDL_WAIT = 2, CDBG_FLAGS = 3, CDBG_GATHER = 4, CDBG_DECIDE = 5,
+  CDBG_FEDAVG = 6, CDBG_ARRIVE = 7, CDBG_LAST_FENCE = 8, CDBG_RECORD = 9, CDBG_MIRROR = 10, CDBG_END = 11,
+};
 cudaError_t fed_update_norms(const FedArgs& f, long long dp_off, cudaStream_t s);
 
 cudaError_t fed_pull_candidates(const FedArgs& f, void* stage_shadow, float* stage_master,
diff --git a/bflc_demo_b200/csrc/kernels/elementwise_optim.cu b/bflc_demo_b200/csrc/kernels/elementwise_optim.cu
--- a/bflc_demo_b200/csrc/kernels/elementwise_optim.cu
+++ b/bflc_demo_b200/csrc/kernels/elementwise_optim.cu
@@ -458,23 +458,34 @@
   const float* master; long long off_w1, off_b1, off_w2, off_b2;
   int in_dim, hidden, n_classes; uint8_t* blob; Mx8MlpLayout l; __nv_bfloat16* dq;
 };
-__device__ __forceinline__ void blob_group(const float* w, int ld, int rows, int K, int row, int g, int n_kb,
+constexpr int kBlobLanes = 8;
+__device__ __forceinline__ void blob_group(const float* w, int ld, int rows, int K, int row, int g, int j, int n_kb,
                                            uint8_t* q, uint8_t* sf, int q_rows, __nv_bfloat16* dq) {
   uint8_t* sfp = sf + epi::mx8_sf_index(row, g, n_kb);
   const int k0 = g * 32;
-  if (k0 >= K || row >= q_rows) { *sfp = 127; return; }
+  if (k0 >= K || row >= q_rows) {
+    if (j == 0) *sfp = 127;
+    return;
+  }
   const int n = K - k0 < 32 ? K - k0 : 32;
-  float v[32];
-#pragma unroll
-  for (int i = 0; i < 32; ++i) v[i] = (row < rows && i < n) ? w[static_cast<long long>(row) * ld + k0 + i] : 0.f;
-  uint32_t o[8];
-  const int e = epi::mx8_quant32(v, o);
-  *sfp = static_cast<uint8_t>(e);
-  uint8_t* qp = q + static_cast<long long>(row) * ld + k0;
-  for (int i = 0; i < n / 4; ++i) reinterpret_cast<uint32_t*>(qp)[i] = o[i];
-  if (dq != nullptr) {
-    __nv_bfloat16* d = dq + static_cast<long long>(row) * ld + k0;
-    for (int i = 0; i < n / 4; ++i) *reinterpret_cast<uint2*>(d + 4 * i) = epi::mx8_dq4(o[i], e);
+  const int c = 4 * j;
+  float v[4];
+  float amax = 0.f;
+#pragma unroll
+  for (int i = 0; i < 4; ++i) {
+    v[i] = (row < rows && c + i < n) ? w[static_cast<long long>(row) * ld + k0 + c + i] : 0.f;
+    amax = fmaxf(amax, fabsf(v[i]));
+  }
+  const unsigned mask = 0xFFu << (threadIdx.x & 24);
+#pragma unroll
+  for (int o = 1; o < kBlobLanes; o <<= 1) amax = fmaxf(amax, __shfl_xor_sync(mask, amax, o));
+  const int e = epi::mx8_scale_byte(amax);
+  const float inv = epi::mx8_inv_scale(e);
+  if (j == 0) *sfp = static_cast<uint8_t>(e);
+  if (c + 4 <= n) {
+    const uint32_t o = epi::mx8_pack4(v[0] * inv, v[1] * inv, v[2] * inv, v[3] * inv);
+    *reinterpret_cast<uint32_t*>(q + static_cast<long long>(row) * ld + k0 + c) = o;
+    if (dq != nullptr) *reinterpret_cast<uint2*>(dq + static_cast<long long>(row) * ld + k0 + c) = epi::mx8_dq4(o, e);
   }
 }
 __global__ void __launch_bounds__(256) k_quantize_mlp_blob(BlobArgs a) {
@@ -482,16 +493,18 @@
   ptx::pdl_wait();
   const int g1 = a.l.kb1 * 4, g2 = a.l.kb2 * 4;
   const int r1 = (a.hidden + 127) / 128 * 128;
-  const long long n1 = static_cast<long long>(r1) * g1, n2 = 128LL * g2, n3 = a.hidden + 64;
+  const long long n1 = static_cast<long long>(r1) * g1 * kBlobLanes, n2 = 128LL * g2 * kBlobLanes;
+  const long long n3 = a.hidden + 64;
   const long long stride = static_cast<long long>(gridDim.x) * blockDim.x;
   for (long long i = blockIdx.x * static_cast<long long>(blockDim.x) + threadIdx.x; i < n1 + n2 + n3; i += stride) {
     if (i < n1) {
-      blob_group(a.master + a.off_w1, a.in_dim, a.hidden, a.in_dim, static_cast<int>(i / g1), static_cast<int>(i % g1),
-                 a.l.kb1, a.blob + a.l.w1q, a.blob + a.l.w1sf, a.hidden, a.dq);
+      const long long u = i / kBlobLanes;
+      blob_group(a.master + a.off_w1, a.in_dim, a.hidden, a.in_dim, static_cast<int>(u / g1), static_cast<int>(u % g1),
+                 static_cast<int>(i % kBlobLanes), a.l.kb1, a.blob + a.l.w1q, a.blob + a.l.w1sf, a.hidden, a.dq);
     } else if (i < n1 + n2) {
-      const long long u = i - n1;
+      const long long u = (i - n1) / kBlobLanes;
       blob_group(a.master + a.off_w2, a.hidden, a.n_classes, a.hidden, static_cast<int>(u / g2), static_cast<int>(u % g2),
-                 a.l.kb2, a.blob + a.l.w2q, a.blob + a.l.w2sf, 64,
+                 static_cast<int>(i % kBlobLanes), a.l.kb2, a.blob + a.l.w2q, a.blob + a.l.w2sf, 64,
                  a.dq != nullptr ? a.dq + static_cast<long long>(a.hidden) * a.in_dim : nullptr);
     } else {
       const int u = static_cast<int>(i - n1 - n2);
@@ -554,8 +567,8 @@
   if (in_dim % 4 != 0 || hidden % 4 != 0 || n_classes > 64) return cudaErrorInvalidValue;
   BlobArgs a{master, off_w1, off_b1, off_w2, off_b2, in_dim, hidden, n_classes, blob,
              mx8_mlp_layout(in_dim, hidden), static_cast<__nv_bfloat16*>(dq)};
-  const long long total = static_cast<long long>((hidden + 127) / 128 * 128) * a.l.kb1 * 4 + 128LL * a.l.kb2 * 4 +
-                          hidden + 64;
+  const long long total = (static_cast<long long>((hidden + 127) / 128 * 128) * a.l.kb1 * 4 + 128LL * a.l.kb2 * 4) *
+                              kBlobLanes + hidden + 64;
   note_launch();
   return launch_pdl(k_quantize_mlp_blob, dim3(grid_for(total)), dim3(kBlock), 0, s, a);
 }
diff --git a/bflc_demo_b200/csrc/kernels/fed_kernels.cu b/bflc_demo_b200/csrc/kernels/fed_kernels.cu
--- a/bflc_demo_b200/csrc/kernels/fed_kernels.cu
+++ b/bflc_demo_b200/csrc/kernels/fed_kernels.cu
@@ -190,11 +190,17 @@
 template <bool kRobust, int kServerOpt, int kDp>
 __device__ __forceinline__ void consensus_body(FedArgs f, int n_val, int weight_by_score, int two_shot, int use_mc,
                                                uint32_t* host_mirror, uint32_t* bump_seq, uint32_t agg,
-                                               ServerOptArgs so, DpArgs dp, DpShared* dsh) {
+                                               ServerOptArgs so, DpArgs dp, DpShared* dsh, int early,
+                                               unsigned long long* dbg) {
   __shared__ ConsShared sh;
   __shared__ bool last;
+  unsigned long long* drow = dbg != nullptr && threadIdx.x == 0 ? dbg + blockIdx.x * kConsDbgSlots : nullptr;
+  auto dstamp = [&](int slot) {
+    if (drow != nullptr) drow[slot] = globaltimer_ns();
+  };
+  dstamp(CDBG_ENTRY);
   ptx::pdl_launch_dependents();
-  ptx::pdl_wait();
+  if (!early) ptx::pdl_wait();
   char* me = f.peers.base[f.rank];
   RoundState* st = at<RoundState>(me, f.lay.state_off);
   RoundPlan* plan = at<RoundPlan>(me, f.lay.plan_off);
@@ -203,20 +209,44 @@
   const uint32_t par = epoch & 1u;
   const int n = f.n_ranks;
   const bool i_am_comm = (st->role[f.rank] & ROLE_COMM) != 0;
-  if (blockIdx.x == 0 && threadIdx.x == 0) stamp(plan, STAMP_CONS_BEGIN);
 
   const bool fk = admit::first_k(st);
   __shared__ int cand_of[kMaxRanks];
   __shared__ uint32_t adm_mask;
   if (threadIdx.x == 0) {
     uint32_t m = 0;
-    for (int z = 0; z < plan->n_cand; ++z) {
+    const int n_cand = plan->n_cand;
+    for (int z = 0; z < n_cand; ++z) {
       cand_of[z] = fk ? admit::wait_slot(admit::page(me, f.lay, par), z, epoch) : plan->cand_rank[z];
       m |= 1u << cand_of[z];
     }
     adm_mask = m;
-  }
-  __syncthreads();
+    ConsensusIn<kMaxRanks>& in = sh.in;
+    in.n_ranks = n;
+    in.n_comm = static_cast<int>(st->n_comm);
+    in.n_aggregate = static_cast<int>(st->n_aggregate);
+    in.weight_by_score = weight_by_score;
+  }
+  __syncthreads();
+  if (threadIdx.x < n) {
+    const int r = threadIdx.x;
+    if ((st->role[r] & ROLE_TRAINER) && ((adm_mask >> r) & 1u)) ptx::wait_flag_ge(flags + FLAG_TRAINED + r, epoch + 1);
+  }
+  __syncthreads();
+  if (threadIdx.x >= kMaxRanks * kMaxRanks && threadIdx.x < kMaxRanks * kMaxRanks + kMaxRanks) {
+    ConsensusIn<kMaxRanks>& in = sh.in;
+    const UploadMeta* meta = at<UploadMeta>(me, f.lay.meta_off) + par * kMaxRanks;
+    const int r = threadIdx.x - kMaxRanks * kMaxRanks;
+    in.role[r] = r < n ? st->role[r] : 0u;
+    in.admitted[r] = (r < n && (st->role[r] & ROLE_TRAINER) && ((adm_mask >> r) & 1u)) ? 1 : 0;
+    in.n_samples[r] = r < n ? ptx::ld_relaxed_sys(&meta[r].n_samples) : 0u;
+    in.avg_cost[r] =
+        r < n ? __uint_as_float(ptx::ld_relaxed_sys(reinterpret_cast<const uint32_t*>(&meta[r].avg_cost))) : 0.f;
+  }
+  dstamp(CDBG_PROLOGUE);
+  ptx::pdl_wait();
+  dstamp(CDBG_PDL_WAIT);
+  if (blockIdx.x == 0 && threadIdx.x == 0) stamp(plan, STAMP_CONS_BEGIN);
 
   if (blockIdx.x == 0 && i_am_comm) {
     if (threadIdx.x < n) {
@@ -234,40 +264,25 @@
   if (threadIdx.x < n) {
     const int r = threadIdx.x;
     if (st->role[r] & ROLE_COMM) ptx::wait_flag_ge(flags + FLAG_SCORED + r, epoch + 1);
-    if ((st->role[r] & ROLE_TRAINER) && ((adm_mask >> r) & 1u)) ptx::wait_flag_ge(flags + FLAG_TRAINED + r, epoch + 1);
   }
   __syncthreads();
   if (blockIdx.x == 0 && threadIdx.x == 0) stamp(plan, STAMP_CONS_SCORED);
-
-  {
+  dstamp(CDBG_FLAGS);
+
+  if (threadIdx.x < kMaxRanks * kMaxRanks) {
     ConsensusIn<kMaxRanks>& in = sh.in;
     const float* rows = at<float>(me, f.lay.scores_off) + par * kMaxRanks * kMaxRanks;
-    const UploadMeta* meta = at<UploadMeta>(me, f.lay.meta_off) + par * kMaxRanks;
-    const int i = threadIdx.x;
-    if (i < kMaxRanks * kMaxRanks) {
-      const int r = i / kMaxRanks, t = i % kMaxRanks;
-      const bool ok = r < n && t < n && (st->role[r] & ROLE_COMM) && (st->role[t] & ROLE_TRAINER) &&
-                      ((adm_mask >> t) & 1u);
-      in.scored[r][t] = ok ? 1 : 0;
-      in.score[r][t] =
-          ok ? __uint_as_float(ptx::ld_relaxed_sys(reinterpret_cast<const uint32_t*>(rows + r * kMaxRanks + t))) : 0.f;
-    } else if (i < kMaxRanks * kMaxRanks + kMaxRanks) {
-      const int r = i - kMaxRanks * kMaxRanks;
-      in.role[r] = r < n ? st->role[r] : 0u;
-      in.admitted[r] = (r < n && (st->role[r] & ROLE_TRAINER) && ((adm_mask >> r) & 1u)) ? 1 : 0;
-      in.n_samples[r] = r < n ? ptx::ld_relaxed_sys(&meta[r].n_samples) : 0u;
-      in.avg_cost[r] =
-          r < n ? __uint_as_float(ptx::ld_relaxed_sys(reinterpret_cast<const uint32_t*>(&meta[r].avg_cost))) : 0.f;
-    }
-  }
-  __syncthreads();
+    const int r = threadIdx.x / kMaxRanks, t = threadIdx.x % kMaxRanks;
+    const bool ok = r < n && t < n && (st->role[r] & ROLE_COMM) && (st->role[t] & ROLE_TRAINER) &&
+                    ((adm_mask >> t) & 1u);
+    in.scored[r][t] = ok ? 1 : 0;
+    in.score[r][t] =
+        ok ? __uint_as_float(ptx::ld_relaxed_sys(reinterpret_cast<const uint32_t*>(rows + r * kMaxRanks + t))) : 0.f;
+  }
+  __syncthreads();
+  dstamp(CDBG_GATHER);
   if (threadIdx.x == 0) {
-    ConsensusIn<kMaxRanks>& in = sh.in;
-    in.n_ranks = n;
-    in.n_comm = static_cast<int>(st->n_comm);
-    in.n_aggregate = static_cast<int>(st->n_aggregate);
-    in.weight_by_score = weight_by_score;
-    run_consensus<kMaxRanks>(in, sh.out);
+    run_consensus<kMaxRanks>(sh.in, sh.out);
     int k = 0;
     for (int r = 0; r < n; ++r)
       if (sh.out.selected[r]) {
@@ -278,6 +293,7 @@
     sh.n_sel = k;
   }
   __syncthreads();
+  dstamp(CDBG_DECIDE);
   if constexpr (kDp != DP_OFF) {
     if (threadIdx.x < n) ptx::wait_flag_ge(flags + FLAG_NORM + threadIdx.x, epoch + 1);
     __syncthreads();
@@ -437,12 +453,14 @@
   if ((threadIdx.x & 31) == 0 && dig) atomicAdd(&plan->digest_acc, dig);
 
   __syncthreads();
+  dstamp(CDBG_FEDAVG);
   if (threadIdx.x == 0) {
     __threadfence_system();
     const unsigned done = atomicAdd(&plan->consensus_blocks_done, 1u);
     last = (done == gridDim.x - 1);
   }
   __syncthreads();
+  dstamp(CDBG_ARRIVE);
   if (!last) return;
   __threadfence_system();
 
@@ -463,70 +481,80 @@
     __syncthreads();
   }
 
-  if (threadIdx.x == 0) {
-    unsigned long long digest = 0ull;
-    if (two_shot) {
-      const unsigned long long* slots =
-          reinterpret_cast<const unsigned long long*>(at<float>(me, f.lay.scores_off) +
-                                                      2 * kMaxRanks * kMaxRanks) +
-          par * kMaxRanks;
-      for (int r = 0; r < n; ++r)
-        digest += *reinterpret_cast<const volatile unsigned long long*>(slots + r);
-    } else {
-      digest = *reinterpret_cast<volatile unsigned long long*>(&plan->digest_acc);
-    }
+  dstamp(CDBG_LAST_FENCE);
+  {
     const ConsensusIn<kMaxRanks>& in = sh.in;
     const ConsensusOut<kMaxRanks>& out = sh.out;
     BlockRecord* rec =
         at<BlockRecord>(me, f.lay.ring_off) + (epoch % static_cast<uint32_t>(f.lay.ring_slots));
-    rec->epoch = epoch;
-    rec->n_ranks = static_cast<uint32_t>(n);
-    rec->n_comm = st->n_comm;
-    rec->n_aggregate = st->n_aggregate;
-    uint32_t adm = 0, sel = 0;
-    for (int r = 0; r < kMaxRanks; ++r) {
+    const int i = threadIdx.x;
+    if (i < kMaxRanks * kMaxRanks) {
+      rec->score_rows[i / kMaxRanks][i % kMaxRanks] = in.score[i / kMaxRanks][i % kMaxRanks];
+    } else if (i < kMaxRanks * kMaxRanks + kMaxRanks) {
+      const int r = i - kMaxRanks * kMaxRanks;
+      uint32_t m = 0;
+      for (int t = 0; t < kMaxRanks; ++t)
+        if (in.scored[r][t]) m |= 1u << t;
+      rec->scored_mask[r] = m;
       rec->role_before[r] = in.role[r];
       rec->role_after[r] = r < n ? out.role_after[r] : 0u;
-      uint32_t m = 0;
-      for (int t = 0; t < kMaxRanks; ++t) {
-        rec->score_rows[r][t] = in.score[r][t];
-        if (in.scored[r][t]) m |= 1u << t;
-      }
-      rec->scored_mask[r] = m;
       rec->median[r] = r < n ? out.median[r] : 0.f;
       rec->n_samples[r] = in.n_samples[r];
       rec->avg_cost[r] = in.avg_cost[r];
       rec->weight[r] = r < n ? out.weight[r] : 0.f;
-      if (in.admitted[r]) adm |= 1u << r;
-      if (r < n && out.selected[r]) sel |= 1u << r;
-    }
-    rec->admitted_mask = adm;
-    rec->selected_mask = sel;
-    rec->global_loss = out.global_loss;
-    rec->weight_by_score = static_cast<uint32_t>(weight_by_score);
-    rec->model_digest = digest;
-    rec->agg = agg;
-    __threadfence();
-    rec->seq = epoch + 1;
-    for (int r = 0; r < n; ++r) {
-      st->role[r] = out.role_after[r];
-      st->last_median[r] = out.median[r];
-    }
-    st->selected_mask = sel;
-    st->global_loss = out.global_loss;
-    st->model_digest = digest;
-    st->blocks_appended = st->blocks_appended + 1;
-    st->epoch = epoch + 1;
-    if constexpr (kDp != DP_OFF) {
-      DpPage* page = at<DpPage>(me, dp.off);
-      for (int t = 0; t < kMaxRanks; ++t) {
-        page->norm[t] = dsh->norm[t];
-        page->scale[t] = dsh->scale[t];
-      }
-      page->sigma = dsh->sigma;
-      page->epoch = epoch + 1;
-    }
-    __threadfence_system();
+      if (r < n) {
+        st->role[r] = out.role_after[r];
+        st->last_median[r] = out.median[r];
+      }
+      if constexpr (kDp != DP_OFF) {
+        DpPage* page = at<DpPage>(me, dp.off);
+        page->norm[r] = dsh->norm[r];
+        page->scale[r] = dsh->scale[r];
+      }
+    } else if (i == kMaxRanks * kMaxRanks + kMaxRanks) {
+      unsigned long long digest = 0ull;
+      if (two_shot) {
+        const unsigned long long* slots =
+            reinterpret_cast<const unsigned long long*>(at<float>(me, f.lay.scores_off) +
+                                                        2 * kMaxRanks * kMaxRanks) +
+            par * kMaxRanks;
+        for (int r = 0; r < n; ++r)
+          digest += *reinterpret_cast<const volatile unsigned long long*>(slots + r);
+      } else {
+        digest = *reinterpret_cast<volatile unsigned long long*>(&plan->digest_acc);
+      }
+      uint32_t adm = 0, sel = 0;
+      for (int r = 0; r < kMaxRanks; ++r) {
+        if (in.admitted[r]) adm |= 1u << r;
+        if (r < n && out.selected[r]) sel |= 1u << r;
+      }
+      rec->epoch = epoch;
+      rec->n_ranks = static_cast<uint32_t>(n);
+      rec->n_comm = st->n_comm;
+      rec->n_aggregate = st->n_aggregate;
+      rec->admitted_mask = adm;
+      rec->selected_mask = sel;
+      rec->global_loss = out.global_loss;
+      rec->weight_by_score = static_cast<uint32_t>(weight_by_score);
+      rec->model_digest = digest;
+      rec->agg = agg;
+      st->selected_mask = sel;
+      st->global_loss = out.global_loss;
+      st->model_digest = digest;
+      st->blocks_appended = st->blocks_appended + 1;
+      if constexpr (kDp != DP_OFF) {
+        DpPage* page = at<DpPage>(me, dp.off);
+        page->sigma = dsh->sigma;
+        page->epoch = epoch + 1;
+      }
+    }
+    __syncthreads();
+    dstamp(CDBG_RECORD);
+    if (threadIdx.x == 0) {
+      __threadfence();
+      rec->seq = epoch + 1;
+      st->epoch = epoch + 1;
+    }
   }
   __syncthreads();
   if (bump_seq != nullptr && threadIdx.x == 0) *bump_seq = *bump_seq + 1u;
@@ -539,27 +567,31 @@
     __syncthreads();
     if (threadIdx.x == 0) ptx::st_release_sys(host_mirror + kMirrorSeqWord, epoch + 1);
   }
+  dstamp(CDBG_MIRROR);
   if (threadIdx.x < n)
     ptx::st_release_sys(
         at<uint32_t>(f.peers.base[threadIdx.x], f.lay.flags_off) + FLAG_DONE + f.rank, epoch + 1);
   if (threadIdx.x == 0) stamp(plan, STAMP_CONS_END);
+  dstamp(CDBG_END);
 }
 
 template <bool kRobust, int kServerOpt>
 __global__ void __launch_bounds__(kFedThreads)
 k_consensus(FedArgs f, int n_val, int weight_by_score, int two_shot, int use_mc,
-            uint32_t* host_mirror, uint32_t* bump_seq, uint32_t agg, ServerOptArgs so) {
+            uint32_t* host_mirror, uint32_t* bump_seq, uint32_t agg, ServerOptArgs so, int early,
+            unsigned long long* dbg) {
   consensus_body<kRobust, kServerOpt, DP_OFF>(f, n_val, weight_by_score, two_shot, use_mc, host_mirror, bump_seq,
-                                               agg, so, DpArgs{}, nullptr);
+                                               agg, so, DpArgs{}, nullptr, early, dbg);
 }
 
 template <bool kRobust, int kServerOpt, int kDp>
 __global__ void __launch_bounds__(kFedThreads)
 k_consensus_dp(FedArgs f, int n_val, int weight_by_score, int two_shot, int use_mc,
-               uint32_t* host_mirror, uint32_t* bump_seq, uint32_t agg, ServerOptArgs so, DpArgs dp) {
+               uint32_t* host_mirror, uint32_t* bump_seq, uint32_t agg, ServerOptArgs so, DpArgs dp, int early,
+               unsigned long long* dbg) {
   __shared__ DpShared dsh;
   consensus_body<kRobust, kServerOpt, kDp>(f, n_val, weight_by_score, two_shot, use_mc, host_mirror, bump_seq,
-                                           agg, so, dp, &dsh);
+                                           agg, so, dp, &dsh, early, dbg);
 }
 
 __global__ void __launch_bounds__(kFedThreads) k_update_norms(FedArgs f, long long dp_off) {
@@ -808,40 +840,42 @@
 template <bool kRobust>
 static cudaError_t launch_consensus(int opt, dim3 grid, dim3 block, cudaStream_t s, const FedArgs& f, int n_val,
                                     int weight_by_score, int two_shot, int use_multicast, uint32_t* host_mirror,
-                                    uint32_t* bump_seq, uint32_t agg, const ServerOptArgs& so) {
+                                    uint32_t* bump_seq, uint32_t agg, const ServerOptArgs& so, int early,
+                                    unsigned long long* dbg) {
   switch (opt) {
     case SOPT_MOMENTUM:
       return launch_pdl(k_consensus<kRobust, SOPT_MOMENTUM>, grid, block, 0, s, f, n_val, weight_by_score, two_shot,
-                        use_multicast, host_mirror, bump_seq, agg, so);
+                        use_multicast, host_mirror, bump_seq, agg, so, early, dbg);
     case SOPT_ADAM:
       return launch_pdl(k_consensus<kRobust, SOPT_ADAM>, grid, block, 0, s, f, n_val, weight_by_score, two_shot,
-                        use_multicast, host_mirror, bump_seq, agg, so);
+                        use_multicast, host_mirror, bump_seq, agg, so, early, dbg);
     case SOPT_YOGI:
       return launch_pdl(k_consensus<kRobust, SOPT_YOGI>, grid, block, 0, s, f, n_val, weight_by_score, two_shot,
-                        use_multicast, host_mirror, bump_seq, agg, so);
+                        use_multicast, host_mirror, bump_seq, agg, so, early, dbg);
     default:
       return launch_pdl(k_consensus<kRobust, SOPT_NONE>, grid, block, 0, s, f, n_val, weight_by_score, two_shot,
-                        use_multicast, host_mirror, bump_seq, agg, so);
+                        use_multicast, host_mirror, bump_seq, agg, so, early, dbg);
   }
 }
 
 template <bool kRobust, int kDp>
 static cudaError_t launch_consensus_dp(int opt, dim3 grid, dim3 block, cudaStream_t s, const FedArgs& f, int n_val,
                                        int weight_by_score, int two_shot, int use_multicast, uint32_t* host_mirror,
-                                       uint32_t* bump_seq, uint32_t agg, const ServerOptArgs& so, const DpArgs& dp) {
+                                       uint32_t* bump_seq, uint32_t agg, const ServerOptArgs& so, const DpArgs& dp,
+                                       int early, unsigned long long* dbg) {
   switch (opt) {
     case SOPT_MOMENTUM:
       return launch_pdl(k_consensus_dp<kRobust, SOPT_MOMENTUM, kDp>, grid, block, 0, s, f, n_val, weight_by_score,
-                        two_shot, use_multicast, host_mirror, bump_seq, agg, so, dp);
+                        two_shot, use_multicast, host_mirror, bump_seq, agg, so, dp, early, dbg);
     case SOPT_ADAM:
       return launch_pdl(k_consensus_dp<kRobust, SOPT_ADAM, kDp>, grid, block, 0, s, f, n_val, weight_by_score,
-                        two_shot, use_multicast, host_mirror, bump_seq, agg, so, dp);
+                        two_shot, use_multicast, host_mirror, bump_seq, agg, so, dp, early, dbg);
     case SOPT_YOGI:
       return launch_pdl(k_consensus_dp<kRobust, SOPT_YOGI, kDp>, grid, block, 0, s, f, n_val, weight_by_score,
-                        two_shot, use_multicast, host_mirror, bump_seq, agg, so, dp);
+                        two_shot, use_multicast, host_mirror, bump_seq, agg, so, dp, early, dbg);
     default:
       return launch_pdl(k_consensus_dp<kRobust, SOPT_NONE, kDp>, grid, block, 0, s, f, n_val, weight_by_score,
-                        two_shot, use_multicast, host_mirror, bump_seq, agg, so, dp);
+                        two_shot, use_multicast, host_mirror, bump_seq, agg, so, dp, early, dbg);
   }
 }
 
@@ -856,7 +890,8 @@
 cudaError_t fed_consensus_aggregate(const FedArgs& f, int n_val, int weight_by_score,
                                     int two_shot, int use_multicast, cudaStream_t s,
                                     uint32_t* host_mirror, uint32_t* bump_seq, int rule, int trim,
-                                    const ServerOptArgs* so, const DpArgs* dp) {
+                                    const ServerOptArgs* so, const DpArgs* dp, int early_prologue,
+                                    unsigned long long* dbg) {
   if (!agg_rule_valid(rule, trim) || (rule != AGG_FEDAVG && weight_by_score)) return cudaErrorInvalidValue;
   ServerOptArgs sa{};
   if (so != nullptr) sa = *so;
@@ -875,20 +910,21 @@
   note_launch();
   const dim3 grid(fed_grid(work)), block(kFedThreads);
   const uint32_t agg = agg_word(rule, trim, sa.opt, da.mode);
+  const int early = early_prologue ? 1 : 0;
   if (da.mode == DP_CLIP && rule == AGG_FEDAVG)
     return launch_consensus_dp<false, DP_CLIP>(sa.opt, grid, block, s, f, n_val, weight_by_score, two_shot,
-                                               use_multicast, host_mirror, bump_seq, agg, sa, da);
+                                               use_multicast, host_mirror, bump_seq, agg, sa, da, early, dbg);
   if (da.mode == DP_CLIP)
     return launch_consensus_dp<true, DP_CLIP>(sa.opt, grid, block, s, f, n_val, weight_by_score, two_shot,
-                                              use_multicast, host_mirror, bump_seq, agg, sa, da);
+                                              use_multicast, host_mirror, bump_seq, agg, sa, da, early, dbg);
   if (da.mode == DP_NOISE)
     return launch_consensus_dp<false, DP_NOISE>(sa.opt, grid, block, s, f, n_val, weight_by_score, two_shot,
-                                                use_multicast, host_mirror, bump_seq, agg, sa, da);
+                                                use_multicast, host_mirror, bump_seq, agg, sa, da, early, dbg);
   if (rule == AGG_FEDAVG)
     return launch_consensus<false>(sa.opt, grid, block, s, f, n_val, weight_by_score, two_shot, use_multicast,
-                                   host_mirror, bump_seq, agg, sa);
+                                   host_mirror, bump_seq, agg, sa, early, dbg);
   return launch_consensus<true>(sa.opt, grid, block, s, f, n_val, weight_by_score, two_shot, use_multicast,
-                                host_mirror, bump_seq, agg, sa);
+                                host_mirror, bump_seq, agg, sa, early, dbg);
 }
 
 cudaError_t fed_pull_candidates(const FedArgs& f, void* stage_shadow, float* stage_master,
diff --git a/bflc_demo_b200/csrc/kernels/mlp_val_sm100.cu b/bflc_demo_b200/csrc/kernels/mlp_val_sm100.cu
--- a/bflc_demo_b200/csrc/kernels/mlp_val_sm100.cu
+++ b/bflc_demo_b200/csrc/kernels/mlp_val_sm100.cu
@@ -95,7 +95,6 @@
   uint64_t* hx = w2k + 1;
   float* sb = reinterpret_cast<float*>(smem + kOffBar + kBarBytes);
 
-  ptx::pdl_launch_dependents();
   const int warp = threadIdx.x >> 5, lane = threadIdx.x & 31;
   const uint32_t rank = blockIdx.x & 1;
   const bool leader = rank == 0;
@@ -113,6 +112,7 @@
   }
   ptx::cluster_sync();
   ptx::pdl_wait();
+  ptx::pdl_launch_dependents();
   const bool inactive = (v.pred != nullptr && *v.pred == 0) || z >= v.dyn1->active_batches;
   if (inactive) return;
   const int kb_d = (v.in_dim + 63) / 64;
diff --git a/bflc_demo_b200/engine/base.py b/bflc_demo_b200/engine/base.py
--- a/bflc_demo_b200/engine/base.py
+++ b/bflc_demo_b200/engine/base.py
@@ -185,13 +185,15 @@
             if errs:
                 raise RuntimeError(f"host/device ledgers disagree: {errs[:2]}")
 
-    def _consensus(self, mirror_ptr: int = 0, seq_ptr: int = 0):
+    def _consensus(self, mirror_ptr: int = 0, seq_ptr: int = 0, early_prologue: bool = False):
         m, cfg = self.mod, self.cfg
         if self.dp_kw:
             m.fed_update_norms(self.fed, self.layout.offsets["dp"])
+        dbg = getattr(self, "consensus_dbg", None)
         m.fed_consensus_aggregate(self.fed, self.n_val_targets, cfg.weight_by_score, self.two_shot, self.multicast,
                                   mirror_ptr, seq_ptr, cfg.aggregation_rule, cfg.trim,
-                                  **self.server_kw, **self.dp_kw)
+                                  **self.server_kw, **self.dp_kw, early_prologue=early_prologue,
+                                  dbg=dbg.data_ptr() if dbg is not None else 0)
 
     @property
     def consensus_captured(self) -> bool:
diff --git a/bflc_demo_b200/engine/fused.py b/bflc_demo_b200/engine/fused.py
--- a/bflc_demo_b200/engine/fused.py
+++ b/bflc_demo_b200/engine/fused.py
@@ -222,7 +222,7 @@
         else:
             self._validate_two_gemms(self.x_bf[: self.n_val], yv, H)
         self._consensus(self.mirror.data_ptr() if (pipe and self.mirror_result) else 0,
-                        self.in_seq.data_ptr() if pipe else 0)
+                        self.in_seq.data_ptr() if pipe else 0, early_prologue=self.val_chain)
         self.launches_per_round = int(m.launch_count() - n0)
 
     def _validate_two_gemms(self, xv, yv, H):
```

Result: no change. 4275, median of 6 (+1.6%).
